# tusen-ai/SST

Measured on AMD Instinct MI355X. Metric: LiDAR frames/sec (SST backbone fwd+bwd) at Waymo 0.32m voxels, higher is better.
Workload: dtype f32 (storage, accumulation, attention, LayerNorm, reductions: fp32; the dense products of the encoder layers from the EXACT three-way bf16 split of both fp32 operands, six bf16 MFMA products with fp32 accumulation - error vs float64 <= 2 x the fp32 matrix pipe's: tests/test_gpu_dense_f32x6.py)

## Files before the change

include/sst_amd.h:

```cpp
#ifndef SST_AMD_H
#define SST_AMD_H

#include <stdint.h>

#ifdef __cplusplus
extern "C" {
#endif

#define SST_OK 0
#define SST_ERR_ARG (-1)
#define SST_ERR_UNSUPPORTED (-2)
#define SST_ERR_KEYSPACE (-3)

typedef enum { SST_REDUCE_SUM = 0, SST_REDUCE_MEAN = 1, SST_REDUCE_MAX = 2 } sst_reduce_t;

const char* sst_version(void);

int sst_dynamic_voxelize_f32(const float* d_points, int64_t n, int64_t row_stride,
                             const float voxel_size[3], const float coors_range[6],
                             int32_t* d_coors, int64_t coors_stride, int coors_col0, int batch_idx,
                             void* stream);
void sst_dynamic_voxelize_grid(const float voxel_size[3], const float coors_range[6], int32_t grid_xyz[3]);

int64_t sst_scan_workspace_bytes(int64_t n);
// ... 162 lines not shown
  float* out_b;
  int32_t p, bias_side, transpose_out, reserved;
} sst_wgrad_problem_bf16;
int64_t sst_wgrad_group_workspace_bytes(const sst_wgrad_problem_bf16* problems, int n);
int sst_wgrad_group_bf16(const sst_wgrad_problem_bf16* problems, int n, void* d_workspace, void* stream);
typedef struct sst_cast_problem_bf16 {
  const float* src;
  void* dst;
  int64_t ld_src;
  int32_t rows, cols, transpose, reserved;
} sst_cast_problem_bf16;
int sst_cast_group_bf16(const sst_cast_problem_bf16* problems, int n, void* stream);

int sst_gather_rows_f32(const float* d_src, int64_t ld_src, const int32_t* d_idx, int64_t n_out, int c,
                        float fill, float* d_out, int64_t ld_out, void* stream);
int sst_add_table_rows_f32(const float* d_x, int64_t ldx, const float* d_table, int64_t ld_table, const int32_t* d_idx, int64_t m,
                           int c, float* d_out, int64_t ld_out, void* stream);
int sst_scatter_rows_f32(const float* d_src, int64_t ld_src, const int32_t* d_idx, int64_t n_src, int c,
                         float* d_out, int64_t ld_out, void* stream);

int sst_add_layernorm_act_fwd_f32(const float* d_x, const float* d_res, const float* d_weight, const float* d_bias,
                                  int64_t m, int c, float eps, int act, float* d_y, float* d_sum, float* d_stats,
                                  void* stream);
int sst_add_layernorm_act_bwd_f32(const float* d_dy, const float* d_sum, const float* d_stats, const float* d_weight,
                                  const float* d_bias, int act, int64_t m, int c, float* d_dx, float* d_dweight,
                                  float* d_dbias, void* d_workspace, void* stream);
int sst_add_layernorm_fwd_f32(const float* d_x, const float* d_res, const float* d_weight, const float* d_bias,
                              int64_t m, int c, float eps, float* d_y, float* d_sum, float* d_stats,
                              void* stream);
int sst_add_layernorm_pos_fwd_f32(const float* d_x, const float* d_res, const float* d_weight, const float* d_bias, int64_t m,
                                  int c, float eps, float* d_y, float* d_sum, float* d_stats, const float* d_pos_table,
                                  const int32_t* d_pos_idx, float* d_y_plus_pos, void* stream);
int64_t sst_add_layernorm_bwd_workspace_bytes(int64_t m, int c);
int sst_add_layernorm_bwd_f32(const float* d_dy, const float* d_sum, const float* d_stats,
                              const float* d_weight, int64_t m, int c, float* d_dx, float* d_dweight,
                              float* d_dbias, void* d_workspace, void* stream);
int64_t sst_colsum_workspace_bytes(int64_t m, int c);
int sst_colsum_f32(const float* d_x, int64_t m, int c, int64_t ld, float* d_out, void* d_workspace, void* stream);

int64_t sst_weight_grad_workspace_bytes(int64_t m, int out, int in);
int sst_weight_grad_f32(const float* d_dy, const float* d_x, int64_t m, int out, int in, int64_t ld_dy,
                        int64_t ld_x, float* d_dw, float* d_db, void* d_workspace, void* stream);
typedef struct sst_wgrad_problem_f32 {
  const float* dy;
  const float* x;
  int64_t m, ld_dy, ld_x;
  float* dw;
  float* db;
  int32_t out, in;
  const float* x_add_rows;
  const int32_t* x_add_index;
} sst_wgrad_problem_f32;
int64_t sst_weight_grad_group_workspace_bytes(const sst_wgrad_problem_f32* problems, int n);
int sst_weight_grad_group_f32(const sst_wgrad_problem_f32* problems, int n, void* d_workspace, void* stream);
int64_t sst_weight_grad_group_f32x6_workspace_bytes(const sst_wgrad_problem_f32* problems, int n);
int sst_weight_grad_group_f32x6(const sst_wgrad_problem_f32* problems, int n, void* d_workspace, void* stream);
int sst_weight_grad_group_f32x6_plan(const sst_wgrad_problem_f32* problems, int n, int* tiles, int* slices,
                                     int64_t* tokens_per_slice, int* lean_slices);

int64_t sst_bn_workspace_bytes(int64_t n, int c);
int sst_bn_stats_f32(const float* d_x, int64_t n, int c, int64_t ld, float* d_mean, float* d_var,
                     void* d_workspace, void* stream);
int sst_bn_act_fwd_f32(const float* d_x, int64_t n, int c, int64_t ldx, const float* d_scale,
                       const float* d_shift, int act, float* d_y, int64_t ldy, void* stream);
int sst_bn_act_bwd_reduce_f32(const float* d_dy, const float* d_x, int64_t n, int c, int64_t lddy, int64_t ldx,
                              const float* d_mean, const float* d_invstd, const float* d_scale,
                              const float* d_shift, int act, float* d_sum_g, float* d_sum_gxhat,
                              void* d_workspace, void* stream);
int sst_bn_act_bwd_apply_f32(const float* d_dy, const float* d_x, int64_t n, int c, int64_t lddy, int64_t ldx,
                             const float* d_mean, const float* d_invstd, const float* d_scale,
                             const float* d_shift, const float* d_coef_a, const float* d_coef_b, float coef_scale,
                             int act, float* d_dx, int64_t lddx, void* stream);
int sst_bn_prepare_f32(const float* d_x, int64_t n, int c, int64_t ld, const float* d_weight, const float* d_bias,
                       float eps, float* d_running_mean, float* d_running_var, float factor, float* d_out4,
                       void* d_workspace, void* stream);
int sst_bn_prepare_tracked_f32(const float* d_x, int64_t n, int c, int64_t ld, const float* d_weight,
                               const float* d_bias, float eps, float* d_running_mean, float* d_running_var,
                               float factor, int64_t* d_num_batches_tracked, float* d_out4, void* d_workspace,
                               void* stream);
int sst_vfe_linear_moments_f32(const float* d_x, int64_t ldx, int64_t n, int k, const float* d_w, int64_t ldw, int c,
                               float* d_y, int64_t ldy, void* d_workspace, void* stream);
int sst_bn_prepare_from_partials_f32(int64_t n, int c, const float* d_weight, const float* d_bias, float eps,
                                     float* d_running_mean, float* d_running_var, float factor,
                                     int64_t* d_num_batches_tracked, float* d_out4, void* d_workspace, void* stream);
int sst_bn_stats_from_partials_f32(int64_t n, int c, float* d_mean, float* d_var, void* d_workspace, void* stream);
int sst_bn_act_pool_bwd_reduce_f32(const float* d_dy, const float* d_x, int64_t n, int c, int64_t lddy, int64_t ldx,
                                   const float* d_mean, const float* d_invstd, const float* d_scale, const float* d_shift,
                                   int act, const int32_t* d_group, const int32_t* d_arg, const float* d_dpool, int64_t ldp,
                                   float* d_sum_g, float* d_sum_gxhat, void* d_workspace, void* stream);
int sst_bn_act_pool_bwd_apply_f32(const float* d_dy, const float* d_x, int64_t n, int c, int64_t lddy, int64_t ldx,
                                  const float* d_mean, const float* d_invstd, const float* d_scale, const float* d_shift,
                                  const float* d_coef_a, const float* d_coef_b, float coef_scale, int act,
                                  const int32_t* d_group, const int32_t* d_arg, const float* d_dpool, int64_t ldp, float* d_dx,
                                  int64_t lddx, void* stream);
int sst_bn_act_res_fwd_f32(const float* d_x, int64_t n, int c, int64_t ldx, const float* d_res, int64_t ldr,
                           const float* d_scale, const float* d_shift, int act, float* d_y, int64_t ldy, void* stream);
int sst_bn_act_res_bwd_reduce_f32(const float* d_dy, const float* d_x, const float* d_res, int64_t n, int c,
                                  int64_t lddy, int64_t ldx, int64_t ldr, const float* d_mean, const float* d_invstd,
                                  const float* d_scale, const float* d_shift, int act, float* d_sum_g,
                                  float* d_sum_gxhat, void* d_workspace, void* stream);
int sst_bn_act_res_bwd_apply_f32(const float* d_dy, const float* d_x, const float* d_res, int64_t n, int c,
                                 int64_t lddy, int64_t ldx, int64_t ldr, const float* d_mean, const float* d_invstd,
                                 const float* d_scale, const float* d_shift, const float* d_coef_a,
                                 const float* d_coef_b, float coef_scale, int act, float* d_dres, int64_t lddres,
                                 float* d_dx, int64_t lddx, void* stream);

int sst_tall_linear_f32(const float* d_x, int64_t ldx, const float* d_w, int64_t ldw, const float* d_bias,
                        int64_t m, int n, int k, int trans_w, int accumulate, float* d_y, int64_t ldy,
                        void* stream);
int sst_tall_linear_ln_f32(const float* d_x, int64_t ldx, const float* d_w, int64_t ldw, const float* d_bias, int64_t m, int k,
                           const float* d_res, int64_t ldres, const float* d_ln_weight, const float* d_ln_bias, float eps,
                           float* d_y, float* d_sum, float* d_stats, const float* d_pos_table, const int32_t* d_pos_idx,
                           float* d_y_plus_pos, void* stream);
int sst_tall_linear_epi_f32x3(const float* d_x, int64_t ldx, const float* d_w, int64_t ldw, int trans_w, const float* d_bias,
                              int64_t m, int k, int n, int epilogue, const float* d_aux_in, float* d_aux_out, int64_t ldaux,
                              float* d_y, int64_t ldy, void* stream);
int sst_tall_linear_ln_f32x3(const float* d_x, int64_t ldx, const float* d_w, int64_t ldw, const float* d_bias, int64_t m, int k,
                             const float* d_res, int64_t ldres, const float* d_ln_weight, const float* d_ln_bias, float eps,
                             float* d_y, float* d_sum, float* d_stats, const float* d_pos_table, const int32_t* d_pos_idx,
                             float* d_y_plus_pos, void* stream);
int sst_tall_linear_epi_f32x6(const float* d_x, int64_t ldx, const float* d_w, int64_t ldw, int trans_w, const float* d_bias,
                              int64_t m, int k, int n, int epilogue, const float* d_aux_in, float* d_aux_out, int64_t ldaux,
                              float* d_y, int64_t ldy, void* stream);
int sst_tall_linear_epi2_f32x6(const float* d_x, const float* d_x2, int x2_from_col, int64_t ldx, const float* d_w, int64_t ldw,
                               int trans_w, const float* d_bias, int64_t m, int k, int n, int epilogue, const float* d_aux_in,
                               float* d_aux_out, int64_t ldaux, float* d_y, int64_t ldy, void* stream);
int sst_tall_linear_add_rows_f32x6(const float* d_x, int64_t ldx, const float* d_w, int64_t ldw, int64_t m, int k, int n,
                                   const float* d_rows, int64_t ldrows, const int32_t* d_row_index, float* d_y, int64_t ldy,
                                   void* stream);
int sst_inproj_pos_f32x6(const float* d_x, int64_t ldx, const float* d_rows, const int32_t* d_index, const float* d_w, int64_t ldw,
                         const float* d_bias, int64_t m, float* d_y, int64_t ldy, void* stream);
int sst_tall_linear_f32x6_partition(int64_t m, int groups, int64_t* row_blocks, int64_t* rows_per_wave);
int sst_tall_linear_ln_f32x6(const float* d_x, int64_t ldx, const float* d_w, int64_t ldw, const float* d_bias, int64_t m, int k,
                             const float* d_res, int64_t ldres, const float* d_ln_weight, const float* d_ln_bias, float eps,
                             float* d_y, float* d_sum, float* d_stats, const float* d_pos_table, const int32_t* d_pos_idx,
                             float* d_y_plus_pos, void* stream);
int sst_add_layernorm_bwd2_f32(const float* d_dy, const float* d_dy2, const float* d_sum, const float* d_stats,
                               const float* d_weight, int64_t m, int c, float* d_dx, float* d_dweight, float* d_dbias,
                               void* d_workspace, void* stream);
typedef struct sst_encoder_layer_fwd_args {
  int64_t m, n_windows;
  int32_t n_heads, act, max_tokens, impl;
  float eps, scale;
  const float *x, *xp;
  const float *w_in, *b_in, *w_out, *b_out, *w1, *b1, *w2, *b2, *n1w, *n1b, *n2w, *n2b;
  const int32_t *tok, *winoff, *order;
  const float* pos_table;
  const int32_t* pos_idx;
  float *qkv, *o, *lse, *y1, *s1, *st1, *pre, *h, *s2, *y2, *st2, *y2p;
  const float* head_scale;
  void* wpack;
  const float* xpos_table;
  const int32_t* xpos_idx;
} sst_encoder_layer_fwd_args;
typedef struct sst_encoder_layer_bwd_args {
  int64_t m, n_windows;
  int32_t n_heads, act, max_tokens, impl;
  float eps, scale;
  const float *dy2, *dy2p;
  const float *x, *xp, *qkv, *o, *lse, *s1, *st1, *y1, *pre, *h, *s2, *st2;
  const float *w_in, *w_out, *w1, *w2, *n1w, *n2w;
  const int32_t *tok, *winoff, *order;
  float *ds2, *dpre, *ds1, *d_o, *dqkv;
  float *dw_in, *db_in, *dwo, *dbo, *dw1, *db1, *dw2, *db2, *dn1w, *dn1b, *dn2w, *dn2b;
  void* workspace;
  const float* head_scale;
  float* cos_r;
  float* dy1;
  const void* wpack;
  const float* xpos_table;
  const int32_t* xpos_idx;
} sst_encoder_layer_bwd_args;
int64_t sst_encoder_layer_bwd_workspace_bytes(int64_t m, int n_heads);
int64_t sst_encoder_layer_wpack_bytes(void);
int sst_encoder_layer_fwd_f32x6(const sst_encoder_layer_fwd_args* args, void* stream);
int sst_encoder_layer_bwd_f32x6(const sst_encoder_layer_bwd_args* args, void* stream);

typedef struct sst_encoder_tail_fwd_args {
  int64_t m;
  int32_t act, reserved;
  float eps, reserved_f;
  const float *o, *x;
  const void* packed;
  const float *b_out, *b1, *b2, *n1w, *n1b, *n2w, *n2b;
  const float* pos_table;
  const int32_t* pos_idx;
  float *s1, *st1, *y1, *pre, *h, *s2, *st2, *y2, *y2p;
} sst_encoder_tail_fwd_args;
typedef struct sst_encoder_tail_bwd_args {
  int64_t m;
  int32_t act, reserved;
  const float *dy2, *dy2p, *s2, *st2, *pre, *s1, *st1;
  const void* packed;
  const float *n1w, *n2w;
  float *ds2, *dpre, *ds1, *d_o;
  float *dn2w, *dn2b, *dn1w, *dn1b;
  void* workspace;
} sst_encoder_tail_bwd_args;
int64_t sst_encoder_tail_pack_bytes(void);
int sst_encoder_tail_pack_f32x6(const float* d_w_out, const float* d_w1, const float* d_w2, void* d_packed, void* stream);
int sst_encoder_tail_pack_f32x6_many(const float* const* d_w_out, const float* const* d_w1, const float* const* d_w2,
                                     void* const* d_packed, int n, void* stream);
int64_t sst_encoder_tail_bwd_workspace_bytes(int64_t m);
int sst_encoder_tail_fwd_f32x6(const sst_encoder_tail_fwd_args* args, void* stream);
int sst_encoder_tail_bwd_f32x6(const sst_encoder_tail_bwd_args* args, void* stream);

typedef struct sst_encoder_tail_fwd_bf16_args {
  int64_t m;
  int32_t act, reserved;
  float eps, reserved_f;
  const void *o, *x;
  const void* packed;
  const float *b_out, *b1, *b2, *n1w, *n1b, *n2w, *n2b;
  const float* pos_table;
  const int32_t* pos_idx;
  void* s1;
  float* st1;
  void *y1, *pre, *h, *s2;
  float* st2;
  void *y2, *y2p;
} sst_encoder_tail_fwd_bf16_args;
typedef struct sst_encoder_tail_bwd_bf16_args {
  int64_t m;
  int32_t act, reserved;
  const void *dy2, *dy2p, *s2;
  const float* st2;
  const void *pre, *s1;
  const float* st1;
  const void* packed;
  const float *n1w, *n2w;
  void *ds2, *dpre, *ds1, *d_o;
  float *dn2w, *dn2b, *dn1w, *dn1b;
  void* workspace;
} sst_encoder_tail_bwd_bf16_args;
int64_t sst_encoder_tail_pack_bf16_bytes(void);
int sst_encoder_tail_pack_bf16(const float* d_w_out, const float* d_w1, const float* d_w2, void* d_packed, void* stream);
int sst_encoder_tail_pack_bf16_many(const float* const* d_w_out, const float* const* d_w1, const float* const* d_w2,
                                    void* const* d_packed, int n, void* stream);
int64_t sst_encoder_tail_bwd_bf16_workspace_bytes(int64_t m);
int sst_encoder_tail_fwd_bf16(const sst_encoder_tail_fwd_bf16_args* args, void* stream);
int sst_encoder_tail_bwd_bf16(const sst_encoder_tail_bwd_bf16_args* args, void* stream);

typedef struct sst_encoder_layer_fwd_bf16_args {
  int64_t m, n_windows;
  int32_t n_heads, act, max_tokens, reserved;
  float eps, scale;
  const void *x, *xp;
  const void *wqk, *wv, *wout, *w1, *w2;
  const float *b_in, *b_out, *b1, *b2, *n1w, *n1b, *n2w, *n2b;
  const int32_t *tok, *winoff, *order;
  const float* pos_table;
  const int32_t* pos_idx;
  void *qk, *v, *o;
  float* lse;
  void *y1, *s1;
  float* st1;
  void *pre, *h, *s2;
  float* st2;
  void *y2, *y2p;
  const float* head_scale;
  const void* wpack;
} sst_encoder_layer_fwd_bf16_args;
typedef struct sst_encoder_layer_bwd_bf16_args {
  int64_t m, n_windows;
  int32_t n_heads, act, max_tokens, reserved;
  float eps, scale;
  const void *dy2, *dy2p;
  const void *x, *xp, *qk, *v, *o;
  const float* lse;
  const void* s1;
  const float* st1;
  const void *y1, *pre, *h, *s2;
  const float* st2;
  const void *wqk_t, *wv_t, *wout_t, *w1_t, *w2_t;
  const float *n1w, *n2w;
  const int32_t *tok, *winoff, *order;
  void *ds2, *dpre, *dy1, *ds1, *d_o, *dqkv, *dxp, *dx;
  float *dw_in, *db_in, *dwo, *dbo, *dw1, *db1, *dw2, *db2, *dn1w, *dn1b, *dn2w, *dn2b;
  void* workspace;
  const float* head_scale;
  float* cos_r;
  const void* wpack;
} sst_encoder_layer_bwd_bf16_args;
int64_t sst_encoder_layer_bwd_bf16_workspace_bytes(int64_t m);
int sst_encoder_layer_fwd_bf16(const sst_encoder_layer_fwd_bf16_args* args, void* stream);
int sst_encoder_layer_bwd_bf16(const sst_encoder_layer_bwd_bf16_args* args, void* stream);

int sst_tall_linear_epi_f32(const float* d_x, int64_t ldx, const float* d_w, int64_t ldw, int trans_w, const float* d_bias,
                            int64_t m, int k, int n, int epilogue, const float* d_aux_in, float* d_aux_out, int64_t ldaux,
                            float* d_y, int64_t ldy, void* stream);
int sst_tall_linear_gelu_f32(const float* d_x, int64_t ldx, const float* d_w, int64_t ldw, const float* d_bias,
                             int64_t m, int n, int k, int trans_w, int mode, float* d_aux, float* d_y, int64_t ldy,
                             void* stream);

void* sst_event_create(void);
void sst_event_destroy(void* ev);
float sst_event_elapsed_ms(void* start, void* stop);
int sst_sra_attn_profile_next_fwd(void* start, void* stop);
int sst_sra_attn_profile_next_bwd(void* start, void* stop);

int64_t sst_connected_components_workspace_bytes(int64_t n);
int sst_connected_components_xy_f32(const float* d_points, int64_t ld, const int32_t* d_batch, int64_t n, float dist,
                                    int32_t* d_labels, int32_t* d_num_components, void* d_workspace, void* stream);

int64_t sst_dynamic_point_pool_workspace_bytes(int64_t n_rois, int64_t n_pts);
int sst_dynamic_point_pool_f32(const float* d_rois, const int32_t* d_rois_batch, int64_t n_rois, const float* d_pts,
                               int64_t ld_pts, const int32_t* d_pts_batch, int64_t n_pts, const float* extra_wlh,
                               int max_inbox_point, int64_t max_all_pts, int64_t* d_out_pts_idx,
                               int64_t* d_out_roi_idx, float* d_out_feats, int64_t* d_num_out, void* d_workspace,
                               void* stream);

int sst_spconv_candidates_i32(const int32_t* d_coors, int64_t n, const int32_t* in_shape, const int32_t* out_shape,
                              const int32_t* ksize, const int32_t* stride, const int32_t* padding,
                              const int32_t* dilation, int transpose, int32_t* d_rows, void* stream);
int sst_spconv_inverse_to_map_i32(const int32_t* d_inverse, int64_t total, int32_t* d_in2out, void* stream);
int sst_spconv_grid_subm_i32(const int32_t* d_coors, int64_t n, int batch, const int32_t* shape, const int32_t* ksize,
                             const int32_t* dilation, int32_t* d_grid, int32_t* d_in2out, int32_t* d_out2in,
                             void* stream);
int64_t sst_spconv_grid_conv_workspace_bytes(int64_t cells);
int sst_spconv_grid_conv_count_i32(const int32_t* d_coors, int64_t n, int batch, const int32_t* in_shape,
                                   const int32_t* out_shape, const int32_t* ksize, const int32_t* stride,
                                   const int32_t* padding, const int32_t* dilation, int transpose, void* d_workspace,
                                   int32_t* d_num_out, void* stream);
int sst_spconv_grid_conv_maps_i32(const int32_t* d_coors, int64_t n, int batch, const int32_t* in_shape,
                                  const int32_t* out_shape, const int32_t* ksize, const int32_t* stride,
                                  const int32_t* padding, const int32_t* dilation, int transpose, void* d_workspace,
                                  int64_t m, int32_t* d_outids, int32_t* d_in2out, int32_t* d_out2in, void* stream);
int sst_spconv_subm_map_i32(const int32_t* d_coors, int64_t n, const int32_t* shape, const int32_t* ksize,
                            const int32_t* dilation, const uint64_t* d_sorted_keys, const uint32_t* d_perm,
                            int32_t* d_in2out, void* stream);
int sst_spconv_invert_map_i32(const int32_t* d_in2out, int kvol, int64_t n, int64_t m, int32_t* d_out2in,
                              void* stream);
int64_t sst_spconv_pair_lists_workspace_bytes(int kvol, int64_t n);
int sst_spconv_pair_lists_i32(const int32_t* d_in2out, int kvol, int64_t n, int32_t* d_pairs, int32_t* d_num,
                              void* d_workspace, void* stream);
int sst_spconv_gather_gemm_f32(const float* d_x, int64_t ldx, const int32_t* d_map, int64_t m, int kvol,
                               const float* d_w, int cin, int cout, int trans_w, const float* d_bias, float* d_y,
                               int64_t ldy, int form, void* stream);
int sst_spconv_maxpool_fwd_f32(const float* d_x, int64_t ldx, const int32_t* d_out2in, int64_t m, int kvol, int c,
                               float* d_y, int64_t ldy, void* stream);
int sst_spconv_maxpool_bwd_f32(const float* d_x, int64_t ldx, const float* d_y, int64_t ldy, const float* d_dy,
                               int64_t lddy, const int32_t* d_in2out, int64_t n, int kvol, int c, float* d_dx,
                               int64_t lddx, void* stream);
int64_t sst_spconv_conv_os_workspace_bytes(int kvol, int cin, int cout);
int sst_spconv_conv_os_tile_rows(int64_t m, int cout, int tile_cfg);
int sst_spconv_os_tile_work_i32(const int32_t* d_map, int64_t m, int kvol, int tile_rows, int32_t* d_work, void* stream);
int sst_spconv_conv_os_f32(const float* d_x, int64_t ldx, const int32_t* d_map, int64_t m, int kvol, const float* d_w,
                           int cin, int cout, int trans_w, const float* d_bias, float* d_y, int64_t ldy,
                           int tile_cfg, const int32_t* d_tile_order, void* d_workspace, void* stream);
int sst_spconv_conv_os_f32x3(const float* d_x, int64_t ldx, const int32_t* d_map, int64_t m, int kvol, const float* d_w,
                             int cin, int cout, int trans_w, const float* d_bias, float* d_y, int64_t ldy, int tile_cfg,
// ... 701 lines not shown
```

sst_amd/_lib.py:

```python
import ctypes
import os
import subprocess

import torch

_HERE = os.path.dirname(os.path.abspath(__file__))
_CSRC = os.path.join(_HERE, 'csrc')
LIB_PATH = os.path.join(_CSRC, 'libsst_amd.so')

_lib = None

c_i64 = ctypes.c_int64
c_i32 = ctypes.c_int
c_f32 = ctypes.c_float
c_ptr = ctypes.c_void_p



class WgradProblemBF16(ctypes.Structure):
    _fields_ = [('a', c_ptr), ('b', c_ptr), ('lda', c_i64), ('ldb', c_i64), ('m', c_i64), ('out_w', c_ptr),
                ('out_b', c_ptr), ('p', ctypes.c_int32), ('bias_side', ctypes.c_int32),
                ('transpose_out', ctypes.c_int32), ('reserved', ctypes.c_int32)]


# ... 18 lines not shown
                ('out', ctypes.c_int32), ('inn', ctypes.c_int32), ('x_add_rows', c_ptr), ('x_add_index', c_ptr)]


def _struct(name, doc, fields):
    return type(name, (ctypes.Structure,), {'__doc__': doc, '_fields_': fields})


_I32 = ctypes.c_int32
RoiAssignArgs = _struct('RoiAssignArgs', 'sst_roi_assign_args of include/sst_amd.h', (
    [(k, ctypes.c_void_p) for k in ('props', 'prop_labels', 'prop_offsets', 'gts', 'gt_labels', 'gt_offsets', 'iou', 'max_iou',
                                    'argmax')]
    + [(k, c_i64) for k in ('n_props', 'n_gts', 'ld')]
    + [(k, _I32) for k in ('prop_cols', 'gt_cols', 'batch', 'num_classes', 'class_mask', 'reserved')]))
RoiSampleArgs = _struct('RoiSampleArgs', 'sst_roi_sample_args of include/sst_amd.h', (
    [(k, ctypes.c_void_p) for k in ('props', 'prop_labels', 'prop_offsets', 'gts', 'gt_labels', 'gt_offsets', 'iou', 'max_iou',
                                    'argmax', 'keys', 'assigned', 'rois', 'src', 'gt_index', 'labels', 'iou_out', 'soft_label',
                                    'reg_mask', 'targets', 'counts')]
    + [(k, c_i64) for k in ('n_props', 'n_gts', 'ld', 'max_props_per_sample')]
    + [(k, _I32) for k in ('prop_cols', 'gt_cols', 'batch', 'num_classes', 'class_mask', 'num', 'num_expected_pos', 'n_pieces')]
    + [(k, ctypes.c_float * 16) for k in ('pos_iou_thr', 'neg_iou_thr', 'min_pos_iou')]
    + [('piece_thr', ctypes.c_float * 8)]
    + [(k, ctypes.c_double * 16) for k in ('cls_pos_thr', 'cls_neg_thr')]
    + [('piece_frac', ctypes.c_double * 8)]))
RoiLossArgs = _struct('RoiLossArgs', 'sst_roi_loss_args of include/sst_amd.h', (
    [(k, ctypes.c_void_p) for k in ('cls_score', 'bbox_pred', 'nonempty', 'rois', 'soft_label', 'reg_mask', 'targets',
                                    'gt_index', 'labels', 'gts')]
    + [(k, c_i64) for k in ('n', 'n_gts')]
    + [(k, _I32) for k in ('roi_cols', 'gt_cols', 'with_corner', 'car_index')]
    + [(k, ctypes.c_float) for k in ('beta', 'w_cls', 'w_reg', 'w_corner')]
    + [('code_weight', ctypes.c_float * 7), ('reserved', ctypes.c_float)]))

AnchorGrid = _struct('AnchorGrid', 'sst_anchor_grid of include/sst_amd.h', (
    [('centers', ctypes.c_void_p)] + [(k, _I32) for k in ('H', 'W', 'n_sizes', 'n_rots')]
    + [('sizes', ctypes.c_float * 3 * 8), ('rots', ctypes.c_float * 4)]))
AnchorLossArgs = _struct('AnchorLossArgs', 'sst_anchor_loss_args of include/sst_amd.h', (
    [(k, ctypes.c_void_p) for k in ('cls_score', 'bbox_pred', 'dir_pred', 'assigned', 'gts', 'gt_labels', 'gt_offsets',
                                    'pos_counts')]
    + [('n_gts', c_i64)]
    + [(k, _I32) for k in ('gt_cols', 'batch', 'num_classes', 'smooth_l1', 'sin_diff', 'reserved')]
    + [(k, ctypes.c_float) for k in ('gamma', 'alpha', 'w_cls', 'w_bbox', 'w_dir', 'beta', 'pos_weight', 'dir_offset')]
    + [('code_weight', ctypes.c_float * 7), ('reserved_f', ctypes.c_float)]))

FgSampleArgs = _struct('FgSampleArgs', 'sst_fg_sample_args of include/sst_amd.h', (
    [(k, ctypes.c_void_p) for k in ('logits', 'votes', 'points', 'batch_idx', 'extra_mask', 'slot', 'mask', 'src', 'centers',
                                    'batch_out', 'points_out', 'info', 'aux', 'aux_out', 'aux_inv')]
    + [(k, c_i64) for k in ('n', 'ld_logits', 'ld_votes', 'ld_points', 'max_rows', 'aux_rows')]
    + [(k, _I32) for k in ('num_classes', 'point_cols', 'batch', 'batch_is_i64', 'apply_rule', 'sample_major')]
    + [('thresholds', ctypes.c_float * 32)]))
FgGatherArgs = _struct('FgGatherArgs', 'sst_fg_gather_args of include/sst_amd.h', (
    [(k, ctypes.c_void_p) for k in ('idx', 'logits', 'votes', 'feats', 'points', 'out', 'points_out')]
    + [(k, c_i64) for k in ('m', 'n', 'ld_logits', 'ld_votes', 'ld_feats', 'ld_points')]
    + [(k, _I32) for k in ('c_logits', 'c_votes', 'c_feats', 'c_points')]))
FgGroupSampleArgs = _struct('FgGroupSampleArgs', 'sst_fg_group_sample_args of include/sst_amd.h', (
    [(k, ctypes.c_void_p) for k in ('logits', 'votes', 'points', 'batch_idx', 'extra_mask', 'slot', 'mask', 'src', 'centers',
                                    'batch_out', 'points_out', 'info')]
    + [(k, c_i64) for k in ('n', 'ld_logits', 'ld_votes', 'ld_points', 'max_rows')]
    + [(k, _I32) for k in ('num_groups', 'num_logits', 'point_cols', 'batch', 'batch_is_i64', 'apply_rule')]
    + [('offset_scale', ctypes.c_float), ('thresholds', ctypes.c_float * 32), ('group_begin', ctypes.c_uint8 * 33),
       ('group_class', ctypes.c_uint8 * 64)]))
FgVirtualRowsArgs = _struct('FgVirtualRowsArgs', 'sst_fg_virtual_rows_args of include/sst_amd.h', (
    [(k, ctypes.c_void_p) for k in ('src', 'centers', 'feats', 'logits', 'points', 'out', 'clipped')]
    + [(k, c_i64) for k in ('m', 'n', 'ld_feats', 'ld_logits', 'ld_points')]
    + [(k, _I32) for k in ('c_feats', 'c_logits', 'c_points', 'reserved')]
    + [('lo', ctypes.c_float * 3), ('hi', ctypes.c_float * 3)]))
DeformConvShape = _struct('DeformConvShape', 'sst_deform_conv_shape of include/sst_amd.h', [
    (k, _I32) for k in ('batch', 'in_channels', 'height', 'width', 'out_channels', 'kernel_h', 'kernel_w', 'stride_h', 'stride_w',
                        'pad_h', 'pad_w', 'dil_h', 'dil_w', 'groups', 'deform_groups', 'reserved')])
OptimHyper = _struct('OptimHyper', 'sst_optim_hyper of include/sst_amd.h', (
    [(k, ctypes.c_double * 8) for k in ('lr', 'wd', 'b1', 'b2', 'eps')]
    + [(k, ctypes.c_double) for k in ('max_norm', 'growth_factor', 'backoff_factor')]
    + [(k, _I32) for k in ('growth_interval', 'scale_mode', 'skip_nonfinite', 'n_groups')]))
TrackletTargetsArgs = _struct('TrackletTargetsArgs', 'sst_tracklet_targets_args of include/sst_amd.h', (
    [(k, ctypes.c_void_p) for k in ('boxes', 'ts', 'scores', 'trk_offsets', 'cand_boxes', 'cand_ts', 'cand_offsets',
                                    'trk_cand_offsets', 'trk_class', 'chosen', 'counts', 'matched', 'overlaps',
                                    'assigned_gt_inds', 'rois', 'src', 'frame_inds', 'gt_index', 'labels', 'iou_out',
                                    'scores_out', 'soft_label', 'reg_mask', 'targets', 'pos_gt_bboxes')]
    + [(k, c_i64) for k in ('n_rows', 'n_cand_rows', 'n_cands', 'n_tracklets')]
    + [(k, _I32) for k in ('num_classes', 'object_centric')]
    + [(k, ctypes.c_float) for k in ('candidate_thresh', 'iou_thr')]
    + [(k, ctypes.c_double * 16) for k in ('cls_pos_thr', 'cls_neg_thr')]))
TrackletRowsArgs = _struct('TrackletRowsArgs', 'sst_tracklet_rows_args of include/sst_amd.h', (
    [(k, ctypes.c_void_p) for k in ('feats', 'xyz', 'pts_frame_inds', 'pts_inds', 'roi_inds', 'roi_frame_inds', 'roi_scores',
                                    'out', 'xyz_out')]
    + [(k, c_i64) for k in ('m', 'n_points', 'n_rois', 'ld_feats', 'ld_xyz')]
    + [(k, _I32) for k in ('feat_cols', 'xyz_cols', 'combined', 'with_roi_scores')]))
IncrArgs = _struct('IncrArgs', 'sst_incr_args of include/sst_amd.h', (
    [('points', ctypes.c_void_p * 16), ('frame_inds', ctypes.c_void_p * 16), ('n_points', c_i64 * 16)]
    + [(k, ctypes.c_void_p) for k in ('boxes', 'box_offsets', 'keys', 'counts', 'out', 'workspace')]
    + [('workspace_bytes', c_i64), ('seg_base', c_i64 * (16 * 20))]
    + [(k, _I32) for k in ('n_samples', 'cols', 'n_frames', 'n_queries', 'n_boxes', 'max_crop_points', 'lower_bound')]
    + [(k, _I32 * 4) for k in ('q_inc', 'q_lo', 'q_hi')]
    + [('q_tag', ctypes.c_float * 4), ('lo', ctypes.c_float * 3), ('vs', ctypes.c_float * 3), ('grid', _I32 * 3)]))
IncrDeltaArgs = _struct('IncrDeltaArgs', 'sst_incr_delta_args of include/sst_amd.h', (
    [('base', ctypes.c_void_p * 8), ('n_base', c_i64 * 8), ('ld_base', c_i64 * 8), ('query', ctypes.c_void_p),
     ('n_query', c_i64), ('ld_query', c_i64), ('mask', ctypes.c_void_p), ('workspace', ctypes.c_void_p),
     ('workspace_bytes', c_i64), ('n_clouds', _I32), ('lower_bound', _I32), ('lo', ctypes.c_float * 3),
     ('vs', ctypes.c_float * 3), ('grid', _I32 * 3)]))
FrameTransformArgs = _struct('FrameTransformArgs', 'sst_frame_transform_args of include/sst_amd.h', (
    [('src', ctypes.c_void_p * 8), ('dst', ctypes.c_void_p * 8), ('n', c_i64 * 8), ('mat', (ctypes.c_float * 12) * 8),
     ('n_clouds', _I32), ('cols', _I32)]))
AugmentParams = _struct('AugmentParams', 'sst_augment_params of include/sst_amd.h', (
    [(k, _I32) for k in ('flip_h', 'flip_v', 'rotate', 'shuffle')]
    + [(k, ctypes.c_float) for k in ('cos', 'sin', 'scale', 'angle')]
    + [('trans', ctypes.c_float * 3), ('reserved', ctypes.c_float), ('range', ctypes.c_float * 6), ('seed', ctypes.c_uint64)]))
AugmentArgs = _struct('AugmentArgs', 'sst_augment_args of include/sst_amd.h', (
    [(k, ctypes.c_void_p) for k in ('points', 'row_offsets', 'n_pasted', 'block_offsets', 'params', 'planes', 'plane_offsets',
                                    'out', 'counts', 'workspace')]
    + [(k, c_i64) for k in ('workspace_bytes', 'n_total')]
    + [(k, _I32) for k in ('batch', 'cols', 'n_blocks', 'n_planes', 'norm_mask', 'reserved')]
    + [('norm_mean', ctypes.c_float * 8), ('norm_std', ctypes.c_float * 8)]))
AugmentBoxArgs = _struct('AugmentBoxArgs', 'sst_augment_box_args of include/sst_amd.h', (
    [(k, ctypes.c_void_p) for k in ('boxes', 'labels', 'box_offsets', 'params', 'boxes_out', 'labels_out', 'counts')]
    + [(k, _I32) for k in ('batch', 'cols', 'n_boxes', 'filter', 'always_rotate', 'reserved')]))
TrackletAugmentArgs = _struct('TrackletAugmentArgs', 'sst_tracklet_augment_args of include/sst_amd.h', (
    [(k, ctypes.c_void_p) for k in ('points', 'frame_rows', 'sample_frames', 'block_offsets', 'frames', 'frame_values', 'params',
                                    'out', 'out_frame_inds', 'counts', 'workspace')]
    + [(k, c_i64) for k in ('workspace_bytes', 'n_total')]
    + [(k, _I32) for k in ('batch', 'cols', 'deco', 'n_blocks', 'n_frames', 'max_frames')]))
TrackletTTAViewsArgs = _struct('TrackletTTAViewsArgs', 'sst_tracklet_tta_views_args of include/sst_amd.h', (
    [(k, ctypes.c_void_p) for k in ('points', 'frame_rows', 'sample_frames', 'block_offsets', 'frames', 'frame_values', 'params',
                                    'out', 'out_frame_inds', 'counts', 'workspace')]
    + [(k, c_i64) for k in ('workspace_bytes', 'n_total')]
    + [(k, _I32) for k in ('batch', 'cols', 'deco', 'n_blocks', 'n_frames', 'max_frames', 'n_views', 'reserved')]))
TrackletTTABoxArgs = _struct('TrackletTTABoxArgs', 'sst_tracklet_tta_box_args of include/sst_amd.h', (
    [(k, ctypes.c_void_p) for k in ('boxes', 'box_offsets', 'params', 'boxes_out')]
    + [(k, _I32) for k in ('batch', 'cols', 'n_boxes', 'n_views')]))
TrackletTTAView = _struct('TrackletTTAView', 'sst_tracklet_tta_view of include/sst_amd.h', (
    [(k, _I32) for k in ('flip_h', 'flip_v', 'rotate')] + [(k, ctypes.c_float) for k in ('angle', 'cos', 'sin')]
    + [('reserved', ctypes.c_float * 2)]))
TrackletTTAFinishArgs = _struct('TrackletTTAFinishArgs', 'sst_tracklet_tta_finish_args of include/sst_amd.h', (
    [(k, ctypes.c_void_p) for k in ('boxes', 'scores', 'valid', 'old_boxes', 'old_scores', 'mats', 'merged_boxes', 'merged_scores',
                                    'view_boxes', 'view_scores', 'workspace')]
    + [(k, c_i64) for k in ('workspace_bytes', 'n_rows')]
    + [(k, _I32) for k in ('n_views', 'mode')] + [('iou_merge_thresh', ctypes.c_float), ('reserved', _I32)]
    + [('views', TrackletTTAView * 32)]))
TrackletAffinityArgs = _struct('TrackletAffinityArgs', 'sst_tracklet_affinity_args of include/sst_amd.h', (
    [(k, ctypes.c_void_p) for k in ('pd_boxes', 'pd_ts', 'pd_offsets', 'gt_boxes', 'gt_ts', 'gt_offsets', 'pd_gt_begin', 'pd_gt_end',
                                    'out_offsets', 'block_offsets', 'affinity')]
    + [(k, c_i64) for k in ('n_pd_rows', 'n_gt_rows', 'n_pd', 'n_gt', 'n_out', 'n_blocks')]))
BoxCropsArgs = _struct('BoxCropsArgs', 'sst_box_crops_args of include/sst_amd.h', (
    [(k, ctypes.c_void_p) for k in ('points', 'boxes', 'pt_offsets', 'box_offsets', 'tile_offsets', 'cell_offsets', 'counts',
                                    'tile_counts', 'tile_starts', 'total', 'rows', 'src', 'workspace')]
    + [(k, c_i64) for k in ('workspace_bytes', 'n_points', 'n_boxes', 'n_tiles', 'n_cells', 'n_rows')]
    + [(k, _I32) for k in ('n_frames', 'cols')]))
FgGroupOffsets = _struct('FgGroupOffsets', 'sst_fg_group_offsets of include/sst_amd.h', [('off', c_i64 * 33)])

_P = ctypes.c_void_p
EncoderLayerFwdArgs = _struct('EncoderLayerFwdArgs', 'sst_encoder_layer_fwd_args of include/sst_amd.h', (
    [('m', c_i64), ('n_windows', c_i64)] + [(k, ctypes.c_int32) for k in ('n_heads', 'act', 'max_tokens', 'impl')]
    + [('eps', ctypes.c_float), ('scale', ctypes.c_float)]
    + [(k, _P) for k in ('x', 'xp', 'w_in', 'b_in', 'w_out', 'b_out', 'w1', 'b1', 'w2', 'b2', 'n1w', 'n1b', 'n2w', 'n2b',
                         'tok', 'winoff', 'order', 'pos_table', 'pos_idx',
                         'qkv', 'o', 'lse', 'y1', 's1', 'st1', 'pre', 'h', 's2', 'y2', 'st2', 'y2p', 'head_scale', 'wpack',
                         'xpos_table', 'xpos_idx')]))
EncoderLayerBwdArgs = _struct('EncoderLayerBwdArgs', 'sst_encoder_layer_bwd_args of include/sst_amd.h', (
    [('m', c_i64), ('n_windows', c_i64)] + [(k, ctypes.c_int32) for k in ('n_heads', 'act', 'max_tokens', 'impl')]
    + [('eps', ctypes.c_float), ('scale', ctypes.c_float)]
    + [(k, _P) for k in ('dy2', 'dy2p', 'x', 'xp', 'qkv', 'o', 'lse', 's1', 'st1', 'y1', 'pre', 'h', 's2', 'st2',
                         'w_in', 'w_out', 'w1', 'w2', 'n1w', 'n2w', 'tok', 'winoff', 'order',
                         'ds2', 'dpre', 'ds1', 'd_o', 'dqkv',
                         'dw_in', 'db_in', 'dwo', 'dbo', 'dw1', 'db1', 'dw2', 'db2', 'dn1w', 'dn1b', 'dn2w', 'dn2b',
                         'workspace', 'head_scale', 'cos_r', 'dy1', 'wpack', 'xpos_table', 'xpos_idx')]))


EncoderTailFwdArgs = _struct('EncoderTailFwdArgs', 'sst_encoder_tail_fwd_args of include/sst_amd.h', (
    [('m', c_i64), ('act', ctypes.c_int32), ('reserved', ctypes.c_int32), ('eps', ctypes.c_float), ('reserved_f', ctypes.c_float)]
    + [(k, _P) for k in ('o', 'x', 'packed', 'b_out', 'b1', 'b2', 'n1w', 'n1b', 'n2w', 'n2b', 'pos_table', 'pos_idx',
                         's1', 'st1', 'y1', 'pre', 'h', 's2', 'st2', 'y2', 'y2p')]))
EncoderTailBwdArgs = _struct('EncoderTailBwdArgs', 'sst_encoder_tail_bwd_args of include/sst_amd.h', (
    [('m', c_i64), ('act', ctypes.c_int32), ('reserved', ctypes.c_int32)]
    + [(k, _P) for k in ('dy2', 'dy2p', 's2', 'st2', 'pre', 's1', 'st1', 'packed', 'n1w', 'n2w',
                         'ds2', 'dpre', 'ds1', 'd_o', 'dn2w', 'dn2b', 'dn1w', 'dn1b', 'workspace')]))

EncoderTailFwdBF16Args = _struct('EncoderTailFwdBF16Args', 'sst_encoder_tail_fwd_bf16_args of include/sst_amd.h', (
    [('m', c_i64), ('act', ctypes.c_int32), ('reserved', ctypes.c_int32), ('eps', ctypes.c_float), ('reserved_f', ctypes.c_float)]
    + [(k, _P) for k in ('o', 'x', 'packed', 'b_out', 'b1', 'b2', 'n1w', 'n1b', 'n2w', 'n2b', 'pos_table', 'pos_idx',
                         's1', 'st1', 'y1', 'pre', 'h', 's2', 'st2', 'y2', 'y2p')]))
EncoderTailBwdBF16Args = _struct('EncoderTailBwdBF16Args', 'sst_encoder_tail_bwd_bf16_args of include/sst_amd.h', (
    [('m', c_i64), ('act', ctypes.c_int32), ('reserved', ctypes.c_int32)]
    + [(k, _P) for k in ('dy2', 'dy2p', 's2', 'st2', 'pre', 's1', 'st1', 'packed', 'n1w', 'n2w',
                         'ds2', 'dpre', 'ds1', 'd_o', 'dn2w', 'dn2b', 'dn1w', 'dn1b', 'workspace')]))


EncoderLayerFwdBF16Args = _struct('EncoderLayerFwdBF16Args', 'sst_encoder_layer_fwd_bf16_args of include/sst_amd.h', (
    [('m', c_i64), ('n_windows', c_i64)] + [(k, ctypes.c_int32) for k in ('n_heads', 'act', 'max_tokens', 'reserved')]
    + [('eps', ctypes.c_float), ('scale', ctypes.c_float)]
    + [(k, _P) for k in ('x', 'xp', 'wqk', 'wv', 'wout', 'w1', 'w2', 'b_in', 'b_out', 'b1', 'b2', 'n1w', 'n1b', 'n2w', 'n2b',
                         'tok', 'winoff', 'order', 'pos_table', 'pos_idx',
                         'qk', 'v', 'o', 'lse', 'y1', 's1', 'st1', 'pre', 'h', 's2', 'st2', 'y2', 'y2p', 'head_scale', 'wpack')]))
EncoderLayerBwdBF16Args = _struct('EncoderLayerBwdBF16Args', 'sst_encoder_layer_bwd_bf16_args of include/sst_amd.h', (
    [('m', c_i64), ('n_windows', c_i64)] + [(k, ctypes.c_int32) for k in ('n_heads', 'act', 'max_tokens', 'reserved')]
    + [('eps', ctypes.c_float), ('scale', ctypes.c_float)]
    + [(k, _P) for k in ('dy2', 'dy2p', 'x', 'xp', 'qk', 'v', 'o', 'lse', 's1', 'st1', 'y1', 'pre', 'h', 's2', 'st2',
                         'wqk_t', 'wv_t', 'wout_t', 'w1_t', 'w2_t', 'n1w', 'n2w', 'tok', 'winoff', 'order',
                         'ds2', 'dpre', 'dy1', 'ds1', 'd_o', 'dqkv', 'dxp', 'dx',
                         'dw_in', 'db_in', 'dwo', 'dbo', 'dw1', 'db1', 'dw2', 'db2', 'dn1w', 'dn1b', 'dn2w', 'dn2b',
                         'workspace', 'head_scale', 'cos_r', 'wpack')]))


_SIGNATURES = {
    'sst_version': (ctypes.c_char_p, []),
    'sst_dynamic_voxelize_f32': (c_i32, [c_ptr, c_i64, c_i64, c_ptr, c_ptr, c_ptr, c_i64, c_i32, c_i32, c_ptr]),
    'sst_dynamic_voxelize_grid': (None, [c_ptr, c_ptr, c_ptr]),
    'sst_scan_workspace_bytes': (c_i64, [c_i64]),
    'sst_exclusive_scan_i32': (c_i32, [c_ptr, c_ptr, c_i64, c_ptr, c_ptr, c_ptr]),
    'sst_sort_workspace_bytes': (c_i64, [c_i64]),
    'sst_sort_pairs_u64': (c_i32, [c_ptr, c_ptr, c_ptr, c_i64, c_i32, c_ptr, c_ptr]),
    'sst_unique_workspace_bytes': (c_i64, [c_i64]),
    'sst_unique_rows': (c_i32, [c_ptr, c_i32, c_i64, c_i32, c_i64, c_ptr, c_ptr, c_i32,
                                c_ptr, c_ptr, c_ptr, c_ptr, c_ptr, c_ptr, c_ptr]),
    'sst_unpack_keys': (c_i32, [c_ptr, c_i64, c_i32, c_ptr, c_ptr, c_ptr, c_i32, c_i64, c_i32, c_ptr]),
    'sst_segment_reduce_fwd_f32': (c_i32, [c_ptr, c_i64, c_i32, c_ptr, c_ptr, c_ptr, c_i64, c_i32, c_ptr, c_ptr,
                                           c_ptr, c_ptr]),
    'sst_encoder_layer_bwd_workspace_bytes': (c_i64, [c_i64, c_i32]),
    'sst_tall_linear_f32x6_partition': (c_i32, [c_i64, c_i32, c_ptr, c_ptr]),
    'sst_inproj_pos_f32x6': (c_i32, [c_ptr, c_i64, c_ptr, c_ptr, c_ptr, c_i64, c_ptr, c_i64, c_ptr, c_i64, c_ptr]),
    'sst_encoder_layer_wpack_bytes': (c_i64, []),
    'sst_encoder_layer_fwd_f32x6': (c_i32, [c_ptr, c_ptr]),
    'sst_encoder_layer_bwd_f32x6': (c_i32, [c_ptr, c_ptr]),
    'sst_encoder_tail_pack_bytes': (c_i64, []),
    'sst_encoder_tail_pack_f32x6': (c_i32, [c_ptr, c_ptr, c_ptr, c_ptr, c_ptr]),
    'sst_encoder_tail_pack_f32x6_many': (c_i32, [c_ptr, c_ptr, c_ptr, c_ptr, c_i32, c_ptr]),
    'sst_encoder_tail_bwd_workspace_bytes': (c_i64, [c_i64]),
    'sst_encoder_tail_fwd_f32x6': (c_i32, [c_ptr, c_ptr]),
    'sst_encoder_tail_bwd_f32x6': (c_i32, [c_ptr, c_ptr]),
    'sst_encoder_tail_pack_bf16_bytes': (c_i64, []),
    'sst_encoder_tail_pack_bf16': (c_i32, [c_ptr, c_ptr, c_ptr, c_ptr, c_ptr]),
    'sst_encoder_tail_pack_bf16_many': (c_i32, [c_ptr, c_ptr, c_ptr, c_ptr, c_i32, c_ptr]),
    'sst_encoder_tail_bwd_bf16_workspace_bytes': (c_i64, [c_i64]),
    'sst_encoder_tail_fwd_bf16': (c_i32, [c_ptr, c_ptr]),
    'sst_encoder_tail_bwd_bf16': (c_i32, [c_ptr, c_ptr]),
    'sst_encoder_layer_bwd_bf16_workspace_bytes': (c_i64, [c_i64]),
    'sst_encoder_layer_fwd_bf16': (c_i32, [c_ptr, c_ptr]),
    'sst_encoder_layer_bwd_bf16': (c_i32, [c_ptr, c_ptr]),
    'sst_segment_reduce_work_words': (c_i64, [c_i64, c_i64, c_i32]),
    'sst_segment_reduce_fwd_work_f32': (c_i32, [c_ptr, c_i64, c_i32, c_ptr, c_ptr, c_ptr, c_i64, c_i32, c_ptr, c_ptr,
                                                c_ptr, c_ptr, c_i64, c_ptr, c_ptr, c_ptr]),
    'sst_vfe_linear_moments_f32': (c_i32, [c_ptr, c_i64, c_i64, c_i32, c_ptr, c_i64, c_i32, c_ptr, c_i64, c_ptr, c_ptr]),
    'sst_bn_prepare_from_partials_f32': (c_i32, [c_i64, c_i32, c_ptr, c_ptr, c_f32, c_ptr, c_ptr, c_f32, c_ptr, c_ptr, c_ptr,
                                                 c_ptr]),
    'sst_bn_stats_from_partials_f32': (c_i32, [c_i64, c_i32, c_ptr, c_ptr, c_ptr, c_ptr]),
    'sst_bn_act_pool_bwd_reduce_f32': (c_i32, [c_ptr, c_ptr, c_i64, c_i32, c_i64, c_i64, c_ptr, c_ptr, c_ptr, c_ptr, c_i32,
                                               c_ptr, c_ptr, c_ptr, c_i64, c_ptr, c_ptr, c_ptr, c_ptr]),
    'sst_bn_act_pool_bwd_apply_f32': (c_i32, [c_ptr, c_ptr, c_i64, c_i32, c_i64, c_i64, c_ptr, c_ptr, c_ptr, c_ptr, c_ptr,
                                              c_ptr, c_f32, c_i32, c_ptr, c_ptr, c_ptr, c_i64, c_ptr, c_i64, c_ptr]),
    'sst_tall_linear_add_rows_f32x6': (c_i32, [c_ptr, c_i64, c_ptr, c_i64, c_i64, c_i32, c_i32, c_ptr, c_i64, c_ptr, c_ptr,
                                               c_i64, c_ptr]),
    'sst_segment_long_scratch_bytes': (c_i64, [c_i64, c_i64, c_i32]),
    'sst_segment_reduce_long_f32': (c_i32, [c_ptr, c_i64, c_i32, c_ptr, c_ptr, c_i32, c_ptr, c_i64, c_i32, c_ptr, c_ptr, c_ptr,
                                            c_ptr]),
    'sst_segment_reduce_profile_next': (c_i32, [c_ptr, c_ptr]),
    'sst_segment_reduce_bwd_f32': (c_i32, [c_ptr, c_i64, c_i32, c_ptr, c_i32, c_ptr, c_ptr, c_ptr, c_i64, c_i32,
                                           c_ptr, c_ptr, c_ptr]),
    'sst_ingroup_rank_workspace_bytes': (c_i64, [c_i64]),
    'sst_ingroup_rank_i64': (c_i32, [c_ptr, c_i64, c_i32, c_ptr, c_ptr, c_ptr]),
    'sst_window_coors': (c_i32, [c_ptr, c_i32, c_i64, c_ptr, c_ptr, c_ptr, c_ptr, c_ptr, c_ptr, c_ptr]),
    'sst_window_order_i32': (c_i32, [c_ptr, c_i32, c_i32, c_ptr, c_ptr]),
    'sst_region_batching_workspace_bytes': (c_i64, [c_i64]),
    'sst_region_batching': (c_i32, [c_ptr, c_ptr, c_i64, c_i32, c_ptr, c_i32] + [c_ptr] * 15 + [c_ptr, c_ptr]),
    'sst_frame_windows_per_sample': (c_i64, [c_ptr, c_ptr]),
    'sst_frame_voxels_i32': (c_i32, [c_ptr, c_ptr, c_ptr, c_i64, c_i32, c_ptr, c_i32, c_ptr, c_ptr, c_ptr, c_ptr,
                                     c_ptr, c_ptr, c_ptr]),
    'sst_window_plan_workspace_bytes': (c_i64, [c_i64, c_i64]),
    'sst_window_plan_i32': (c_i32, [c_ptr, c_ptr, c_i64, c_i32, c_ptr, c_ptr, c_ptr, c_i32, ctypes.c_uint32] + [c_ptr] * 11),
    'sst_sra_attn_fwd_f32': (c_i32, [c_ptr, c_ptr, c_ptr, c_i64, c_i64, c_i64, c_ptr, c_ptr, c_i64, c_i32,
                                     c_f32, c_i32, c_i32, c_ptr, c_i64, c_ptr, c_ptr]),
    'sst_sra_attn_bwd_f32': (c_i32, [c_ptr] * 6 + [c_i64] * 5 + [c_ptr, c_ptr, c_i64, c_i64, c_i32, c_f32,
                                                                 c_i32, c_i32, c_ptr, c_ptr, c_ptr,
                                                                 c_i64, c_i64, c_i64, c_ptr, c_ptr]),
    'sst_sra_attn_fwd_ord_f32': (c_i32, [c_ptr, c_ptr, c_ptr, c_i64, c_i64, c_i64, c_ptr, c_ptr, c_ptr, c_i64, c_i32,
                                         c_f32, c_i32, c_i32, c_ptr, c_i64, c_ptr, c_ptr]),
    'sst_sra_attn_bwd_ord_f32': (c_i32, [c_ptr] * 6 + [c_i64] * 5 + [c_ptr, c_ptr, c_ptr, c_i64, c_i64, c_i32, c_f32,
                                                                     c_i32, c_i32, c_ptr, c_ptr, c_ptr,
                                                                     c_i64, c_i64, c_i64, c_ptr, c_ptr]),
    'sst_sra_attn_bwd_workspace_bytes': (c_i64, [c_i64, c_i32]),
    'sst_sra_attn_cos_fwd_f32': (c_i32, [c_ptr, c_ptr, c_ptr, c_i64, c_i64, c_i64, c_ptr, c_ptr, c_ptr, c_i64, c_i32,
                                         c_ptr, c_i32, c_ptr, c_i64, c_ptr, c_ptr]),
    'sst_sra_attn_cos_bwd_f32': (c_i32, [c_ptr] * 6 + [c_i64] * 5 + [c_ptr, c_ptr, c_ptr, c_i64, c_i64, c_i32, c_ptr,
                                                                     c_i32, c_ptr, c_ptr, c_ptr,
                                                                     c_i64, c_i64, c_i64, c_ptr, c_ptr]),
    'sst_sra_attn_fwd_bf16': (c_i32, [c_ptr, c_ptr, c_ptr, c_i64, c_i64, c_i64, c_ptr, c_ptr, c_i64, c_i32, c_f32, c_i32,
                                      c_ptr, c_i64, c_ptr, c_ptr]),
    'sst_sra_attn_bwd_bf16': (c_i32, [c_ptr] * 6 + [c_i64] * 5 + [c_ptr, c_ptr, c_i64, c_i32, c_f32, c_i32, c_ptr, c_ptr,
                                                                  c_ptr, c_i64, c_i64, c_i64, c_ptr]),
    'sst_sra_attn_bf16_profile_next': (c_i32, [c_i32, c_ptr, c_ptr]),
    'sst_sra_attn_fwd_ord_bf16': (c_i32, [c_ptr, c_ptr, c_ptr, c_i64, c_i64, c_i64, c_ptr, c_ptr, c_ptr, c_i64, c_i32, c_f32,
                                          c_i32, c_ptr, c_i64, c_ptr, c_ptr]),
    'sst_sra_attn_bwd_ord_bf16': (c_i32, [c_ptr] * 6 + [c_i64] * 5 + [c_ptr, c_ptr, c_ptr, c_i64, c_i32, c_f32, c_i32, c_ptr,
                                                                      c_ptr, c_ptr, c_i64, c_i64, c_i64, c_ptr]),
    'sst_sra_attn_cos_fwd_bf16': (c_i32, [c_ptr, c_ptr, c_ptr, c_i64, c_i64, c_i64, c_ptr, c_ptr, c_ptr, c_i64, c_i32, c_ptr,
                                          c_i32, c_ptr, c_i64, c_ptr, c_ptr]),
    'sst_sra_attn_cos_bwd_bf16': (c_i32, [c_ptr] * 6 + [c_i64] * 5 + [c_ptr, c_ptr, c_ptr, c_i64, c_i32, c_ptr, c_i32, c_ptr,
                                                                      c_ptr, c_ptr, c_i64, c_i64, c_i64, c_ptr, c_ptr]),
    'sst_add_layernorm_fwd_bf16': (c_i32, [c_ptr, c_ptr, c_ptr, c_ptr, c_i64, c_i32, c_f32, c_ptr, c_ptr, c_ptr, c_ptr,
                                           c_ptr, c_ptr, c_ptr]),
    'sst_add_layernorm_bwd_bf16': (c_i32, [c_ptr, c_ptr, c_ptr, c_ptr, c_ptr, c_i64, c_i32, c_ptr, c_ptr, c_ptr, c_ptr,
                                           c_ptr]),
    'sst_cast_add_pos_bf16': (c_i32, [c_ptr, c_i32, c_i64, c_i32, c_ptr, c_ptr, c_ptr, c_ptr]),
    'sst_weight_grad_group_workspace_bytes': (c_i64, [c_ptr, c_i32]),
    'sst_weight_grad_group_f32': (c_i32, [c_ptr, c_i32, c_ptr, c_ptr]),
    'sst_weight_grad_group_f32x6_workspace_bytes': (c_i64, [c_ptr, c_i32]),
    'sst_weight_grad_group_f32x6': (c_i32, [c_ptr, c_i32, c_ptr, c_ptr]),
    'sst_weight_grad_group_f32x6_plan': (c_i32, [c_ptr, c_i32, c_ptr, c_ptr, c_ptr, c_ptr]),
    'sst_tall_linear_ln_f32': (c_i32, [c_ptr, c_i64, c_ptr, c_i64, c_ptr, c_i64, c_i32, c_ptr, c_i64, c_ptr, c_ptr, c_f32, c_ptr,
                                       c_ptr, c_ptr, c_ptr, c_ptr, c_ptr, c_ptr]),
    'sst_tall_linear_ln_f32x3': (c_i32, [c_ptr, c_i64, c_ptr, c_i64, c_ptr, c_i64, c_i32, c_ptr, c_i64, c_ptr, c_ptr, c_f32, c_ptr,
                                         c_ptr, c_ptr, c_ptr, c_ptr, c_ptr, c_ptr]),
    'sst_tall_linear_epi_f32x3': (c_i32, [c_ptr, c_i64, c_ptr, c_i64, c_i32, c_ptr, c_i64, c_i32, c_i32, c_i32, c_ptr, c_ptr,
                                          c_i64, c_ptr, c_i64, c_ptr]),
    'sst_tall_linear_ln_f32x6': (c_i32, [c_ptr, c_i64, c_ptr, c_i64, c_ptr, c_i64, c_i32, c_ptr, c_i64, c_ptr, c_ptr, c_f32, c_ptr,
                                         c_ptr, c_ptr, c_ptr, c_ptr, c_ptr, c_ptr]),
    'sst_tall_linear_epi_f32x6': (c_i32, [c_ptr, c_i64, c_ptr, c_i64, c_i32, c_ptr, c_i64, c_i32, c_i32, c_i32, c_ptr, c_ptr,
                                          c_i64, c_ptr, c_i64, c_ptr]),
    'sst_tall_linear_epi2_f32x6': (c_i32, [c_ptr, c_ptr, c_i32, c_i64, c_ptr, c_i64, c_i32, c_ptr, c_i64, c_i32, c_i32, c_i32,
                                           c_ptr, c_ptr, c_i64, c_ptr, c_i64, c_ptr]),
    'sst_add_layernorm_bwd2_f32': (c_i32, [c_ptr, c_ptr, c_ptr, c_ptr, c_ptr, c_i64, c_i32, c_ptr, c_ptr, c_ptr, c_ptr, c_ptr]),
    'sst_tall_linear_epi_f32': (c_i32, [c_ptr, c_i64, c_ptr, c_i64, c_i32, c_ptr, c_i64, c_i32, c_i32, c_i32, c_ptr, c_ptr,
                                        c_i64, c_ptr, c_i64, c_ptr]),
    'sst_tall_linear_bf16': (c_i32, [c_ptr, c_i64, c_ptr, c_ptr, c_i64, c_i32, c_i32, c_i32, c_ptr, c_ptr, c_i64, c_ptr,
                                     c_i64, c_ptr]),
    'sst_tall_linear_bf16_partition': (c_i32, [c_i64, c_i32, c_i32, c_i32, c_ptr, c_ptr]),
    'sst_tall_linear_ln_bf16': (c_i32, [c_ptr, c_i64, c_ptr, c_ptr, c_i64, c_i32, c_ptr, c_i64, c_ptr, c_ptr, c_f32, c_ptr, c_ptr,
                                        c_ptr, c_ptr, c_ptr, c_ptr, c_ptr]),
    'sst_wgrad_group_workspace_bytes': (c_i64, [c_ptr, c_i32]),
    'sst_wgrad_group_bf16': (c_i32, [c_ptr, c_i32, c_ptr, c_ptr]),
    'sst_cast_group_bf16': (c_i32, [c_ptr, c_i32, c_ptr]),
    'sst_gather_rows_f32': (c_i32, [c_ptr, c_i64, c_ptr, c_i64, c_i32, c_f32, c_ptr, c_i64, c_ptr]),
    'sst_add_table_rows_f32': (c_i32, [c_ptr, c_i64, c_ptr, c_i64, c_ptr, c_i64, c_i32, c_ptr, c_i64, c_ptr]),
    'sst_scatter_rows_f32': (c_i32, [c_ptr, c_i64, c_ptr, c_i64, c_i32, c_ptr, c_i64, c_ptr]),
    'sst_add_layernorm_fwd_f32': (c_i32, [c_ptr, c_ptr, c_ptr, c_ptr, c_i64, c_i32, c_f32, c_ptr, c_ptr, c_ptr,
                                          c_ptr]),
    'sst_add_layernorm_bwd_workspace_bytes': (c_i64, [c_i64, c_i32]),
    'sst_add_layernorm_pos_fwd_f32': (c_i32, [c_ptr, c_ptr, c_ptr, c_ptr, c_i64, c_i32, c_f32, c_ptr, c_ptr, c_ptr, c_ptr, c_ptr,
                                              c_ptr, c_ptr]),
    'sst_add_layernorm_act_fwd_f32': (c_i32, [c_ptr, c_ptr, c_ptr, c_ptr, c_i64, c_i32, c_f32, c_i32, c_ptr, c_ptr, c_ptr,
                                              c_ptr]),
    'sst_add_layernorm_act_bwd_f32': (c_i32, [c_ptr, c_ptr, c_ptr, c_ptr, c_ptr, c_i32, c_i64, c_i32, c_ptr, c_ptr, c_ptr,
                                              c_ptr, c_ptr]),
    'sst_add_layernorm_bwd_f32': (c_i32, [c_ptr, c_ptr, c_ptr, c_ptr, c_i64, c_i32, c_ptr, c_ptr, c_ptr, c_ptr,
                                          c_ptr]),
    'sst_weight_grad_workspace_bytes': (c_i64, [c_i64, c_i32, c_i32]),
    'sst_weight_grad_f32': (c_i32, [c_ptr, c_ptr, c_i64, c_i32, c_i32, c_i64, c_i64, c_ptr, c_ptr, c_ptr, c_ptr]),
    'sst_colsum_workspace_bytes': (c_i64, [c_i64, c_i32]),
    'sst_colsum_f32': (c_i32, [c_ptr, c_i64, c_i32, c_i64, c_ptr, c_ptr, c_ptr]),
    'sst_tall_linear_f32': (c_i32, [c_ptr, c_i64, c_ptr, c_i64, c_ptr, c_i64, c_i32, c_i32, c_i32, c_i32, c_ptr, c_i64,
                                    c_ptr]),
    'sst_tall_linear_gelu_f32': (c_i32, [c_ptr, c_i64, c_ptr, c_i64, c_ptr, c_i64, c_i32, c_i32, c_i32, c_i32, c_ptr, c_ptr,
                                         c_i64, c_ptr]),
    'sst_connected_components_workspace_bytes': (c_i64, [c_i64]),
    'sst_connected_components_xy_f32': (c_i32, [c_ptr, c_i64, c_ptr, c_i64, ctypes.c_float, c_ptr, c_ptr, c_ptr, c_ptr]),
    'sst_dynamic_point_pool_workspace_bytes': (c_i64, [c_i64, c_i64]),
    'sst_dynamic_point_pool_f32': (c_i32, [c_ptr, c_ptr, c_i64, c_ptr, c_i64, c_ptr, c_i64, c_ptr, c_i32, c_i64, c_ptr,
                                           c_ptr, c_ptr, c_ptr, c_ptr, c_ptr]),
    'sst_spconv_candidates_i32': (c_i32, [c_ptr, c_i64, c_ptr, c_ptr, c_ptr, c_ptr, c_ptr, c_ptr, c_i32, c_ptr, c_ptr]),
    'sst_spconv_inverse_to_map_i32': (c_i32, [c_ptr, c_i64, c_ptr, c_ptr]),
    'sst_spconv_grid_subm_i32': (c_i32, [c_ptr, c_i64, c_i32, c_ptr, c_ptr, c_ptr, c_ptr, c_ptr, c_ptr, c_ptr]),
    'sst_spconv_grid_conv_workspace_bytes': (c_i64, [c_i64]),
    'sst_spconv_grid_conv_count_i32': (c_i32, [c_ptr, c_i64, c_i32, c_ptr, c_ptr, c_ptr, c_ptr, c_ptr, c_ptr, c_i32, c_ptr,
                                               c_ptr, c_ptr]),
    'sst_spconv_grid_conv_maps_i32': (c_i32, [c_ptr, c_i64, c_i32, c_ptr, c_ptr, c_ptr, c_ptr, c_ptr, c_ptr, c_i32, c_ptr,
                                              c_i64, c_ptr, c_ptr, c_ptr, c_ptr]),
    'sst_spconv_subm_map_i32': (c_i32, [c_ptr, c_i64, c_ptr, c_ptr, c_ptr, c_ptr, c_ptr, c_ptr, c_ptr]),
    'sst_spconv_invert_map_i32': (c_i32, [c_ptr, c_i32, c_i64, c_i64, c_ptr, c_ptr]),
    'sst_spconv_pair_lists_workspace_bytes': (c_i64, [c_i32, c_i64]),
    'sst_spconv_pair_lists_i32': (c_i32, [c_ptr, c_i32, c_i64, c_ptr, c_ptr, c_ptr, c_ptr]),
    'sst_spconv_gather_gemm_f32': (c_i32, [c_ptr, c_i64, c_ptr, c_i64, c_i32, c_ptr, c_i32, c_i32, c_i32, c_ptr, c_ptr,
                                           c_i64, c_i32, c_ptr]),
    'sst_spconv_conv_os_workspace_bytes': (c_i64, [c_i32, c_i32, c_i32]),
    'sst_spconv_conv_os_f32': (c_i32, [c_ptr, c_i64, c_ptr, c_i64, c_i32, c_ptr, c_i32, c_i32, c_i32, c_ptr, c_ptr, c_i64,
                                       c_i32, c_ptr, c_ptr, c_ptr]),
    'sst_spconv_conv_os_tile_rows': (c_i32, [c_i64, c_i32, c_i32]),
    'sst_spconv_conv_os_f32x3': (c_i32, [c_ptr, c_i64, c_ptr, c_i64, c_i32, c_ptr, c_i32, c_i32, c_i32, c_ptr, c_ptr, c_i64,
# ... 314 lines not shown
```

sst_amd/csrc/gelu.h:

```cpp
#pragma once
#include <math.h>
#include "common.h"

namespace {

enum { kEpiBias = 0, kEpiGelu = 1, kEpiRelu = 2, kEpiMulGeluGrad = 3, kEpiMulReluGrad = 4, kEpiAdd = 5, kEpiAddLN = 6,
       kEpiAddRows = 7 };

__device__ __forceinline__ float erf_as(float z, float& e) {
  const float az = fabsf(z);
  const float t = __builtin_amdgcn_rcpf(fmaf(0.3275911f, az, 1.f));
  e = __expf(-az * az);
  const float poly = t * fmaf(t, fmaf(t, fmaf(t, fmaf(t, 1.061405429f, -1.453152027f), 1.421413741f), -0.284496736f), 0.254829592f);
  return copysignf(fmaf(-poly, e, 1.f), z);
}
__device__ __forceinline__ float gelu_f(float x) {
  float e;
  return 0.5f * x * (1.f + erf_as(x * 0.70710678118654752f, e));
}
__device__ __forceinline__ float gelu_grad_f(float x) {
  float e;
  const float phi = 0.5f * (1.f + erf_as(x * 0.70710678118654752f, e));
  return fmaf(x * 0.3989422804014327f, e, phi);
}

}
```

sst_amd/csrc/layer_exec.hip:

```cpp
#include <stdint.h>
#include "common.h"

namespace {

enum { kEpiBias = 0, kEpiGelu = 1, kEpiRelu = 2, kEpiMulGeluGrad = 3, kEpiMulReluGrad = 4, kEpiAdd = 5 };
constexpr int kC = 128, kFF = 256;

int64_t wg_ws(int64_t m, int which) {
  sst_wgrad_problem_f32 p[5];
  float* const any = (float*)(uintptr_t)256;
  for (auto& q : p) {
    q.dy = q.x = any;
    q.dw = q.db = any;
    q.m = m;
    q.x_add_rows = nullptr, q.x_add_index = nullptr;
  }
  if (which == 0 || which == 2) {
    p[0].ld_dy = kC, p[0].ld_x = kFF, p[0].out = kC, p[0].in = kFF;
    p[1].ld_dy = kFF, p[1].ld_x = kC, p[1].out = kFF, p[1].in = kC;
    if (which == 0) return sst_weight_grad_group_f32x6_workspace_bytes(p, 2);
    p[2].ld_dy = kC, p[2].ld_x = kC, p[2].out = kC, p[2].in = kC;
    p[3].ld_dy = 3 * kC, p[3].ld_x = kC, p[3].out = 2 * kC, p[3].in = kC;
    p[4].ld_dy = 3 * kC, p[4].ld_x = kC, p[4].out = kC, p[4].in = kC;
    return sst_weight_grad_group_f32x6_workspace_bytes(p, 5);
  }
  p[0].ld_dy = kC, p[0].ld_x = kC, p[0].out = kC, p[0].in = kC;
  p[1].ld_dy = 3 * kC, p[1].ld_x = kC, p[1].out = 2 * kC, p[1].in = kC;
  p[2].ld_dy = 3 * kC, p[2].ld_x = kC, p[2].out = kC, p[2].in = kC;
  return sst_weight_grad_group_f32x6_workspace_bytes(p, 3);
}

int64_t wg_ws_bf16(int64_t m) {
  sst_wgrad_problem_bf16 p[5];
  for (auto& q : p) q.m = m;
  p[0].p = 2 * kC, p[1].p = kC, p[2].p = kC, p[3].p = kFF, p[4].p = kFF;
  return sst_wgrad_group_workspace_bytes(p, 5);
}

}

extern "C" {

int64_t sst_encoder_layer_bwd_workspace_bytes(int64_t m, int n_heads) {
  if (m < 0 || n_heads < 1) return SST_ERR_ARG;
  const int64_t a = sst_encoder_tail_bwd_workspace_bytes(m), d = sst_sra_attn_bwd_workspace_bytes(m, n_heads), e = wg_ws(m, 2);
  if (a < 0 || d < 0 || e < 0) return SST_ERR_UNSUPPORTED;
  return sst_align_up(a, 256) + sst_align_up(e, 256) + sst_align_up(d, 256) + 256;
}

int64_t sst_encoder_layer_wpack_bytes(void) { return sst_encoder_tail_pack_bytes(); }

int sst_encoder_layer_fwd_f32x6(const sst_encoder_layer_fwd_args* a, void* stream) {
  if (!a || a->m < 0 || a->n_heads * 16 != kC || (a->act != 1 && a->act != 2)) return SST_ERR_ARG;
  if (a->m == 0) return SST_OK;
  if (!a->x || !a->qkv || !a->o || !a->lse || !a->y1 || !a->st1 || !a->pre || !a->h || !a->s2 || !a->y2 || !a->st2)
    return SST_ERR_ARG;
  if (!a->xp && (!a->xpos_table || !a->xpos_idx)) return SST_ERR_ARG;
  const int64_t m = a->m;
  int rc;
  if (a->xp == nullptr)
    rc = sst_inproj_pos_f32x6(a->x, kC, a->xpos_table, a->xpos_idx, a->w_in, kC, a->b_in, m, a->qkv, 3 * kC, stream);
  else
    rc = sst_tall_linear_epi2_f32x6(a->xp, a->x, 2 * kC, kC, a->w_in, kC, 0, a->b_in, m, kC, 3 * kC, kEpiBias, nullptr, nullptr, 0,
                                    a->qkv, 3 * kC, stream);
  if (rc) return rc;
  if (a->head_scale != nullptr)
    rc = sst_sra_attn_cos_fwd_f32(a->qkv, a->qkv + kC, a->qkv + 2 * kC, 3 * kC, 3 * kC, 3 * kC, a->tok, a->winoff, a->order,
                                  a->n_windows, a->n_heads, a->head_scale, a->max_tokens, a->o, kC, a->lse, stream);
  else
    rc = sst_sra_attn_fwd_ord_f32(a->qkv, a->qkv + kC, a->qkv + 2 * kC, 3 * kC, 3 * kC, 3 * kC, a->tok, a->winoff, a->order,
                                  a->n_windows, a->n_heads, a->scale, a->max_tokens, a->impl, a->o, kC, a->lse, stream);
  if (rc) return rc;
  if (!a->wpack) return SST_ERR_ARG;
  if (a->w_out || a->w1 || a->w2) {
    rc = sst_encoder_tail_pack_f32x6(a->w_out, a->w1, a->w2, a->wpack, stream);
    if (rc) return rc;
  }
  sst_encoder_tail_fwd_args t;
  t.m = m, t.act = a->act, t.reserved = 0, t.eps = a->eps, t.reserved_f = 0.f;
  t.o = a->o, t.x = a->x, t.packed = a->wpack;
  t.b_out = a->b_out, t.b1 = a->b1, t.b2 = a->b2, t.n1w = a->n1w, t.n1b = a->n1b, t.n2w = a->n2w, t.n2b = a->n2b;
  t.pos_table = a->pos_table, t.pos_idx = a->pos_idx;
  t.s1 = a->s1, t.st1 = a->st1, t.y1 = a->y1, t.pre = a->pre, t.h = a->h, t.s2 = a->s2, t.st2 = a->st2, t.y2 = a->y2;
  t.y2p = a->pos_table != nullptr ? a->y2p : nullptr;
  return sst_encoder_tail_fwd_f32x6(&t, stream);
}

int sst_encoder_layer_bwd_f32x6(const sst_encoder_layer_bwd_args* a, void* stream) {
  if (!a || a->m < 0 || a->n_heads * 16 != kC || (a->act != 1 && a->act != 2)) return SST_ERR_ARG;
  if (a->m == 0) return SST_OK;
  if (!a->dy2 || !a->workspace || !a->ds2 || !a->dpre || !a->ds1 || !a->d_o || !a->dqkv || !a->wpack) return SST_ERR_ARG;
  if (!a->dn2w || !a->dn2b || !a->dn1w || !a->dn1b) return SST_ERR_ARG;
  if (!a->xp && (!a->xpos_table || !a->xpos_idx)) return SST_ERR_ARG;
  const int64_t m = a->m;
  char* ws = (char*)a->workspace;
  void* ws_tail = ws;
  ws += sst_align_up(sst_encoder_tail_bwd_workspace_bytes(m), 256);
  void* ws_wg = ws;
  ws += sst_align_up(wg_ws(m, 2), 256);
  void* ws_sra = ws;
  int rc;
  sst_encoder_tail_bwd_args t;
  t.m = m, t.act = a->act, t.reserved = 0;
  t.dy2 = a->dy2, t.dy2p = a->dy2p, t.s2 = a->s2, t.st2 = a->st2, t.pre = a->pre, t.s1 = a->s1, t.st1 = a->st1;
  t.packed = a->wpack, t.n1w = a->n1w, t.n2w = a->n2w;
  t.ds2 = a->ds2, t.dpre = a->dpre, t.ds1 = a->ds1, t.d_o = a->d_o;
  t.dn2w = a->dn2w, t.dn2b = a->dn2b, t.dn1w = a->dn1w, t.dn1b = a->dn1b;
  t.workspace = ws_tail;
  float *part2 = nullptr, *part1 = nullptr;
  int rows = 0;
  rc = sst_internal_encoder_tail_bwd_f32x6(&t, &part2, &part1, &rows, stream);
  if (rc) return rc;
  sst_colsum_rider riders[2];
  riders[0].partials = part2, riders[0].nb = rows, riders[0].width = 2 * kC, riders[0].split = kC;
  riders[0].out0 = a->dn2w, riders[0].out1 = a->dn2b;
  riders[1].partials = part1, riders[1].nb = rows, riders[1].width = 2 * kC, riders[1].split = kC;
  riders[1].out0 = a->dn1w, riders[1].out1 = a->dn1b;
  if (a->head_scale != nullptr)
    rc = sst_sra_attn_cos_bwd_f32(a->qkv, a->qkv + kC, a->qkv + 2 * kC, a->o, a->d_o, a->lse, 3 * kC, 3 * kC, 3 * kC, kC, kC, a->tok,
                                  a->winoff, a->order, a->n_windows, m, a->n_heads, a->head_scale, a->max_tokens, a->dqkv,
                                  a->dqkv + kC, a->dqkv + 2 * kC, 3 * kC, 3 * kC, 3 * kC, a->cos_r, stream);
  else
    rc = sst_sra_attn_bwd_ord_f32(a->qkv, a->qkv + kC, a->qkv + 2 * kC, a->o, a->d_o, a->lse, 3 * kC, 3 * kC, 3 * kC, kC, kC, a->tok,
                                  a->winoff, a->order, a->n_windows, m, a->n_heads, a->scale, a->max_tokens, a->impl, a->dqkv,
                                  a->dqkv + kC, a->dqkv + 2 * kC, 3 * kC, 3 * kC, 3 * kC, ws_sra, stream);
  if (rc) return rc;
  sst_wgrad_problem_f32 g[5];
  for (auto& q : g) q.x_add_rows = nullptr, q.x_add_index = nullptr;
  g[0].dy = a->ds2, g[0].x = a->h, g[0].m = m, g[0].ld_dy = kC, g[0].ld_x = kFF, g[0].dw = a->dw2, g[0].db = a->db2;
  g[0].out = kC, g[0].in = kFF;
  g[1].dy = a->dpre, g[1].x = a->y1, g[1].m = m, g[1].ld_dy = kFF, g[1].ld_x = kC, g[1].dw = a->dw1, g[1].db = a->db1;
  g[1].out = kFF, g[1].in = kC;
  g[2].dy = a->ds1, g[2].x = a->o, g[2].m = m, g[2].ld_dy = kC, g[2].ld_x = kC, g[2].dw = a->dwo, g[2].db = a->dbo;
  g[2].out = kC, g[2].in = kC;
  g[3].dy = a->dqkv, g[3].x = a->xp ? a->xp : a->x, g[3].m = m, g[3].ld_dy = 3 * kC, g[3].ld_x = kC, g[3].dw = a->dw_in;
  g[3].db = a->db_in, g[3].out = 2 * kC, g[3].in = kC;
  if (!a->xp) g[3].x_add_rows = a->xpos_table, g[3].x_add_index = a->xpos_idx;
  g[4].dy = a->dqkv + 2 * kC, g[4].x = a->x, g[4].m = m, g[4].ld_dy = 3 * kC, g[4].ld_x = kC;
  g[4].dw = a->dw_in + 2 * kC * kC, g[4].db = a->db_in + 2 * kC, g[4].out = kC, g[4].in = kC;
  rc = sst_internal_weight_grad_group_f32x6(g, 5, ws_wg, riders, 2, stream);
  if (rc) return rc;
  return sst_tall_linear_epi_f32x6(a->dqkv, 3 * kC, a->w_in, kC, 1, nullptr, m, 3 * kC, kC, kEpiAdd, a->ds1, nullptr, kC, a->ds1, kC,
                                   stream);
}

int64_t sst_encoder_layer_bwd_bf16_workspace_bytes(int64_t m) {
  if (m < 0) return SST_ERR_ARG;
  const int64_t a = sst_encoder_tail_bwd_bf16_workspace_bytes(m), b = wg_ws_bf16(m);
  if (a < 0 || b < 0) return SST_ERR_UNSUPPORTED;
  return sst_align_up(a, 256) + sst_align_up(b, 256) + 256;
}

int sst_encoder_layer_fwd_bf16(const sst_encoder_layer_fwd_bf16_args* a, void* stream) {
  if (!a || a->m < 0 || a->n_heads * 16 != kC || (a->act != 1 && a->act != 2)) return SST_ERR_ARG;
  if (a->m == 0) return SST_OK;
  if (!a->x || !a->xp || !a->wqk || !a->wv || !a->wout || !a->w1 || !a->w2 || !a->qk || !a->v || !a->o || !a->lse || !a->y1 ||
      !a->st1 || !a->pre || !a->h || !a->y2 || !a->st2)
    return SST_ERR_ARG;
  const int64_t m = a->m;
  const unsigned short* qk = (const unsigned short*)a->qk;
  int rc;
  rc = sst_tall_linear_bf16(a->xp, kC, a->wqk, a->b_in, m, kC, 2 * kC, kEpiBias, nullptr, nullptr, 0, a->qk, 2 * kC, stream);
  if (rc) return rc;
  rc = sst_tall_linear_bf16(a->x, kC, a->wv, a->b_in ? a->b_in + 2 * kC : nullptr, m, kC, kC, kEpiBias, nullptr, nullptr, 0, a->v,
                            kC, stream);
  if (rc) return rc;
  if (a->head_scale != nullptr)
    rc = sst_sra_attn_cos_fwd_bf16(qk, qk + kC, a->v, 2 * kC, 2 * kC, kC, a->tok, a->winoff, a->order, a->n_windows, a->n_heads,
                                   a->head_scale, a->max_tokens, a->o, kC, a->lse, stream);
  else
    rc = sst_sra_attn_fwd_ord_bf16(qk, qk + kC, a->v, 2 * kC, 2 * kC, kC, a->tok, a->winoff, a->order, a->n_windows, a->n_heads,
                                   a->scale, a->max_tokens, a->o, kC, a->lse, stream);
  if (rc) return rc;
  if (!a->wpack) return SST_ERR_ARG;
  sst_encoder_tail_fwd_bf16_args t;
  t.m = m, t.act = a->act, t.reserved = 0, t.eps = a->eps, t.reserved_f = 0.f;
  t.o = a->o, t.x = a->x, t.packed = a->wpack;
  t.b_out = a->b_out, t.b1 = a->b1, t.b2 = a->b2, t.n1w = a->n1w, t.n1b = a->n1b, t.n2w = a->n2w, t.n2b = a->n2b;
  t.pos_table = a->pos_table, t.pos_idx = a->pos_idx;
  t.s1 = a->s1, t.st1 = a->st1, t.y1 = a->y1, t.pre = a->pre, t.h = a->h, t.s2 = a->s2, t.st2 = a->st2, t.y2 = a->y2;
  t.y2p = a->pos_table ? a->y2p : nullptr;
  return sst_encoder_tail_fwd_bf16(&t, stream);
}

int sst_encoder_layer_bwd_bf16(const sst_encoder_layer_bwd_bf16_args* a, void* stream) {
  if (!a || a->m < 0 || a->n_heads * 16 != kC || (a->act != 1 && a->act != 2)) return SST_ERR_ARG;
  if (a->m == 0) return SST_OK;
  if (!a->dy2 || !a->workspace || !a->ds2 || !a->dpre || !a->ds1 || !a->d_o || !a->dqkv || !a->dxp || !a->dx ||
      !a->s1 || !a->s2 || !a->wpack)
    return SST_ERR_ARG;
  if (!a->dn2w || !a->dn2b || !a->dn1w || !a->dn1b) return SST_ERR_ARG;
  const int64_t m = a->m;
  char* ws = (char*)a->workspace;
  void* ws_tail = ws;
  ws += sst_align_up(sst_encoder_tail_bwd_bf16_workspace_bytes(m), 256);
  void* ws_wg = ws;
  const unsigned short* qk = (const unsigned short*)a->qk;
  unsigned short* dqkv = (unsigned short*)a->dqkv;
  int rc;
  sst_encoder_tail_bwd_bf16_args t;
  t.m = m, t.act = a->act, t.reserved = 0;
  t.dy2 = a->dy2, t.dy2p = a->dy2p, t.s2 = a->s2, t.st2 = a->st2, t.pre = a->pre, t.s1 = a->s1, t.st1 = a->st1;
  t.packed = a->wpack, t.n1w = a->n1w, t.n2w = a->n2w;
  t.ds2 = a->ds2, t.dpre = a->dpre, t.ds1 = a->ds1, t.d_o = a->d_o;
  t.dn2w = a->dn2w, t.dn2b = a->dn2b, t.dn1w = a->dn1w, t.dn1b = a->dn1b;
  t.workspace = ws_tail;
  float *part2 = nullptr, *part1 = nullptr;
  int rows = 0;
  rc = sst_internal_encoder_tail_bwd_bf16(&t, &part2, &part1, &rows, stream);
  if (rc) return rc;
  sst_colsum_rider riders[2];
  riders[0].partials = part2, riders[0].nb = rows, riders[0].width = 2 * kC, riders[0].split = kC;
  riders[0].out0 = a->dn2w, riders[0].out1 = a->dn2b;
  riders[1].partials = part1, riders[1].nb = rows, riders[1].width = 2 * kC, riders[1].split = kC;
  riders[1].out0 = a->dn1w, riders[1].out1 = a->dn1b;
  if (a->head_scale != nullptr)
    rc = sst_sra_attn_cos_bwd_bf16(qk, qk + kC, a->v, a->o, a->d_o, a->lse, 2 * kC, 2 * kC, kC, kC, kC, a->tok, a->winoff,
                                   a->order, a->n_windows, a->n_heads, a->head_scale, a->max_tokens, dqkv, dqkv + kC,
                                   dqkv + 2 * kC, 3 * kC, 3 * kC, 3 * kC, a->cos_r, stream);
  else
    rc = sst_sra_attn_bwd_ord_bf16(qk, qk + kC, a->v, a->o, a->d_o, a->lse, 2 * kC, 2 * kC, kC, kC, kC, a->tok, a->winoff,
                                   a->order, a->n_windows, a->n_heads, a->scale, a->max_tokens, dqkv, dqkv + kC, dqkv + 2 * kC,
                                   3 * kC, 3 * kC, 3 * kC, stream);
  if (rc) return rc;
  rc = sst_tall_linear_bf16(dqkv, 3 * kC, a->wqk_t, nullptr, m, 2 * kC, kC, kEpiBias, nullptr, nullptr, 0, a->dxp, kC, stream);
  if (rc) return rc;
  rc = sst_tall_linear_bf16(dqkv + 2 * kC, 3 * kC, a->wv_t, nullptr, m, kC, kC, kEpiAdd, a->ds1, nullptr, kC, a->dx, kC, stream);
  if (rc) return rc;
  sst_wgrad_problem_bf16 g[5];
  for (auto& q : g) {
    q.m = m;
    q.ldb = kC;
    q.bias_side = 1;
    q.transpose_out = 0;
    q.reserved = 0;
  }
  g[0].a = dqkv, g[0].lda = 3 * kC, g[0].b = a->xp, g[0].out_w = a->dw_in, g[0].out_b = a->db_in, g[0].p = 2 * kC;
  g[1].a = dqkv + 2 * kC, g[1].lda = 3 * kC, g[1].b = a->x, g[1].out_w = a->dw_in + 2 * kC * kC, g[1].out_b = a->db_in + 2 * kC;
  g[1].p = kC;
  g[2].a = a->ds1, g[2].lda = kC, g[2].b = a->o, g[2].out_w = a->dwo, g[2].out_b = a->dbo, g[2].p = kC;
  g[3].a = a->dpre, g[3].lda = kFF, g[3].b = a->y1, g[3].out_w = a->dw1, g[3].out_b = a->db1, g[3].p = kFF;
  g[4].a = a->h, g[4].lda = kFF, g[4].b = a->ds2, g[4].out_w = a->dw2, g[4].out_b = a->db2, g[4].p = kFF;
  g[4].bias_side = 2, g[4].transpose_out = 1;
  return sst_internal_wgrad_group_bf16(g, 5, ws_wg, riders, 2, stream);
}

}
```

sst_amd/csrc/layer_tail_x6.hip:

```cpp
#include <math.h>
#include <stdlib.h>
#include "common.h"
#include "gelu.h"
#include "mfma_tile.h"

#ifndef SST_NT_OUT
#define SST_NT_OUT false
#endif
#ifndef SST_NT_BWD
#define SST_NT_BWD true
#endif

namespace {

struct img3 {
  u32x4 p0, p1, p2;
};
__device__ __forceinline__ img3 split8(const f32x4& a, const f32x4& b) {
  img3 r;
  split8(a, b, r.p0, r.p1, r.p2);
  return r;
}
__device__ __forceinline__ void join8(const img3& v, f32x4& a, f32x4& b) {
#pragma unroll
// ... 35 lines not shown
__device__ __forceinline__ void stage_load(const tail_weights W, int chunk, int t, float (&r)[16]) {
  if (!BWD) {
    if (chunk < 2) {
#pragma unroll
      for (int u = 0; u < 2; ++u) {
        const int idx = t + 512 * u, n = idx >> 3, k8 = (idx & 7) * 8;
        const float* p = W.wo + n * kC + 64 * chunk + k8;
        const f32x4 a = *(const f32x4*)p, b = *(const f32x4*)(p + 4);
#pragma unroll
        for (int e = 0; e < 4; ++e) r[8 * u + e] = a[e], r[8 * u + 4 + e] = b[e];
      }
    } else {
      const int j = chunk - 2;
      {
        const float* p = W.w1 + (size_t)(kHC * j + (t >> 4)) * kC + (t & 15) * 8;
        const f32x4 a = *(const f32x4*)p, b = *(const f32x4*)(p + 4);
#pragma unroll
        for (int e = 0; e < 4; ++e) r[e] = a[e], r[4 + e] = b[e];
      }
      {
        const float* p = W.w2 + (size_t)(t >> 2) * kFF + kHC * j + (t & 3) * 8;
        const f32x4 a = *(const f32x4*)p, b = *(const f32x4*)(p + 4);
#pragma unroll
        for (int e = 0; e < 4; ++e) r[8 + e] = a[e], r[12 + e] = b[e];
      }
    }
  } else {
    if (chunk >= kNF) {
      const int q = chunk - kNF;
#pragma unroll
      for (int u = 0; u < 2; ++u) {
        const int idx = t + 512 * u, jn = idx & 127, k8 = (idx >> 7) * 8;
        const float* p = W.wo + (size_t)(64 * q + k8) * kC + jn;
#pragma unroll
        for (int e = 0; e < 8; ++e) r[8 * u + e] = p[e * kC];
      }
    } else {
      const int j = chunk;
      {
        const float* p = W.w2 + (size_t)((t >> 5) * 8) * kFF + kHC * j + (t & 31);
#pragma unroll
        for (int e = 0; e < 8; ++e) r[e] = p[e * kFF];
      }
      {
        const float* p = W.w1 + (size_t)(kHC * j + (t >> 7) * 8) * kC + (t & 127);
#pragma unroll
        for (int e = 0; e < 8; ++e) r[8 + e] = p[e * kC];
      }
    }
  }
}

__device__ __forceinline__ void store_images(unsigned char* base, int image_bytes, int off, const float* v) {
  const f32x4 a = {v[0], v[1], v[2], v[3]}, b = {v[4], v[5], v[6], v[7]};
  const img3 s = split8(a, b);
  *(u32x4*)(base + off) = s.p0;
  *(u32x4*)(base + image_bytes + off) = s.p1;
  *(u32x4*)(base + 2 * image_bytes + off) = s.p2;
}

template <bool BWD>
__device__ __forceinline__ void stage_store(unsigned char* slot, int chunk, int t, const float (&r)[16]) {
  const bool outproj = BWD ? chunk >= kNF : chunk < 2;
  if (outproj) {
#pragma unroll
    for (int u = 0; u < 2; ++u) {
      const int idx = t + 512 * u;
      const int n = BWD ? (idx & 127) : (idx >> 3), k8 = BWD ? (idx >> 7) * 8 : (idx & 7) * 8;
      store_images(slot, kIA, frag_off(w_lds_row(n), k8, 2), r + 8 * u);
    }
  } else {
    const int n1 = BWD ? (t & 31) : (t >> 4), k1 = BWD ? (t >> 5) * 8 : (t & 15) * 8;
    store_images(slot, kI1, frag_off(w_lds_row(n1), k1, 4), r);
    const int n2 = BWD ? (t & 127) : (t >> 2), k2 = BWD ? (t >> 7) * 8 : (t & 3) * 8;
    store_images(slot + kPart1, kI2, frag_off(w_lds_row(n2), k2, 1), r + 8);
  }
}

constexpr int kPackMany = 16;
struct pack_batch {
  tail_weights w[kPackMany];
  unsigned char* dst[kPackMany];
};
__global__ __launch_bounds__(512) void encoder_tail_pack_k(const pack_batch B) {
  extern __shared__ __attribute__((aligned(16))) unsigned char lds[];
  const int layer = blockIdx.x / (2 * kNChunks), blk = blockIdx.x % (2 * kNChunks);
  const tail_weights W = B.w[layer];
  const int chunk = blk % kNChunks, dir = blk / kNChunks;
  float r[16];
  if (dir == 0) {
    stage_load<false>(W, chunk, threadIdx.x, r);
    stage_store<false>(lds, chunk, threadIdx.x, r);
  } else {
    stage_load<true>(W, chunk, threadIdx.x, r);
    stage_store<true>(lds, chunk, threadIdx.x, r);
  }
  __syncthreads();
  unsigned char* dst = B.dst[layer] + (size_t)blk * kSlot;
  for (int i = threadIdx.x; i < kSlot / 16; i += 512) *(u32x4*)(dst + 16 * i) = *(const u32x4*)(lds + 16 * i);
}

__device__ __forceinline__ void barrier_lds_only() { asm volatile("s_waitcnt lgkmcnt(0)\n\ts_barrier" ::: "memory"); }

struct tile_io {
  unsigned char* scr;
  int frag_off0;
  int row_off[2];
  int64_t rrow[2];
  bool rvalid[2];
  int rcol;
};
__device__ __forceinline__ tile_io make_tile_io(unsigned char* scr, int lane, int64_t r0, int64_t m) {
  tile_io t;
  const int c = lane & 15, g = lane >> 4;
  t.scr = scr;
  t.frag_off0 = c * 128 + (((2 * g) ^ (c & 7)) << 4);
#pragma unroll
  for (int i = 0; i < 2; ++i) {
    const int r = 8 * i + (lane >> 3), p = lane & 7;
    t.row_off[i] = r * 128 + ((p ^ (r & 7)) << 4);
    t.rvalid[i] = r0 + r < m;
    t.rrow[i] = t.rvalid[i] ? r0 + r : m - 1;
  }
  t.rcol = (lane & 7) * 4;
  return t;
}
template <bool STREAM>
__device__ __forceinline__ void store32(const tile_io& t, float* __restrict__ base, int64_t ld, int col0, const f32x4& v0,
                                        const f32x4& v1) {
  *(f32x4*)(t.scr + t.frag_off0) = v0;
  *(f32x4*)(t.scr + (t.frag_off0 ^ 16)) = v1;
#pragma unroll
  for (int i = 0; i < 2; ++i) {
    const f32x4 w = *(const f32x4*)(t.scr + t.row_off[i]);
    if (t.rvalid[i]) {
      if (STREAM)
        __builtin_nontemporal_store(w, (f32x4*)(base + t.rrow[i] * ld + col0 + t.rcol));
      else
        *(f32x4*)(base + t.rrow[i] * ld + col0 + t.rcol) = w;
    }
  }
}
__device__ __forceinline__ void load32_issue(const tile_io& t, const float* __restrict__ base, int64_t ld, int col0, f32x4 (&w)[2]) {
#pragma unroll
  for (int i = 0; i < 2; ++i) w[i] = *(const f32x4*)(base + t.rrow[i] * ld + col0 + t.rcol);
}
__device__ __forceinline__ void load32_finish(const tile_io& t, const f32x4 (&w)[2], f32x4& v0, f32x4& v1) {
#pragma unroll
  for (int i = 0; i < 2; ++i) *(f32x4*)(t.scr + t.row_off[i]) = w[i];
  v0 = *(const f32x4*)(t.scr + t.frag_off0);
  v1 = *(const f32x4*)(t.scr + (t.frag_off0 ^ 16));
}

template <int HALF>
__device__ __forceinline__ void mma_half(const unsigned char* slot, int lane_off, const f32x4 (&x)[4][2], f32x4 (&acc)[8]) {
#pragma unroll
  for (int s2 = 0; s2 < 2; ++s2) {
    const img3 xs = split8(x[2 * HALF + s2][0], x[2 * HALF + s2][1]);
#pragma unroll
    for (int t0 = 0; t0 < 8; t0 += 4) {
      u32x4 a0[4], a1[4], a2[4];
#pragma unroll
      for (int u = 0; u < 4; ++u) {
        const int off = lane_off + ((t0 + u) * 2 + s2) * kFrag;
        a0[u] = *(const u32x4*)(slot + off);
        a1[u] = *(const u32x4*)(slot + kIA + off);
        a2[u] = *(const u32x4*)(slot + 2 * kIA + off);
      }
#pragma unroll
      for (int u = 0; u < 4; ++u) acc[t0 + u] = mma32(a0[u], xs.p2, acc[t0 + u]);
#pragma unroll
      for (int u = 0; u < 4; ++u) acc[t0 + u] = mma32(a2[u], xs.p0, acc[t0 + u]);
#pragma unroll
      for (int u = 0; u < 4; ++u) acc[t0 + u] = mma32(a1[u], xs.p1, acc[t0 + u]);
#pragma unroll
      for (int u = 0; u < 4; ++u) acc[t0 + u] = mma32(a0[u], xs.p1, acc[t0 + u]);
#pragma unroll
      for (int u = 0; u < 4; ++u) acc[t0 + u] = mma32(a1[u], xs.p0, acc[t0 + u]);
#pragma unroll
      for (int u = 0; u < 4; ++u) acc[t0 + u] = mma32(a0[u], xs.p0, acc[t0 + u]);
    }
  }
}

__device__ __forceinline__ f32x4 add4(const f32x4& a, const f32x4& b) {
  return (f32x4){a[0] + b[0], a[1] + b[1], a[2] + b[2], a[3] + b[3]};
}

__device__ __forceinline__ void mma_first(const unsigned char* slot, int lane_off1, const img3 (&y)[4], f32x4& out0, f32x4& out1) {
  const f32x4 z = {0.f, 0.f, 0.f, 0.f};
  f32x4 am[2] = {z, z}, ca[2] = {z, z}, cb[2] = {z, z};
#pragma unroll
  for (int s = 0; s < 4; ++s) {
    u32x4 a0[2], a1[2], a2[2];
#pragma unroll
    for (int T = 0; T < 2; ++T) {
      const int off = lane_off1 + (T * 4 + s) * kFrag;
      a0[T] = *(const u32x4*)(slot + off);
      a1[T] = *(const u32x4*)(slot + kI1 + off);
      a2[T] = *(const u32x4*)(slot + 2 * kI1 + off);
    }
#pragma unroll
    for (int T = 0; T < 2; ++T) ca[T] = mma32(a0[T], y[s].p2, ca[T]);
#pragma unroll
    for (int T = 0; T < 2; ++T) cb[T] = mma32(a0[T], y[s].p1, cb[T]);
#pragma unroll
    for (int T = 0; T < 2; ++T) ca[T] = mma32(a2[T], y[s].p0, ca[T]);
#pragma unroll
    for (int T = 0; T < 2; ++T) am[T] = mma32(a0[T], y[s].p0, am[T]);
#pragma unroll
    for (int T = 0; T < 2; ++T) ca[T] = mma32(a1[T], y[s].p1, ca[T]);
#pragma unroll
    for (int T = 0; T < 2; ++T) cb[T] = mma32(a1[T], y[s].p0, cb[T]);
  }
  out0 = add4(am[0], add4(cb[0], ca[0]));
  out1 = add4(am[1], add4(cb[1], ca[1]));
}

__device__ __forceinline__ void mma_second(const unsigned char* slot2, int lane_off2, const img3& h, f32x4 (&acc)[8]) {
#pragma unroll
  for (int t0 = 0; t0 < 8; t0 += 4) {
    u32x4 a0[4], a1[4], a2[4];
#pragma unroll
    for (int u = 0; u < 4; ++u) {
      const int off = lane_off2 + (t0 + u) * kFrag;
      a0[u] = *(const u32x4*)(slot2 + off);
      a1[u] = *(const u32x4*)(slot2 + kI2 + off);
      a2[u] = *(const u32x4*)(slot2 + 2 * kI2 + off);
    }
#pragma unroll
    for (int u = 0; u < 4; ++u) acc[t0 + u] = mma32(a0[u], h.p2, acc[t0 + u]);
#pragma unroll
    for (int u = 0; u < 4; ++u) acc[t0 + u] = mma32(a2[u], h.p0, acc[t0 + u]);
#pragma unroll
    for (int u = 0; u < 4; ++u) acc[t0 + u] = mma32(a1[u], h.p1, acc[t0 + u]);
#pragma unroll
    for (int u = 0; u < 4; ++u) acc[t0 + u] = mma32(a0[u], h.p1, acc[t0 + u]);
#pragma unroll
    for (int u = 0; u < 4; ++u) acc[t0 + u] = mma32(a1[u], h.p0, acc[t0 + u]);
#pragma unroll
    for (int u = 0; u < 4; ++u) acc[t0 + u] = mma32(a0[u], h.p0, acc[t0 + u]);
  }
}

__device__ __forceinline__ void ln_stats(f32x4 (&v)[4][2], float eps, float& mean, float& rstd) {
  float sum = 0.f;
#pragma unroll
  for (int s = 0; s < 4; ++s)
#pragma unroll
    for (int r = 0; r < 4; ++r) sum += v[s][0][r] + v[s][1][r];
  sum += __shfl_xor(sum, 16, 64);
  sum += __shfl_xor(sum, 32, 64);
  mean = sum * (1.f / 128.f);
  float sq = 0.f;
#pragma unroll
  for (int s = 0; s < 4; ++s)
#pragma unroll
    for (int h = 0; h < 2; ++h)
#pragma unroll
      for (int r = 0; r < 4; ++r) {
        v[s][h][r] -= mean;
        sq = fmaf(v[s][h][r], v[s][h][r], sq);
      }
  sq += __shfl_xor(sq, 16, 64);
  sq += __shfl_xor(sq, 32, 64);
  rstd = rsqrtf(sq * (1.f / 128.f) + eps);
}

struct tail_fwd_params {
  const float *o, *x;
  const unsigned char* packed;
  const float *b_out, *b1, *b2, *n1w, *n1b, *n2w, *n2b;
  float eps;
  int64_t m;
  float *s1, *st1, *y1, *pre, *h, *s2, *st2, *y2;
  const float* pos_table;
  const int32_t* pos_idx;
  float* y2p;
};

template <int ACT>
__global__ __launch_bounds__(kNTH, 2) void encoder_tail_fwd_x6_k(const tail_fwd_params P) {
  extern __shared__ __attribute__((aligned(16))) unsigned char lds[];
  float* par = (float*)(lds + kArea);
  const int lane = threadIdx.x & 63, g = lane >> 4, c = lane & 15, wave = threadIdx.x >> 6;
  const int64_t r0 = (int64_t)blockIdx.x * kRowsPerWg + wave * 16;
  const bool valid = r0 + c < P.m;
  const int64_t row = valid ? r0 + c : P.m - 1;
  const tile_io io = make_tile_io(lds + kArea + kParF * 4 + wave * kScr, lane, r0, P.m);
  const unsigned char* packed = P.packed;
  unsigned char* const part2 = lds + kPart1;
  dma_pieces<kWaves>(packed, lds, 3 * kIA / 1024, wave, lane);
  f32x4 ob[4][2], xr[4][2];
  {
    f32x4 wo[4][2], wx[4][2];
#pragma unroll
    for (int s = 0; s < 4; ++s) load32_issue(io, P.o, kC, 32 * s, wo[s]);
#pragma unroll
    for (int s = 0; s < 4; ++s) load32_issue(io, P.x, kC, 32 * s, wx[s]);
#pragma unroll
    for (int s = 0; s < 4; ++s) load32_finish(io, wo[s], ob[s][0], ob[s][1]);
#pragma unroll
    for (int s = 0; s < 4; ++s) load32_finish(io, wx[s], xr[s][0], xr[s][1]);
  }
  for (int i = threadIdx.x; i < kC; i += kNTH) {
    par[i] = P.b_out ? P.b_out[i] : 0.f;
    par[kC + i] = P.n1w[i];
    par[2 * kC + i] = P.n1b[i];
    par[3 * kC + i] = P.b2 ? P.b2[i] : 0.f;
    par[4 * kC + i] = P.n2w[i];
    par[5 * kC + i] = P.n2b[i];
  }
  for (int i = threadIdx.x; i < kFF; i += kNTH) par[6 * kC + i] = P.b1 ? P.b1[i] : 0.f;

  const int lane_offA = lane * 16, lane_off1 = lane * 16, lane_off2 = lane * 16;
  const f32x4 z4 = {0.f, 0.f, 0.f, 0.f};
  f32x4 acc[8];
#pragma unroll
  for (int T = 0; T < 8; ++T) acc[T] = z4;
  img3 yi[4];

  barrier_drain();
  mma_half<0>(lds, lane_offA, ob, acc);
  barrier_drain();
  dma_pieces<kWaves>(packed + kSlot, lds, 3 * kIA / 1024, wave, lane);
  barrier_drain();
  mma_half<1>(lds, lane_offA, ob, acc);
  barrier_drain();
  dma_pieces<kWaves>(packed + 2 * kSlot, lds, kSlot / 1024, wave, lane);
  {
    f32x4 v[4][2];
#pragma unroll
    for (int s = 0; s < 4; ++s) {
      const int n0 = 32 * s + 8 * g;
      v[s][0] = acc[2 * s] + *(const f32x4*)(par + n0) + xr[s][0];
      v[s][1] = acc[2 * s + 1] + *(const f32x4*)(par + n0 + 4) + xr[s][1];
      if (P.s1 != nullptr) store32<true>(io, P.s1, kC, 32 * s, v[s][0], v[s][1]);
    }
    float mean, rstd;
    ln_stats(v, P.eps, mean, rstd);
    if (valid && g == 0) ((float2*)P.st1)[row] = make_float2(mean, rstd);
#pragma unroll
    for (int s = 0; s < 4; ++s) {
      const int n0 = 32 * s + 8 * g;
      const f32x4 y0 = v[s][0] * rstd * *(const f32x4*)(par + kC + n0) + *(const f32x4*)(par + 2 * kC + n0);
      const f32x4 y1 = v[s][1] * rstd * *(const f32x4*)(par + kC + n0 + 4) + *(const f32x4*)(par + 2 * kC + n0 + 4);
      store32<true>(io, P.y1, kC, 32 * s, y0, y1);
      yi[s] = split8(y0, y1);
    }
#pragma unroll
    for (int T = 0; T < 8; ++T) acc[T] = z4;
  }
  barrier_drain();
  f32x4 sp0 = z4, sp1 = z4, sh0 = z4, sh1 = z4;
#pragma unroll 1
  for (int j = 0; j < kNF; ++j) {
    if (j > 0) {
      store32<true>(io, P.pre, kFF, kHC * (j - 1), sp0, sp1);
      store32<true>(io, P.h, kFF, kHC * (j - 1), sh0, sh1);
    }
    f32x4 p0, p1;
    mma_first(lds, lane_off1, yi, p0, p1);
    const int nl = kHC * j + 8 * g;
    p0 = add4(p0, *(const f32x4*)(par + 6 * kC + nl));
    p1 = add4(p1, *(const f32x4*)(par + 6 * kC + nl + 4));
    f32x4 h0, h1;
#pragma unroll
    for (int r = 0; r < 4; ++r) {
      h0[r] = ACT == 1 ? gelu_f(p0[r]) : fmaxf(p0[r], 0.f);
      h1[r] = ACT == 1 ? gelu_f(p1[r]) : fmaxf(p1[r], 0.f);
    }
    const img3 hs = split8(h0, h1);
    barrier_drain();
    if (j + 1 < kNF) dma_pieces<kWaves>(packed + (size_t)(j + 3) * kSlot, lds, kPart1 / 1024, wave, lane);
    mma_second(part2, lane_off2, hs, acc);
    sp0 = p0, sp1 = p1, sh0 = h0, sh1 = h1;
    barrier_drain();
    if (j + 1 < kNF) dma_pieces<kWaves>(packed + (size_t)(j + 3) * kSlot + kPart1, part2, kPart2 / 1024, wave, lane);
  }
  store32<true>(io, P.pre, kFF, kHC * (kNF - 1), sp0, sp1);
  store32<true>(io, P.h, kFF, kHC * (kNF - 1), sh0, sh1);
  f32x4 v[4][2];
#pragma unroll
  for (int s = 0; s < 4; ++s) {
    const int n0 = 32 * s + 8 * g;
    f32x4 ya, yb;
    join8(yi[s], ya, yb);
    v[s][0] = acc[2 * s] + *(const f32x4*)(par + 3 * kC + n0) + ya;
    v[s][1] = acc[2 * s + 1] + *(const f32x4*)(par + 3 * kC + n0 + 4) + yb;
    if (P.s2 != nullptr) store32<true>(io, P.s2, kC, 32 * s, v[s][0], v[s][1]);
  }
  float mean, rstd;
  ln_stats(v, P.eps, mean, rstd);
  if (valid && g == 0) ((float2*)P.st2)[row] = make_float2(mean, rstd);
  const float* prow = P.pos_table != nullptr ? P.pos_table + (size_t)P.pos_idx[row] * kC : nullptr;
#pragma unroll
  for (int s = 0; s < 4; ++s) {
    const int n0 = 32 * s + 8 * g;
    const f32x4 y0 = v[s][0] * rstd * *(const f32x4*)(par + 4 * kC + n0) + *(const f32x4*)(par + 5 * kC + n0);
    const f32x4 y1 = v[s][1] * rstd * *(const f32x4*)(par + 4 * kC + n0 + 4) + *(const f32x4*)(par + 5 * kC + n0 + 4);
    store32<SST_NT_OUT>(io, P.y2, kC, 32 * s, y0, y1);
    if (prow != nullptr) store32<SST_NT_OUT>(io, P.y2p, kC, 32 * s, y0 + *(const f32x4*)(prow + n0), y1 + *(const f32x4*)(prow + n0 + 4));
  }
}

struct tail_bwd_params {
  const float *dy2, *dy2p, *s2, *st2, *n2w, *pre, *s1, *st1, *n1w;
  const unsigned char* packed;
  int64_t m;
  float *ds2, *dpre, *ds1, *d_o;
  float *part2, *part1;
};

__device__ __forceinline__ void ln_bwd(f32x4 (&d)[4][2], f32x4 (&sv)[4][2], const float2 st, const float* gamma, int g, int c,
                                       bool valid, float* red) {
  float sg = 0.f, sgx = 0.f;
#pragma unroll
  for (int s = 0; s < 4; ++s)
#pragma unroll
    for (int h = 0; h < 2; ++h) {
      const f32x4 w = *(const f32x4*)(gamma + 32 * s + 8 * g + 4 * h);
      sv[s][h] = (sv[s][h] - st.x) * st.y;
      f32x4 a, b;
#pragma unroll
      for (int r = 0; r < 4; ++r) {
        a[r] = row_sum16(valid ? d[s][h][r] * sv[s][h][r] : 0.f);
        b[r] = row_sum16(valid ? d[s][h][r] : 0.f);
      }
      if (c == 0) {
        *(f32x4*)(red + 32 * s + 8 * g + 4 * h) = a;
        *(f32x4*)(red + kC + 32 * s + 8 * g + 4 * h) = b;
      }
      d[s][h] *= w;
#pragma unroll
      for (int r = 0; r < 4; ++r) {
        sg += d[s][h][r];
        sgx = fmaf(d[s][h][r], sv[s][h][r], sgx);
      }
    }
  sg += __shfl_xor(sg, 16, 64);
  sg += __shfl_xor(sg, 32, 64);
  sgx += __shfl_xor(sgx, 16, 64);
  sgx += __shfl_xor(sgx, 32, 64);
  const float mg = sg * (1.f / 128.f), mgx = sgx * (1.f / 128.f);
#pragma unroll
  for (int s = 0; s < 4; ++s)
#pragma unroll
    for (int h = 0; h < 2; ++h)
#pragma unroll
      for (int r = 0; r < 4; ++r) d[s][h][r] = st.y * (d[s][h][r] - mg - sv[s][h][r] * mgx);
}

template <int ACT>
__global__ __launch_bounds__(kNTH, 2) void encoder_tail_bwd_x6_k(const tail_bwd_params P) {
  extern __shared__ __attribute__((aligned(16))) unsigned char lds[];
  float* par = (float*)(lds + kArea);
  float* red = par + 2 * kC;
  const int lane = threadIdx.x & 63, g = lane >> 4, c = lane & 15, wave = threadIdx.x >> 6;
  const int64_t r0 = (int64_t)blockIdx.x * kRowsPerWg + wave * 16;
  const bool valid = r0 + c < P.m;
  const int64_t row = valid ? r0 + c : P.m - 1;
  const tile_io io = make_tile_io(lds + kArea + 2 * kC * 4 + kWaves * 2 * kC * 4 + wave * kScr, lane, r0, P.m);
  const unsigned char* packed = P.packed;
  unsigned char* const part2 = lds + kPart1;
  dma_pieces<kWaves>(packed, lds, kSlot / 1024, wave, lane);
  f32x4 d[4][2], sv[4][2];
  {
    f32x4 wd[4][2], we[4][2];
#pragma unroll
    for (int s = 0; s < 4; ++s) load32_issue(io, P.dy2, kC, 32 * s, wd[s]);
    if (P.dy2p != nullptr) {
#pragma unroll
      for (int s = 0; s < 4; ++s) load32_issue(io, P.dy2p, kC, 32 * s, we[s]);
#pragma unroll
      for (int s = 0; s < 4; ++s) {
        wd[s][0] += we[s][0];
        wd[s][1] += we[s][1];
      }
    }
#pragma unroll
    for (int s = 0; s < 4; ++s) load32_issue(io, P.s2, kC, 32 * s, we[s]);
#pragma unroll
    for (int s = 0; s < 4; ++s) load32_finish(io, wd[s], d[s][0], d[s][1]);
#pragma unroll
    for (int s = 0; s < 4; ++s) load32_finish(io, we[s], sv[s][0], sv[s][1]);
  }
  const float2 st2 = ((const float2*)P.st2)[row];
  for (int i = threadIdx.x; i < kC; i += kNTH) {
    par[i] = P.n2w[i];
    par[kC + i] = P.n1w[i];
  }
  barrier_drain();

  img3 di[4];
  {
    ln_bwd(d, sv, st2, par, g, c, valid, red + wave * 2 * kC);
#pragma unroll
    for (int s = 0; s < 4; ++s) {
      store32<SST_NT_BWD>(io, P.ds2, kC, 32 * s, d[s][0], d[s][1]);
      di[s] = split8(d[s][0], d[s][1]);
    }
  }
  const int lane_offA = lane * 16, lane_off1 = lane * 16, lane_off2 = lane * 16;
  const f32x4 z4 = {0.f, 0.f, 0.f, 0.f};
  f32x4 acc[8];
#pragma unroll
  for (int T = 0; T < 8; ++T) acc[T] = z4;
  f32x4 xs1[4][2];
  f32x4 pq[2];
  load32_issue(io, P.pre, kFF, 0, pq);

  f32x4 sd0 = z4, sd1 = z4;
  auto ffn_chunk = [&](int j, const f32x4 q0, const f32x4 q1) __attribute__((always_inline)) {
    if (j > 0) store32<SST_NT_BWD>(io, P.dpre, kFF, kHC * (j - 1), sd0, sd1);
    f32x4 p0, p1;
    mma_first(lds, lane_off1, di, p0, p1);
#pragma unroll
    for (int r = 0; r < 4; ++r) {
      p0[r] *= ACT == 1 ? gelu_grad_f(q0[r]) : (q0[r] > 0.f ? 1.f : 0.f);
      p1[r] *= ACT == 1 ? gelu_grad_f(q1[r]) : (q1[r] > 0.f ? 1.f : 0.f);
    }
    const img3 hs = split8(p0, p1);
    barrier_drain();
    if (j + 1 < kNF) dma_pieces<kWaves>(packed + (size_t)(j + 1) * kSlot, lds, kPart1 / 1024, wave, lane);
    mma_second(part2, lane_off2, hs, acc);
    sd0 = p0, sd1 = p1;
    barrier_drain();
    if (j + 1 < kNF)
      dma_pieces<kWaves>(packed + (size_t)(j + 1) * kSlot + kPart1, part2, kPart2 / 1024, wave, lane);
    else
      dma_pieces<kWaves>(packed + (size_t)kNF * kSlot, lds, 3 * kIA / 1024, wave, lane);
  };
  barrier_drain();
  if (threadIdx.x < 2 * kC) {
    float a = 0.f;
#pragma unroll
    for (int w = 0; w < kWaves; ++w) a += red[w * 2 * kC + threadIdx.x];
    P.part2[(int64_t)blockIdx.x * 2 * kC + threadIdx.x] = a;
  }
#pragma unroll 1
  for (int j = 0; j < kNF - 1; ++j) {
    f32x4 q0, q1;
    load32_finish(io, pq, q0, q1);
    load32_issue(io, P.pre, kFF, kHC * (j + 1), pq);
    ffn_chunk(j, q0, q1);
  }
  {
    f32x4 q0, q1;
    load32_finish(io, pq, q0, q1);
    ffn_chunk(kNF - 1, q0, q1);
    store32<SST_NT_BWD>(io, P.dpre, kFF, kHC * (kNF - 1), sd0, sd1);
    {
      f32x4 ws[4][2];
#pragma unroll
      for (int s = 0; s < 4; ++s) load32_issue(io, P.s1, kC, 32 * s, ws[s]);
#pragma unroll
      for (int s = 0; s < 4; ++s) load32_finish(io, ws[s], xs1[s][0], xs1[s][1]);
    }
    f32x4 dd[4][2];
#pragma unroll
    for (int s = 0; s < 4; ++s) {
      f32x4 ya, yb;
      join8(di[s], ya, yb);
      dd[s][0] = acc[2 * s] + ya;
      dd[s][1] = acc[2 * s + 1] + yb;
    }
    const float2 st1 = ((const float2*)P.st1)[row];
    barrier_drain();
    ln_bwd(dd, xs1, st1, par + kC, g, c, valid, red + wave * 2 * kC);
#pragma unroll
    for (int s = 0; s < 4; ++s) {
      store32<SST_NT_BWD>(io, P.ds1, kC, 32 * s, dd[s][0], dd[s][1]);
      xs1[s][0] = dd[s][0];
      xs1[s][1] = dd[s][1];
    }
#pragma unroll
    for (int T = 0; T < 8; ++T) acc[T] = z4;
    barrier_drain();
    mma_half<0>(lds, lane_offA, xs1, acc);
    barrier_drain();
    dma_pieces<kWaves>(packed + (size_t)(kNF + 1) * kSlot, lds, 3 * kIA / 1024, wave, lane);
    barrier_drain();
    mma_half<1>(lds, lane_offA, xs1, acc);
  }
#pragma unroll
  for (int s = 0; s < 4; ++s) store32<SST_NT_OUT>(io, P.d_o, kC, 32 * s, acc[2 * s], acc[2 * s + 1]);
  barrier_drain();
  if (threadIdx.x < 2 * kC) {
    float b = 0.f;
#pragma unroll
    for (int w = 0; w < kWaves; ++w) b += red[w * 2 * kC + threadIdx.x];
    P.part1[(int64_t)blockIdx.x * 2 * kC + threadIdx.x] = b;
  }
}

bool aligned16(const void* p) { return ((uintptr_t)p & 15) == 0; }

template <typename K>
int configure(K kernel, int lds_bytes, unsigned long long* mask) {
  if (sst_first_use_on_device(mask)) {
    SST_HIP(hipFuncSetAttribute((const void*)kernel, hipFuncAttributeMaxDynamicSharedMemorySize, lds_bytes));
    sst_mark_device(mask);
  }
  return SST_OK;
}

}

int sst_internal_encoder_tail_bwd_f32x6(const sst_encoder_tail_bwd_args* a, float** part2, float** part1, int* partial_rows,
                                        void* stream) {
  if (!a || a->m <= 0 || (a->act != 1 && a->act != 2)) return SST_ERR_ARG;
  const void* need[] = {a->dy2, a->s2, a->st2, a->n2w, a->pre, a->s1, a->st1, a->n1w, a->packed,
                        a->ds2, a->dpre, a->ds1, a->d_o, a->workspace};
  for (const void* p : need)
    if (!p || !aligned16(p)) return SST_ERR_ARG;
  if (a->dy2p && !aligned16(a->dy2p)) return SST_ERR_ARG;
  const int64_t rows = sst_div_up(a->m, (int64_t)kRowsPerWg);
  if (rows > 0x7fffffff / 2) return SST_ERR_UNSUPPORTED;
  tail_bwd_params P;
  P.dy2 = a->dy2, P.dy2p = a->dy2p, P.s2 = a->s2, P.st2 = a->st2, P.n2w = a->n2w, P.pre = a->pre, P.s1 = a->s1, P.st1 = a->st1;
  P.n1w = a->n1w, P.packed = (const unsigned char*)a->packed + kPackDir, P.m = a->m;
  P.ds2 = a->ds2, P.dpre = a->dpre, P.ds1 = a->ds1, P.d_o = a->d_o;
  P.part2 = (float*)a->workspace;
  P.part1 = P.part2 + rows * 2 * kC;
  hipStream_t st = (hipStream_t)stream;
  static unsigned long long cfg1 = 0, cfg2 = 0;
  if (a->act == 1) {
    const int rc = configure(encoder_tail_bwd_x6_k<1>, kLdsBwd, &cfg1);
    if (rc) return rc;
    hipLaunchKernelGGL(encoder_tail_bwd_x6_k<1>, dim3((unsigned)rows), dim3(kNTH), kLdsBwd, st, P);
  } else {
    const int rc = configure(encoder_tail_bwd_x6_k<2>, kLdsBwd, &cfg2);
    if (rc) return rc;
    hipLaunchKernelGGL(encoder_tail_bwd_x6_k<2>, dim3((unsigned)rows), dim3(kNTH), kLdsBwd, st, P);
  }
  SST_LAUNCH_CHECK();
  *part2 = P.part2, *part1 = P.part1, *partial_rows = (int)rows;
  return SST_OK;
}

namespace {
__global__ __launch_bounds__(1024) void tail_colsum_k(const float* __restrict__ partials, int nb, int width, float* __restrict__ out0,
                                                      float* __restrict__ out1, int split) {
  __shared__ float red[32][33];
  const int cx = threadIdx.x & 31, gy = threadIdx.x >> 5;
  const int i = blockIdx.x * 32 + cx;
  float acc = 0.f;
  if (i < width)
    for (int b = gy; b < nb; b += 32) acc += partials[(int64_t)b * width + i];
  red[gy][cx] = acc;
  __syncthreads();
  if (gy == 0 && i < width) {
    float t = 0.f;
#pragma unroll
    for (int k = 0; k < 32; ++k) t += red[k][cx];
    if (i < split)
      out0[i] = t;
    else
      out1[i - split] = t;
  }
}
}

extern "C" {

int64_t sst_encoder_tail_pack_bytes(void) { return 2 * (int64_t)kPackDir; }

int sst_encoder_tail_pack_f32x6_many(const float* const* d_w_out, const float* const* d_w1, const float* const* d_w2,
                                     void* const* d_packed, int n, void* stream) {
  if (n < 0 || (n > 0 && (!d_w_out || !d_w1 || !d_w2 || !d_packed))) return SST_ERR_ARG;
  static unsigned long long cfg = 0;
  const int rc = configure(encoder_tail_pack_k, kSlot, &cfg);
  if (rc) return rc;
  for (int base = 0; base < n; base += kPackMany) {
    pack_batch B;
    const int cnt = n - base < kPackMany ? n - base : kPackMany;
    for (int i = 0; i < cnt; ++i) {
      const float *wo = d_w_out[base + i], *w1 = d_w1[base + i], *w2 = d_w2[base + i];
      void* dst = d_packed[base + i];
      if (!wo || !w1 || !w2 || !dst || !aligned16(wo) || !aligned16(w1) || !aligned16(w2) || !aligned16(dst)) return SST_ERR_ARG;
      B.w[i].wo = wo, B.w[i].w1 = w1, B.w[i].w2 = w2;
      B.dst[i] = (unsigned char*)dst;
    }
    hipLaunchKernelGGL(encoder_tail_pack_k, dim3(cnt * 2 * kNChunks), dim3(512), kSlot, (hipStream_t)stream, B);
  }
  SST_LAUNCH_CHECK();
  return SST_OK;
}

int sst_encoder_tail_pack_f32x6(const float* d_w_out, const float* d_w1, const float* d_w2, void* d_packed, void* stream) {
  return sst_encoder_tail_pack_f32x6_many(&d_w_out, &d_w1, &d_w2, &d_packed, 1, stream);
}

int64_t sst_encoder_tail_bwd_workspace_bytes(int64_t m) {
  if (m < 0) return SST_ERR_ARG;
  return sst_align_up(2 * sst_div_up(m > 0 ? m : 1, (int64_t)kRowsPerWg) * 2 * kC * (int64_t)sizeof(float), 256);
}

int sst_encoder_tail_fwd_f32x6(const sst_encoder_tail_fwd_args* a, void* stream) {
  if (!a || a->m < 0 || (a->act != 1 && a->act != 2)) return SST_ERR_ARG;
  if (a->m == 0) return SST_OK;
  const void* need[] = {a->o, a->x, a->packed, a->n1w, a->n1b, a->n2w, a->n2b, a->st1, a->y1, a->pre, a->h, a->st2, a->y2};
  for (const void* p : need)
    if (!p || !aligned16(p)) return SST_ERR_ARG;
  if ((a->s1 && !aligned16(a->s1)) || (a->s2 && !aligned16(a->s2))) return SST_ERR_ARG;
  if ((a->pos_table != nullptr) != (a->pos_idx != nullptr) || (a->pos_table != nullptr) != (a->y2p != nullptr)) return SST_ERR_ARG;
  if (a->pos_table && (!aligned16(a->pos_table) || !aligned16(a->y2p))) return SST_ERR_ARG;
  tail_fwd_params P;
  P.o = a->o, P.x = a->x, P.packed = (const unsigned char*)a->packed;
  P.b_out = a->b_out, P.b1 = a->b1, P.b2 = a->b2, P.n1w = a->n1w, P.n1b = a->n1b, P.n2w = a->n2w, P.n2b = a->n2b;
  P.eps = a->eps, P.m = a->m;
  P.s1 = a->s1, P.st1 = a->st1, P.y1 = a->y1, P.pre = a->pre, P.h = a->h, P.s2 = a->s2, P.st2 = a->st2, P.y2 = a->y2;
  P.pos_table = a->pos_table, P.pos_idx = a->pos_idx, P.y2p = a->y2p;
  const int64_t rows = sst_div_up(a->m, (int64_t)kRowsPerWg);
  if (rows > 0x7fffffff) return SST_ERR_UNSUPPORTED;
  hipStream_t st = (hipStream_t)stream;
  static unsigned long long cfg1 = 0, cfg2 = 0;
  if (a->act == 1) {
    const int rc = configure(encoder_tail_fwd_x6_k<1>, kLdsFwd, &cfg1);
    if (rc) return rc;
    hipLaunchKernelGGL(encoder_tail_fwd_x6_k<1>, dim3((unsigned)rows), dim3(kNTH), kLdsFwd, st, P);
  } else {
    const int rc = configure(encoder_tail_fwd_x6_k<2>, kLdsFwd, &cfg2);
    if (rc) return rc;
    hipLaunchKernelGGL(encoder_tail_fwd_x6_k<2>, dim3((unsigned)rows), dim3(kNTH), kLdsFwd, st, P);
  }
  SST_LAUNCH_CHECK();
  return SST_OK;
}

int sst_encoder_tail_bwd_f32x6(const sst_encoder_tail_bwd_args* a, void* stream) {
  if (!a || a->m < 0) return SST_ERR_ARG;
  if (!a->dn2w || !a->dn2b || !a->dn1w || !a->dn1b) return SST_ERR_ARG;
  hipStream_t st = (hipStream_t)stream;
  if (a->m == 0) {
    for (float* p : {a->dn2w, a->dn2b, a->dn1w, a->dn1b}) SST_HIP(hipMemsetAsync(p, 0, sizeof(float) * kC, st));
    return SST_OK;
  }
  float *part2 = nullptr, *part1 = nullptr;
  int rows = 0;
  const int rc = sst_internal_encoder_tail_bwd_f32x6(a, &part2, &part1, &rows, stream);
  if (rc) return rc;
  hipLaunchKernelGGL(tail_colsum_k, dim3(2 * kC / 32), dim3(1024), 0, st, part2, rows, 2 * kC, a->dn2w, a->dn2b, kC);
  hipLaunchKernelGGL(tail_colsum_k, dim3(2 * kC / 32), dim3(1024), 0, st, part1, rows, 2 * kC, a->dn1w, a->dn1b, kC);
  SST_LAUNCH_CHECK();
  return SST_OK;
}

}
```

sst_amd/dense.py:

```python
import torch
from torch.autograd import Function

from . import _lib


def colsum(x):
    m, c = x.shape
    if x.dtype != torch.float32 or (c % 4) != 0 or c > 1024 or x.stride(1) != 1 or not x.is_cuda:
        return x.sum(0)
    out = torch.empty(c, dtype=torch.float32, device=x.device)
    lib = _lib.load()
    ws = _lib.workspace(lib.sst_colsum_workspace_bytes(m, c), x.device)
    rc = lib.sst_colsum_f32(_lib.ptr(x), m, c, x.stride(0), _lib.ptr(out), _lib.ptr(ws), _lib.stream_ptr())
    _lib.check(rc, 'sst_colsum_f32')
    return out


def weight_grad_splitk(dy, x, chunk=1024):
    m = dy.size(0)
    s = m // chunk
    if s < 4:
        return dy.t() @ x
    body = s * chunk
    dw = torch.bmm(dy[:body].view(s, chunk, -1).transpose(1, 2), x[:body].view(s, chunk, -1)).sum(0)
# ... 219 lines not shown
    return pre, h


def dgrad_gelu(dy, w2, pre):
    m, k = dy.shape
    n = w2.size(1)
    if w2.size(0) != k or not _gelu_gemm_ok(dy, w2, n, k) or pre.shape != (m, n) or not pre.is_contiguous():
        return None
    out = torch.empty((m, n), dtype=torch.float32, device=dy.device)
    lib = _lib.load()
    for j in range(0, n, 128):
        rc = lib.sst_tall_linear_gelu_f32(_lib.ptr(dy), dy.stride(0), _lib.ptr(w2[:, j:]), w2.stride(0), None, m, 128,
                                          k, 1, 1, _lib.ptr(pre[:, j:]), _lib.ptr(out[:, j:]), n, _lib.stream_ptr())
        _lib.check(rc, 'sst_tall_linear_gelu_f32')
    return out


class TallLinear(Function):

    @staticmethod
    def forward(ctx, x, weight, bias):
        ctx.save_for_backward(x, weight)
        ctx.has_bias = bias is not None
        if bias is not None:
            return torch.addmm(bias, x, weight.t())
        return x @ weight.t()

    @staticmethod
    def backward(ctx, dy):
        x, weight = ctx.saved_tensors
        dy = dy.contiguous()
        dx = dw = db = None
        if ctx.needs_input_grad[0]:
            dx = dy @ weight
        want_b = ctx.has_bias and ctx.needs_input_grad[2]
        if ctx.needs_input_grad[1]:
            dw, db = weight_bias_grad(dy, x, want_b)
        elif want_b:
            db = colsum(dy)
        return dx, dw, db


def tall_linear(x, weight, bias=None):
    if x.dim() != 2 or x.dtype != torch.float32 or not x.is_cuda:
        return torch.nn.functional.linear(x, weight, bias)
    return TallLinear.apply(x, weight, bias)


_LN_ACTS = {None: 0, 'gelu': 1, 'relu': 2}


def add_ln_fwd(x, res, weight, bias, eps, save_sum=True, act=None, pos=None):
    x = x.contiguous()
    m, c = x.shape
    if res is not None:
        res = res.contiguous()
    y = torch.empty_like(x)
    s = (torch.empty_like(x) if save_sum else None) if res is not None else x
    stats = torch.empty((m, 2), dtype=torch.float32, device=x.device)
    if pos is not None:
        assert act is None
        yp = torch.empty_like(x)
        rc = _lib.load().sst_add_layernorm_pos_fwd_f32(_lib.ptr(x), _lib.ptr(res), _lib.ptr(weight), _lib.ptr(bias), m, c, float(eps),
                                                       _lib.ptr(y), _lib.ptr(s) if (res is not None and save_sum) else None,
                                                       _lib.ptr(stats), _lib.ptr(pos[0]), _lib.ptr(pos[1]), _lib.ptr(yp),
                                                       _lib.stream_ptr())
        _lib.check(rc, 'sst_add_layernorm_pos_fwd_f32')
        return y, s, stats, yp
    rc = _lib.load().sst_add_layernorm_act_fwd_f32(_lib.ptr(x), _lib.ptr(res), _lib.ptr(weight), _lib.ptr(bias), m, c,
                                                   float(eps), _LN_ACTS[act], _lib.ptr(y),
                                                   _lib.ptr(s) if (res is not None and save_sum) else None,
                                                   _lib.ptr(stats), _lib.stream_ptr())
    _lib.check(rc, 'sst_add_layernorm_act_fwd_f32')
    return y, s, stats


def add_ln_act_bwd(dy, s, stats, weight, bias, act):
    dy = dy.contiguous()
    m, c = s.shape
    dx = torch.empty_like(s)
    dw = torch.empty(c, dtype=torch.float32, device=s.device)
    db = torch.empty(c, dtype=torch.float32, device=s.device)
    lib = _lib.load()
    ws = _lib.workspace(lib.sst_add_layernorm_bwd_workspace_bytes(m, c), s.device)
    rc = lib.sst_add_layernorm_act_bwd_f32(_lib.ptr(dy), _lib.ptr(s), _lib.ptr(stats), _lib.ptr(weight), _lib.ptr(bias),
                                           _LN_ACTS[act], m, c, _lib.ptr(dx), _lib.ptr(dw), _lib.ptr(db), _lib.ptr(ws),
                                           _lib.stream_ptr())
    _lib.check(rc, 'sst_add_layernorm_act_bwd_f32')
    return dx, dw, db


def add_ln_bwd(dy, s, stats, weight, dy2=None):
    dy = dy.contiguous()
    m, c = s.shape
    dx = torch.empty_like(s)
    dw = torch.empty(c, dtype=torch.float32, device=s.device)
    db = torch.empty(c, dtype=torch.float32, device=s.device)
    lib = _lib.load()
    ws = _lib.workspace(lib.sst_add_layernorm_bwd_workspace_bytes(m, c), s.device)
    if dy2 is not None and c != 128:
        dy, dy2 = dy + dy2, None
    rc = lib.sst_add_layernorm_bwd2_f32(_lib.ptr(dy), _lib.ptr(dy2.contiguous() if dy2 is not None else None), _lib.ptr(s),
                                        _lib.ptr(stats), _lib.ptr(weight), m, c, _lib.ptr(dx), _lib.ptr(dw), _lib.ptr(db),
                                        _lib.ptr(ws), _lib.stream_ptr())
    _lib.check(rc, 'sst_add_layernorm_bwd2_f32')
    return dx, dw, db


def lds_linear_add_ln_ok(x, w, res, c):
    return (c == 128 and lds_linear_ok(x, w) and w.size(0) == 128 and res.is_cuda and res.dtype == torch.float32
            and res.shape == (x.size(0), 128) and res.is_contiguous() and res.data_ptr() % 16 == 0)


def lds_linear_add_ln(x, w, bias, res, ln_weight, ln_bias, eps, save_sum=True, pos=None):
    m, k = x.shape
    y = torch.empty((m, 128), dtype=torch.float32, device=x.device)
    s = torch.empty((m, 128), dtype=torch.float32, device=x.device) if save_sum else None
    stats = torch.empty((m, 2), dtype=torch.float32, device=x.device)
    yp = torch.empty((m, 128), dtype=torch.float32, device=x.device) if pos is not None else None
    lib = _lib.load()
    if _MATMUL_MODE == 'f32x6' and k != 128:
        s = lds_linear(x, w, bias, EPI_ADD, aux_in=res)
        out = add_ln_fwd(s, None, ln_weight, ln_bias, eps, pos=pos)
        return out[0], s, out[2], (out[3] if pos is not None else None)
    entry = getattr(lib, 'sst_tall_linear_ln_' + _MATMUL_MODE)
    rc = entry(
        _lib.ptr(x), x.stride(0), _lib.ptr(w), w.stride(0), _lib.ptr(bias), m, k, _lib.ptr(res), 128, _lib.ptr(ln_weight),
        _lib.ptr(ln_bias), float(eps), _lib.ptr(y), _lib.ptr(s), _lib.ptr(stats),
        _lib.ptr(pos[0]) if pos is not None else None, _lib.ptr(pos[1]) if pos is not None else None, _lib.ptr(yp),
        _lib.stream_ptr())
    _lib.check(rc, 'sst_tall_linear_ln_' + _MATMUL_MODE)
    return y, s, stats, yp


def encoder_tail_ok(o, x, w_out, w1, w2):
    if _MATMUL_MODE != 'f32x6':
        return False
    if not (o.shape == x.shape and x.dim() == 2 and x.size(1) == 128 and w_out.shape == (128, 128) and w1.shape == (256, 128)
            and w2.shape == (128, 256)):
        return False
    return all(t.is_cuda and t.dtype == torch.float32 and t.is_contiguous() and t.data_ptr() % 16 == 0
               for t in (o, x, w_out, w1, w2))


def encoder_tail_pack(w_out, w1, w2, out=None):
    lib = _lib.load()
    if out is None:
        out = torch.empty(int(lib.sst_encoder_tail_pack_bytes()), dtype=torch.uint8, device=w_out.device)
    _lib.check(lib.sst_encoder_tail_pack_f32x6(_lib.ptr(w_out), _lib.ptr(w1), _lib.ptr(w2), _lib.ptr(out), _lib.stream_ptr()),
               'sst_encoder_tail_pack_f32x6')
    return out


def encoder_tail_fwd(o, x, packed, b_out, b1, b2, n1w, n1b, n2w, n2b, eps, act, save=True, pos=None, out=None):
    m = x.size(0)
    dev = x.device
    out = dict(out) if out else {}

    def e(name, cols):
        if name not in out or out[name] is None:
            out[name] = torch.empty((m, cols), dtype=torch.float32, device=dev)
        return out[name]
    s1 = e('s1', 128) if save else None
    out['s1'] = s1
    st1, y1, pre, h, s2, st2, y2 = e('st1', 2), e('y1', 128), e('pre', 256), e('h', 256), e('s2', 128), e('st2', 2), e('y2', 128)
    y2p = e('y2p', 128) if pos is not None else None
    out['y2p'] = y2p
    P = lambda t: None if t is None else t.data_ptr()
    args = _lib.EncoderTailFwdArgs(
        m, 1 if act == 'gelu' else 2, 0, float(eps), 0.0, P(o), P(x), P(packed), P(b_out), P(b1), P(b2), P(n1w), P(n1b),
        P(n2w), P(n2b), P(pos[0]) if pos is not None else None, P(pos[1]) if pos is not None else None,
        P(s1), P(st1), P(y1), P(pre), P(h), P(s2), P(st2), P(y2), P(y2p))
    import ctypes
    _lib.check(_lib.load().sst_encoder_tail_fwd_f32x6(ctypes.byref(args), _lib.stream_ptr()), 'sst_encoder_tail_fwd_f32x6')
    return out


def encoder_tail_bwd(dy2, dy2p, s2, st2, pre, s1, st1, packed, n1w, n2w, act, out=None):
    m = dy2.size(0)
    dev = dy2.device
    out = out or {}

    def e(name, cols):
        return out[name] if name in out else torch.empty((m, cols), dtype=torch.float32, device=dev)
    ds2, dpre, ds1, d_o = e('ds2', 128), e('dpre', 256), e('ds1', 128), e('d_o', 128)
    dn = out['dn'] if 'dn' in out else torch.empty((4, 128), dtype=torch.float32, device=dev)
    lib = _lib.load()
    ws = out['ws'] if 'ws' in out else _lib.workspace(lib.sst_encoder_tail_bwd_workspace_bytes(m), dev)
    P = lambda t: None if t is None else t.data_ptr()
    d0 = dn.data_ptr()
    args = _lib.EncoderTailBwdArgs(m, 1 if act == 'gelu' else 2, 0, P(dy2), P(dy2p), P(s2), P(st2), P(pre), P(s1), P(st1), P(packed),
                                   P(n1w), P(n2w), P(ds2), P(dpre), P(ds1), P(d_o), d0, d0 + 512, d0 + 1024, d0 + 1536, P(ws))
    import ctypes
    _lib.check(lib.sst_encoder_tail_bwd_f32x6(ctypes.byref(args), _lib.stream_ptr()), 'sst_encoder_tail_bwd_f32x6')
    return ds2, dpre, ds1, d_o, dn


class AddLayerNorm(Function):

    @staticmethod
    def forward(ctx, x, res, weight, bias, eps, act=None):
        y, s, stats = add_ln_fwd(x, res, weight, bias, eps, act=act)
        ctx.save_for_backward(s, stats, weight, bias)
        ctx.has_res, ctx.act = res is not None, act
        return y

    @staticmethod
    def backward(ctx, dy):
        s, stats, weight, bias = ctx.saved_tensors
        if ctx.act is None:
            dx, dw, db = add_ln_bwd(dy, s, stats, weight)
        else:
            dx, dw, db = add_ln_act_bwd(dy, s, stats, weight, bias, ctx.act)
        return dx, (dx if ctx.has_res else None), dw, db, None, None


def _act_name(act):
    if act is None or isinstance(act, torch.nn.Identity):
        return None
    if isinstance(act, torch.nn.GELU) and getattr(act, 'approximate', 'none') == 'none':
        return 'gelu'
    if type(act) is torch.nn.ReLU:
        return 'relu'
    return False


def add_layer_norm(x, res, norm, act=None):
    c = x.size(-1)
    post = (lambda t: t) if act is None else act
    if not isinstance(norm, torch.nn.LayerNorm):
        return post(norm(x + res if res is not None else x))
    ok = (x.dim() == 2 and x.dtype == torch.float32 and x.is_cuda
          and norm.elementwise_affine and norm.bias is not None and 1 <= c <= 512 and len(norm.normalized_shape) == 1)
    if not ok:
        y = x + res if res is not None else x
        return post(torch.nn.functional.layer_norm(y, norm.normalized_shape, norm.weight, norm.bias, norm.eps))
    name = _act_name(act)
    if name is False:
        return act(AddLayerNorm.apply(x, res, norm.weight, norm.bias, norm.eps))
    return AddLayerNorm.apply(x, res, norm.weight, norm.bias, norm.eps, name)
```

sst_amd/sst_basic_block.py:

```python
import math

import torch
import torch.nn as nn
import torch.nn.functional as F
from torch.utils.checkpoint import checkpoint

from . import _lib
from . import kernels as K
from .sra_composed import sra_attention_composed
from .dense import (encoder_tail_ok, encoder_tail_pack, encoder_tail_fwd, encoder_tail_bwd, inproj_pos_ok, inproj_pos,
                    EPI_ADD, EPI_BIAS, EPI_GELU, EPI_MUL_GELU_GRAD, EPI_MUL_RELU_GRAD, EPI_RELU, lds_linear, lds_linear_ok,
                    lds_linear_add_ln, lds_linear_add_ln_ok, lds_linear_dqkv_ok, lds_linear_qkv, lds_linear_qkv_ok,
                    weight_bias_grad_group,
                    tall_gemm, add_layer_norm, add_ln_bwd, add_ln_fwd, dgrad_gelu, linear_gelu, tall_linear,
                    weight_bias_grad)
from .norm import build_norm_layer


class CosineMultiheadAttention(nn.MultiheadAttention):

    def __init__(self, embed_dim, num_heads, dropout=0.0, batch_first=False, tau_min=0.01, cosine=True,
                 non_shared_tau=False):
        super().__init__(embed_dim, num_heads, dropout=dropout)
        self.tau_min = tau_min
# ... 12 lines not shown
    for dl in info:
        if dl not in ind_dict:
            continue
        f2w, (flat_pos,) = ind_dict[dl][0].long(), ind_dict[dl][1]
        if f2w.numel() == 0:
            continue
        t = int(info[dl]['max_tokens'])
        tmax = max(tmax, t)
        w = torch.div(f2w, t, rounding_mode='floor')
        wkeys.append(w + wbase)
        inner.append(f2w - w * t)
        toks.append(flat_pos.long())
        wbase += int(w.max().item()) + 1
    wkeys, inner, toks = torch.cat(wkeys), torch.cat(inner), torch.cat(toks)
    order = torch.argsort(wkeys * tmax + inner)
    _, counts = torch.unique_consecutive(wkeys[order], return_counts=True)
    winoff = torch.zeros(counts.numel() + 1, dtype=torch.int32, device=device)
    winoff[1:] = torch.cumsum(counts, 0).to(torch.int32)
    return K.WindowPlan(toks[order].to(torch.int32).contiguous(), winoff, counts.numel(), num_voxels, tmax)


def flat_pos_from_reference_dict(pos_dict, ind_dict, num_voxels):
    from .sst_ops import window2flat_v2
    if pos_dict is None or any(v is None for v in pos_dict.values()):
        return None
    return window2flat_v2(pos_dict, ind_dict)


class WindowAttention(nn.Module):

    def __init__(self, d_model, nhead, dropout, batch_first=False, layer_id=None, layer_cfg=dict()):
        super().__init__()
        self.nhead = nhead
        self.d_model = d_model
        if d_model % nhead != 0:
            raise ValueError('embed_dim must be divisible by num_heads')
        self.head_dim = d_model // nhead
        self.cosine = layer_cfg.get('cosine', False)
        if self.cosine:
            tau_min = layer_cfg.get('tau_min', 0.01)
            self.self_attn = CosineMultiheadAttention(
                d_model, nhead, dropout=dropout, batch_first=False, tau_min=tau_min, cosine=True,
                non_shared_tau=layer_cfg.get('non_shared_tau', False))
        elif layer_cfg.get('linear', False):
            raise NotImplementedError
        else:
            self.self_attn = nn.MultiheadAttention(d_model, nhead, dropout=dropout)
        self.attn_dropout = dropout
        self.exe_counter = 0
        self.layer_id = layer_id
        self.impl = 0

    def head_scale(self):
        if not self.cosine:
            return None
        attn = self.self_attn
        return (1.0 / attn.tau.float().clamp(min=attn.tau_min)).reshape(-1).expand(self.nhead).contiguous()

    def forward(self, feat_2d, pos_dict, ind_dict, key_padding_dict=None):
        composed = self.head_dim != 16 or (self.attn_dropout > 0 and self.training)
        if isinstance(ind_dict, K.WindowPlan):
            plan, pos = ind_dict, pos_dict
        else:
            plan = plan_from_reference_dicts(ind_dict, feat_2d.size(0), feat_2d.device)
            pos = flat_pos_from_reference_dict(pos_dict, ind_dict, feat_2d.size(0)) if isinstance(pos_dict, dict) \
                else pos_dict
        attn = self.self_attn
        c = self.d_model
        x = feat_2d.float()
        w, b = attn.in_proj_weight, attn.in_proj_bias
        xp = x + pos if pos is not None else x
        qk = tall_linear(xp, w[:2 * c], b[:2 * c])
        v = tall_linear(x, w[2 * c:], b[2 * c:])
        if self.cosine and not composed and K.cosine_kernels_ok(plan, self.nhead, self.impl) and qk.is_cuda:
            o = K.sra_cosine_attention_qk_v(qk, v, self.head_scale(), plan, self.nhead)
        elif self.cosine:
            h = self.nhead
            q = F.normalize(qk[:, :c].reshape(-1, h, self.head_dim), dim=2)
            k = F.normalize(qk[:, c:].reshape(-1, h, self.head_dim), dim=2)
            tau = attn.tau.clamp(min=attn.tau_min).reshape(1, -1, 1)
            q = (q / tau).reshape(-1, c)
            if composed:
                o = sra_attention_composed(q, k.reshape(-1, c), v, plan, h, 1.0, self.attn_dropout, self.training)
            else:
                o = K.sra_attention(q, k.reshape(-1, c), v, plan, h, scale=1.0, impl=self.impl)
        elif composed:
            o = sra_attention_composed(qk[:, :c], qk[:, c:], v, plan, self.nhead, 1.0 / math.sqrt(self.head_dim),
                                       self.attn_dropout, self.training)
        else:
            o = K.sra_attention_qk_v(qk, v, plan, self.nhead, scale=1.0 / math.sqrt(16.0), impl=self.impl)
        return tall_linear(o, attn.out_proj.weight, attn.out_proj.bias)


import os as _os
_TALL_GEMM = int(_os.environ.get('SST_AMD_TALL_GEMM', '1'))
_FUSED_GELU = int(_os.environ.get('SST_AMD_FUSED_GELU', '0'))
_LDS_LINEAR = int(_os.environ.get('SST_AMD_LDS_LINEAR', '1'))


def _linear_fwd(x, w, b):
    if _LDS_LINEAR and lds_linear_ok(x, w):
        return lds_linear(x, w, b)
    if _TALL_GEMM and w.size(0) == 128 and (w.size(1) == 128 or _TALL_GEMM > 1):
        y = tall_gemm(x, w, b)
        if y is not None:
            return y
    return torch.addmm(b, x, w.t())


def _linear_dgrad(dy, w, out=None, add=None):
    if _LDS_LINEAR and lds_linear_ok(dy, w, trans_w=True):
        if out is not None:
            return lds_linear(dy, w, None, EPI_ADD, trans_w=True, aux_in=out if add is None else add, out=out)
        return lds_linear(dy, w, None, trans_w=True)
    if out is not None and add is not None:
        out.copy_(add)
    if _TALL_GEMM and w.size(1) == 128 and (w.size(0) == 128 or _TALL_GEMM > 1):
        y = tall_gemm(dy, w, None, trans_w=True, out=out, accumulate=out is not None)
        if y is not None:
            return y
    if out is not None:
        return out.addmm_(dy, w)
    return dy @ w


_LAYER_EXEC = int(_os.environ.get('SST_AMD_LAYER_EXEC', '1'))
_POS_FOLD = int(_os.environ.get('SST_AMD_POS_FOLD', '1'))


def _layer_exec_ok(x, xp, plan, nhead, act, params):
    from . import dense
    if not (_LAYER_EXEC and _LDS_LINEAR and dense.matmul_mode() == 'f32x6' and act in ('gelu', 'relu') and nhead == 8):
        return False
    w_in, b_in, w_out, b_out, w1, b1, w2, b2, n1w, n1b, n2w, n2b = params
    if any(p is None for p in params):
        return False
    m = x.size(0)
    shapes_ok = (x.shape == (m, 128) and (xp is None or xp.shape == (m, 128)) and w_in.shape == (384, 128) and w_out.shape == (128, 128)
                 and w1.shape == (256, 128) and w2.shape == (128, 256) and plan.n_tokens == m
                 and m >= 4096)
    if not shapes_ok:
        return False
    for t in (x,) + ((xp,) if xp is not None else ()) + tuple(params):
        if not (t.is_cuda and t.dtype == torch.float32 and t.is_contiguous() and t.data_ptr() % 16 == 0):
            return False
    from . import _lib
    return int(_lib.load().sst_encoder_layer_bwd_workspace_bytes(m, nhead)) >= 0


_SLAB = (('qkv', 384), ('o', 128), ('lse', 8), ('s1', 128), ('st1', 2), ('y1', 128), ('pre', 256), ('h', 256), ('s2', 128),
         ('st2', 2))


def _slab_offsets(m):
    off, out = 0, {}
    for name, cols in _SLAB:
        out[name] = off
        off += (m * cols * 4 + 255) // 256 * 256
    return out, off


def _layer_exec_fwd(x, xp, plan, nhead, impl, act, params, eps, scale, pos_next, need_bwd, head_scale=None, pos_spec=None,
                    wpack=None):
    from . import _lib
    import ctypes
    w_in, b_in, w_out, b_out, w1, b1, w2, b2, n1w, n1b, n2w, n2b = params
    m = x.size(0)
    dev = x.device
    offs, total = _slab_offsets(m)
    slab = torch.empty(total, dtype=torch.uint8, device=dev)
    base = slab.data_ptr()
    y2 = torch.empty((m, 128), dtype=torch.float32, device=dev)
    y2p = torch.empty((m, 128), dtype=torch.float32, device=dev) if pos_next is not None else None
    lib = _lib.load()
    packed = wpack is not None
    if not packed:
        wpack = torch.empty(int(lib.sst_encoder_layer_wpack_bytes()), dtype=torch.uint8, device=dev)
    order = plan.order
    P = lambda t: None if t is None else t.data_ptr()
    S = lambda name: base + offs[name]
    args = _lib.EncoderLayerFwdArgs(
        m, plan.n_windows, nhead, 1 if act == 'gelu' else 2, plan.max_tokens, impl, float(eps), float(scale),
        P(x), P(xp), P(w_in), P(b_in), None if packed else P(w_out), P(b_out), None if packed else P(w1), P(b1),
        None if packed else P(w2), P(b2), P(n1w), P(n1b), P(n2w), P(n2b),
        None if plan.tok_ptr(impl) is None else plan.tok.data_ptr(), P(plan.winoff), P(order),
        P(pos_next[0]) if pos_next is not None else None, P(pos_next[1]) if pos_next is not None else None,
        S('qkv'), S('o'), S('lse'), S('y1'), S('s1') if need_bwd else None, S('st1'), S('pre'), S('h'), S('s2'), P(y2), S('st2'),
        P(y2p), P(head_scale), P(wpack), P(pos_spec[0]) if pos_spec is not None else None,
        P(pos_spec[1]) if pos_spec is not None else None)
    rc = K._bracket('sra_fwd', plan.n_tokens, lambda: lib.sst_encoder_layer_fwd_f32x6(ctypes.byref(args), _lib.stream_ptr()))
    if rc == _lib.SST_ERR_UNSUPPORTED:
        return None
    _lib.check(rc, 'sst_encoder_layer_fwd_f32x6')
    return slab, y2, y2p, wpack


def _layer_exec_bwd(ctx, dy2, dy2p, saved):
    from . import _lib
    import ctypes
    x, xp, slab, w_in, w_out, w1, w2, n1w, n2w, wpack = saved[:10]
    rest = list(saved[10:])
    pos_spec = (rest.pop(0), rest.pop(0)) if ctx.pos_fold else None
    if ctx.pos_fold:
        xp = None
    head_scale = rest.pop(0) if rest else None
    m = x.size(0)
    dev = x.device
    plan, nhead, impl = ctx.plan, ctx.nhead, ctx.impl
    offs, _ = _slab_offsets(m)
    base = slab.data_ptr()

    def e(*shape):
        return torch.empty(shape, dtype=torch.float32, device=dev)
    dy2 = dy2.contiguous()
    dy2p = dy2p.contiguous() if dy2p is not None else None
    ds1 = e(m, 128)
    scratch = e(m, 128 + 256 + 128 + 384)
    sb = scratch.data_ptr()
    p_ds2, p_dpre, p_do, p_dqkv = sb, sb + 4 * m * 128, sb + 4 * m * 384, sb + 4 * m * 512
    dw_in, db_in, dwo, dbo = e(384, 128), e(384), e(128, 128), e(128)
    dw1, db1, dw2, db2 = e(256, 128), e(256), e(128, 256), e(128)
    dn = e(4, 128)
    cos_r = e(m, nhead) if head_scale is not None else None
    lib = _lib.load()
    nbytes = lib.sst_encoder_layer_bwd_workspace_bytes(m, nhead)
    if nbytes < 0:
        _lib.check(int(nbytes), 'sst_encoder_layer_bwd_workspace_bytes')
    ws = _lib.workspace(nbytes, dev)
    order = plan.order
    P = lambda t: None if t is None else t.data_ptr()
    S = lambda name: base + offs[name]
    dnp = dn.data_ptr()
    args = _lib.EncoderLayerBwdArgs(
        m, plan.n_windows, nhead, 1 if ctx.act == 'gelu' else 2, plan.max_tokens, impl, 0.0, float(ctx.scale),
        P(dy2), P(dy2p), P(x), P(xp), S('qkv'), S('o'), S('lse'), S('s1'), S('st1'), S('y1'), S('pre'), S('h'), S('s2'), S('st2'),
        P(w_in), P(w_out), P(w1), P(w2), P(n1w), P(n2w),
        None if plan.tok_ptr(impl) is None else plan.tok.data_ptr(), P(plan.winoff), P(order),
        p_ds2, p_dpre, P(ds1), p_do, p_dqkv,
        P(dw_in), P(db_in), P(dwo), P(dbo), P(dw1), P(db1), P(dw2), P(db2), dnp, dnp + 512, dnp + 1024, dnp + 1536, P(ws),
        P(head_scale), P(cos_r), None, P(wpack), P(pos_spec[0]) if pos_spec is not None else None,
        P(pos_spec[1]) if pos_spec is not None else None)
    rc = K._bracket('sra_bwd', plan.n_tokens, lambda: lib.sst_encoder_layer_bwd_f32x6(ctypes.byref(args), _lib.stream_ptr()))
    _lib.check(rc, 'sst_encoder_layer_bwd_f32x6')
    d_scale = K.head_scale_grad(cos_r, head_scale) if head_scale is not None else None
    return (ds1, None, None, None, None, None, dw_in, db_in, dwo, dbo, dw1, db1, dw2, db2, dn[0], dn[1], dn[2], dn[3], None, None,
            None, d_scale, None, None, None, None)


def _bn_rows_fwd(bn, s):
    from .norm import bn_prepare
    prep, batch_stats, count, sync = bn_prepare(bn, s)
    m, c = s.shape
    y = torch.empty((m, c), dtype=torch.float32, device=s.device)
    _lib.check(_lib.load().sst_bn_act_res_fwd_f32(_lib.ptr(s), m, c, s.stride(0), None, 0, _lib.ptr(prep[2]), _lib.ptr(prep[3]), 0,
                                                  _lib.ptr(y), y.stride(0), _lib.stream_ptr()), 'sst_bn_act_res_fwd_f32')
    return y, prep, (bool(batch_stats), float(count), bool(sync))


def _bn_rows_bwd(dy, s, prep, cfg):
    from torch import distributed as dist
    batch_stats, count, sync = cfg
    m, c = s.shape
    dy = dy.contiguous()
    lib = _lib.load()
    sums = torch.empty((2, c), dtype=torch.float32, device=s.device)
    ws = _lib.workspace(lib.sst_bn_workspace_bytes(m, c), s.device)
    _lib.check(lib.sst_bn_act_res_bwd_reduce_f32(_lib.ptr(dy), _lib.ptr(s), None, m, c, dy.stride(0), s.stride(0), 0, _lib.ptr(prep[0]),
                                                 _lib.ptr(prep[1]), _lib.ptr(prep[2]), _lib.ptr(prep[3]), 0, _lib.ptr(sums[0]),
                                                 _lib.ptr(sums[1]), _lib.ptr(ws), _lib.stream_ptr()), 'sst_bn_act_res_bwd_reduce_f32')
    total = sums
    if sync and batch_stats:
        total = sums.clone()
        dist.all_reduce(total, async_op=False)
    ds = torch.empty((m, c), dtype=torch.float32, device=s.device)
    _lib.check(lib.sst_bn_act_res_bwd_apply_f32(_lib.ptr(dy), _lib.ptr(s), None, m, c, dy.stride(0), s.stride(0), 0, _lib.ptr(prep[0]),
                                                _lib.ptr(prep[1]), _lib.ptr(prep[2]), _lib.ptr(prep[3]), _lib.ptr(total[0]),
                                                _lib.ptr(total[1]), (1.0 / count) if batch_stats else 0.0, 0, None, 0, _lib.ptr(ds),
                                                ds.stride(0), _lib.stream_ptr()), 'sst_bn_act_res_bwd_apply_f32')
    return ds, sums[1], sums[0]


def _bn_layer_ok(norm, c):
    return (isinstance(norm, nn.BatchNorm1d) and norm.weight is not None and norm.bias is not None and norm.num_features == c
            and c % 4 == 0 and c <= 1024)


class FusedEncoderLayerFn(torch.autograd.Function):

    @staticmethod
    def forward(ctx, x, pos, plan, nhead, impl, act, w_in, b_in, w_out, b_out, w1, b1, w2, b2, n1w, n1b, n2w, n2b, eps,
                xp=None, pos_next=None, head_scale=None, xp_shares_x=False, pos_spec=None, bn=None, wpack=None):
        c = x.size(1)
        x = x.contiguous()
        if head_scale is not None:
            head_scale = head_scale.contiguous()
        ctx.cosine = head_scale is not None
        from . import dense as _dense
        ctx.matmul = _dense.matmul_mode()
        ctx.set_materialize_grads(False)
        ctx.pos_fold = False
        if pos_spec is not None:
            assert xp is None and pos is None, 'pos_spec replaces pos / xp'
            if _LDS_LINEAR and inproj_pos_ok(x, pos_spec, w_in):
                ctx.pos_fold = True
            else:
                xp = K.add_table_rows(x, pos_spec[0], pos_spec[1])
                xp_shares_x = True
        ctx.split_input = xp is not None
        ctx.fold_xp = (xp is None) or bool(xp_shares_x)
        if xp is None and not ctx.pos_fold:
            xp = x + pos if pos is not None else x
        params = (w_in, b_in, w_out, b_out, w1, b1, w2, b2, n1w, n1b, n2w, n2b)
        ctx.exec = False
        ctx.bn = bn is not None
        if bn is None and c == 128 and ctx.fold_xp and _layer_exec_ok(x, xp, plan, nhead, act, params):
            need_bwd = any(ctx.needs_input_grad)
            scale = 1.0 / math.sqrt(16.0)
            done = _layer_exec_fwd(x, xp, plan, nhead, impl, act, params, eps, scale, pos_next, need_bwd, head_scale,
                                   pos_spec if ctx.pos_fold else None, wpack)
            if done is not None:
                slab, y2, y2p, wpack = done
                if need_bwd:
                    ctx.save_for_backward(x, xp if xp is not None else x, slab, w_in, w_out, w1, w2, n1w, n2w, wpack,
                                          *(pos_spec if ctx.pos_fold else ()), *((head_scale,) if ctx.cosine else ()))
                    ctx.plan, ctx.nhead, ctx.impl, ctx.act, ctx.scale = plan, nhead, impl, act, scale
                    ctx.exec = True
                ctx.two = pos_next is not None
                return (y2, y2p) if ctx.two else y2
        if ctx.pos_fold:
            qkv = inproj_pos(x, pos_spec, w_in, b_in)
            qk, v = qkv[:, :2 * c], qkv[:, 2 * c:]
            xp = x
        elif _LDS_LINEAR and c == 128 and lds_linear_qkv_ok(xp, x, w_in):
            qkv = lds_linear_qkv(xp, x, w_in, b_in)
            qk, v = qkv[:, :2 * c], qkv[:, 2 * c:]
        else:
            qk = _linear_fwd(xp, w_in[:2 * c], b_in[:2 * c])
            v = _linear_fwd(x, w_in[2 * c:], b_in[2 * c:])
        scale = 1.0 / math.sqrt(16.0)
        if ctx.cosine:
            res = K._sra_cos_fwd(qk[:, :c], qk[:, c:], v, plan, nhead, head_scale)
            if res is None:
                raise RuntimeError('sst_amd: cosine attention kernels refused a layout _can_fuse admitted')
            o, lse = res
        else:
            o, lse = K._sra_fwd(qk[:, :c], qk[:, c:], v, plan, nhead, scale, impl)
        need_bwd = any(ctx.needs_input_grad)
        ctx.tail = False
        if bn is not None:
            y1, s1, st1, pre, h, s2, st2, y2, y2p, ctx.bn_cfg = FusedEncoderLayerFn._tail_batch_norm(
                o, x, w_out, b_out, w1, b1, w2, b2, bn, act, pos_next)
        elif (_LDS_LINEAR and c == 128 and act in ('gelu', 'relu') and o.is_contiguous()
                and encoder_tail_ok(o, x, w_out, w1, w2) and all(t is not None for t in (b_out, b1, b2))):
            if wpack is None:
                wpack = encoder_tail_pack(w_out, w1, w2)
            t = encoder_tail_fwd(o, x, wpack, b_out, b1, b2, n1w, n1b, n2w, n2b, eps, act, save=need_bwd, pos=pos_next)
            s1, st1, y1, pre, h, s2, st2, y2, y2p = (t[k] for k in ('s1', 'st1', 'y1', 'pre', 'h', 's2', 'st2', 'y2', 'y2p'))
            ctx.tail = True
        else:
            y1, s1, st1, pre, h, s2, st2, y2, y2p = FusedEncoderLayerFn._tail_by_products(
                o, x, w_out, b_out, w1, b1, w2, b2, n1w, n1b, n2w, n2b, eps, act, need_bwd, pos_next, c)
        if need_bwd:
            ctx.save_for_backward(x, xp, qk, v, o, lse, s1, st1, y1, pre, h, s2, st2, w_in, w_out, w1, w2, n1w, n2w,
                                  *((wpack,) if ctx.tail else ()), *(pos_spec if ctx.pos_fold else ()),
                                  *((head_scale,) if ctx.cosine else ()))
            ctx.plan, ctx.nhead, ctx.impl, ctx.act, ctx.scale = plan, nhead, impl, act, scale
        ctx.two = pos_next is not None
        return (y2, y2p) if ctx.two else y2

    @staticmethod
    def _tail_batch_norm(o, x, w_out, b_out, w1, b1, w2, b2, bn, act, pos_next):
        if _LDS_LINEAR and lds_linear_ok(o, w_out) and x.is_contiguous():
            s1 = lds_linear(o, w_out, b_out, EPI_ADD, aux_in=x)
        else:
            s1 = torch.addmm(b_out, o, w_out.t()).add_(x)
        y1, prep1, cfg1 = _bn_rows_fwd(bn[0], s1)
        if _LDS_LINEAR and lds_linear_ok(y1, w1) and act in ('gelu', 'relu'):
            h, pre = lds_linear(y1, w1, b1, EPI_GELU if act == 'gelu' else EPI_RELU, want_pre=True)
        else:
            pre = torch.addmm(b1, y1, w1.t())
            h = F.gelu(pre) if act == 'gelu' else F.relu(pre)
        if _LDS_LINEAR and lds_linear_ok(h, w2):
            s2 = lds_linear(h, w2, b2, EPI_ADD, aux_in=y1)
        else:
            s2 = torch.addmm(b2, h, w2.t()).add_(y1)
        y2, prep2, cfg2 = _bn_rows_fwd(bn[1], s2)
        y2p = y2 + pos_next[0].index_select(0, pos_next[1].long()) if pos_next is not None else None
        return y1, s1, prep1, pre, h, s2, prep2, y2, y2p, (cfg1, cfg2)

    @staticmethod
    def _tail_by_products(o, x, w_out, b_out, w1, b1, w2, b2, n1w, n1b, n2w, n2b, eps, act, need_bwd, pos_next, c):
        fuse_ln = _LDS_LINEAR and lds_linear_add_ln_ok(o, w_out, x, c)
        if fuse_ln:
            y1, s1, st1, _ = lds_linear_add_ln(o, w_out, b_out, x, n1w, n1b, eps, save_sum=need_bwd)
        else:
            a = _linear_fwd(o, w_out, b_out)
            y1, s1, st1 = add_ln_fwd(x, a, n1w, n1b, eps, save_sum=need_bwd)
        fused_act = linear_gelu(y1, w1, b1) if (act == 'gelu' and _FUSED_GELU) else None
        if _LDS_LINEAR and lds_linear_ok(y1, w1):
            h, pre = lds_linear(y1, w1, b1, EPI_GELU if act == 'gelu' else EPI_RELU, want_pre=True)
        elif fused_act is not None:
            pre, h = fused_act
        else:
            pre = torch.addmm(b1, y1, w1.t())
            h = F.gelu(pre) if act == 'gelu' else F.relu(pre)
        y2p = None
        if fuse_ln and lds_linear_add_ln_ok(h, w2, y1, c):
            y2, s2, st2, y2p = lds_linear_add_ln(h, w2, b2, y1, n2w, n2b, eps, save_sum=need_bwd, pos=pos_next)
        elif _LDS_LINEAR and lds_linear_ok(h, w2):
            s2 = lds_linear(h, w2, b2, EPI_ADD, aux_in=y1)
            y2, _, st2 = add_ln_fwd(s2, None, n2w, n2b, eps)
        else:
            f = _linear_fwd(h, w2, b2)
            y2, s2, st2 = add_ln_fwd(y1, f, n2w, n2b, eps, save_sum=need_bwd)
        if pos_next is not None and y2p is None:
            y2p = y2 + pos_next[0].index_select(0, pos_next[1].long())
        return y1, s1, st1, pre, h, s2, st2, y2, y2p

    @staticmethod
    def backward(ctx, dy2, dy2p=None):
        from . import dense as _dense
        with _dense.matmul_mode_scope(ctx.matmul):
            return FusedEncoderLayerFn._backward(ctx, dy2, dy2p)

    @staticmethod
    def _backward(ctx, dy2, dy2p=None):
        if ctx.exec:
            if dy2 is None:
                dy2, dy2p = dy2p, None
            return _layer_exec_bwd(ctx, dy2, dy2p if ctx.two else None, ctx.saved_tensors)
        saved = ctx.saved_tensors
        x, xp, qk, v, o, lse, s1, st1, y1, pre, h, s2, st2, w_in, w_out, w1, w2, n1w, n2w = saved[:19]
        rest = list(saved[19:])
        wpack = rest.pop(0) if ctx.tail else None
        pos_spec = (rest.pop(0), rest.pop(0)) if ctx.pos_fold else None
        head_scale = rest.pop(0) if ctx.cosine else None
        c = x.size(1)
        if dy2 is None:
            dy2, dy2p = dy2p, None
        f32 = dict(dtype=torch.float32, device=x.device)
        dw2, db2 = torch.empty_like(w2), torch.empty(w2.size(0), **f32)
        dw1, db1 = torch.empty_like(w1), torch.empty(w1.size(0), **f32)
        if ctx.tail:
            ds2, dpre, ds1, do, dn = encoder_tail_bwd(dy2.contiguous(), dy2p.contiguous() if (ctx.two and dy2p is not None) else None,
                                                      s2, st2, pre, s1, st1, wpack, n1w, n2w, ctx.act)
            ds2_for_w2 = ds2
            dn2w, dn2b, dn1w, dn1b = dn[0], dn[1], dn[2], dn[3]
        else:
            if ctx.bn:
                if ctx.two and dy2p is not None:
                    dy2 = dy2 + dy2p
                ds2, dn2w, dn2b = _bn_rows_bwd(dy2, s2, st2, ctx.bn_cfg[1])
            else:
                ds2, dn2w, dn2b = add_ln_bwd(dy2, s2, st2, n2w, dy2=dy2p if ctx.two else None)
            ds2_for_w2 = ds2
            dpre = dgrad_gelu(ds2, w2, pre) if (ctx.act == 'gelu' and _FUSED_GELU) else None
            if _LDS_LINEAR and lds_linear_ok(ds2, w2, trans_w=True) and pre.is_contiguous():
                dpre = lds_linear(ds2, w2, None, EPI_MUL_GELU_GRAD if ctx.act == 'gelu' else EPI_MUL_RELU_GRAD, trans_w=True,
                                  aux_in=pre)
            if dpre is None:
                dh = ds2 @ w2
                if ctx.act == 'gelu':
                    dpre = torch.ops.aten.gelu_backward(dh, pre)
                else:
                    dpre = dh * (pre > 0).to(dh.dtype)
            dy1 = _linear_dgrad(dpre, w1, out=torch.empty_like(ds2), add=ds2)
            if ctx.bn:
                ds1, dn1w, dn1b = _bn_rows_bwd(dy1, s1, st1, ctx.bn_cfg[0])
            else:
                ds1, dn1w, dn1b = add_ln_bwd(dy1, s1, st1, n1w)
            do = _linear_dgrad(ds1, w_out)
        dqkv = torch.empty((x.size(0), 3 * c), dtype=torch.float32, device=x.device)
        dqk, dv = dqkv[:, :2 * c], dqkv[:, 2 * c:]
        d_scale = None
        if ctx.cosine:
            r = K._sra_cos_bwd(qk[:, :c], qk[:, c:], v, o, lse, do, ctx.plan, ctx.nhead, head_scale, dqkv[:, :c],
                               dqkv[:, c:2 * c], dv)
            d_scale = K.head_scale_grad(r, head_scale)
        else:
            K._sra_bwd(qk[:, :c], qk[:, c:], v, o, lse, do, ctx.plan, ctx.nhead, ctx.scale, ctx.impl, dqkv[:, :c],
                       dqkv[:, c:2 * c], dv)
        dw_in = torch.empty_like(w_in)
        db_in = torch.empty(3 * c, **f32)
        dwo, dbo = torch.empty_like(w_out), torch.empty(w_out.size(0), **f32)
        weight_bias_grad_group([(ds2_for_w2, h, dw2, db2), (dpre, y1, dw1, db1), (ds1, o, dwo, dbo),
                                (dqk, x, dw_in[:2 * c], db_in[:2 * c], pos_spec) if ctx.pos_fold else
                                (dqk, xp, dw_in[:2 * c], db_in[:2 * c]), (dv, x, dw_in[2 * c:], db_in[2 * c:])])
        dxp = None
        if ctx.fold_xp and _LDS_LINEAR and c == 128 and lds_linear_dqkv_ok(dqkv, w_in):
            dx = lds_linear(dqkv, w_in, None, EPI_ADD, trans_w=True, aux_in=ds1, out=ds1)
        elif ctx.split_input:
            dxp = _linear_dgrad(dqk, w_in[:2 * c])
            dx = _linear_dgrad(dv, w_in[2 * c:], out=ds1)
        elif _LDS_LINEAR and lds_linear_ok(dqk, w_in[:2 * c], trans_w=True) and lds_linear_ok(dv, w_in[2 * c:], trans_w=True):
            dx = _linear_dgrad(dv, w_in[2 * c:], out=_linear_dgrad(dqk, w_in[:2 * c], out=ds1))
        else:
            dx = ds1.addmm_(dqkv, w_in)
        return (dx, None, None, None, None, None, dw_in, db_in, dwo, dbo, dw1, db1, dw2, db2, dn1w, dn1b, dn2w, dn2b,
                None, dxp, None, d_scale, None, None, None, None)


class _StackHeadScales(torch.autograd.Function):

    @staticmethod
    def forward(ctx, nhead, tau_mins, *taus):
        flat = torch.cat([t.reshape(-1).expand(nhead) if t.numel() == 1 else t.reshape(-1) for t in taus]).view(len(taus), nhead)
        mins = K.const_tensor(tau_mins, flat.device).view(-1, 1)
        scales = 1.0 / torch.maximum(flat.float(), mins)
        ctx.save_for_backward(flat, scales, mins)
        ctx.shapes = [tuple(t.shape) for t in taus]
        return scales

    @staticmethod
    def backward(ctx, g):
        flat, scales, mins = ctx.saved_tensors
        d = torch.where(flat >= mins, -(g * scales * scales), torch.zeros((), dtype=g.dtype, device=g.device))
        per_layer_sum = None
        out = []
        for l, shape in enumerate(ctx.shapes):
            n = 1
            for v in shape:
                n *= v
            if n == 1:
                if per_layer_sum is None:
                    per_layer_sum = d.sum(1)
                out.append(per_layer_sum[l].reshape(shape))
            else:
                out.append(d[l].reshape(shape))
        return (None, None) + tuple(out)


def stack_head_scales(layers):
    cos = [(i, enc.win_attn) for i, enc in enumerate(layers) if enc.win_attn.cosine]
    out = [None] * len(layers)
    if not cos:
        return out
    heads = {wa.nhead for _, wa in cos}
    if len(heads) != 1:
        for i, wa in cos:
            out[i] = wa.head_scale()
        return out
    nhead = heads.pop()
    rows = _StackHeadScales.apply(nhead, tuple(float(wa.self_attn.tau_min) for _, wa in cos),
                                  *[wa.self_attn.tau for _, wa in cos]).unbind(0)
    for (i, _), row in zip(cos, rows):
        out[i] = row
    return out


def stack_tail_images(layers, like):
    import ctypes
    out = [None] * len(layers)
    take = []
    for i, enc in enumerate(layers):
        attn = enc.win_attn.self_attn
        wo, w1, w2 = attn.out_proj.weight, enc.linear1.weight, enc.linear2.weight
        if (enc.bn_modules() is None and wo.is_cuda and wo.shape == (128, 128) and w1.shape == (256, 128) and w2.shape == (128, 256)
                and all(w.dtype == torch.float32 and w.is_contiguous() and w.data_ptr() % 16 == 0 for w in (wo, w1, w2))
                and enc.act_name in ('gelu', 'relu') and all(b is not None for b in (attn.out_proj.bias, enc.linear1.bias,
                                                                                     enc.linear2.bias))):
            take.append((i, wo, w1, w2))
    if not take or not like.is_cuda:
        return out
    lib = _lib.load()
    nbytes = (int(lib.sst_encoder_tail_pack_bytes()) + 255) // 256 * 256
    buf = torch.empty(len(take) * nbytes, dtype=torch.uint8, device=like.device)
    n = len(take)
    P = ctypes.c_void_p * n
    d = [buf[j * nbytes:(j + 1) * nbytes] for j in range(n)]
    with torch.no_grad():
        _lib.check(lib.sst_encoder_tail_pack_f32x6_many(P(*[t[1].data_ptr() for t in take]), P(*[t[2].data_ptr() for t in take]),
                                                        P(*[t[3].data_ptr() for t in take]), P(*[v.data_ptr() for v in d]), n,
                                                        _lib.stream_ptr()), 'sst_encoder_tail_pack_f32x6_many')
    for (i, _, _, _), v in zip(take, d):
        out[i] = v
    return out


def run_encoder_stack_fp32(blocks, feats, plans, pos_specs, checkpoint_blocks=()):
    n_layers = 2 * len(blocks)

    scales = stack_head_scales([enc for block in blocks for enc in block.encoder_list])

    from . import dense as _dense
    mode = _dense.matmul_mode()
    fold = _POS_FOLD and mode == 'f32x6' and _LDS_LINEAR and all(inproj_pos_ok(feats.contiguous(), spec, blocks[0].encoder_list[0].win_attn.
                                                                 self_attn.in_proj_weight) for spec in pos_specs[:2])

    layers = [enc for block in blocks for enc in block.encoder_list]
    wpacks = stack_tail_images(layers, feats) if (mode == 'f32x6' and _LDS_LINEAR) else [None] * n_layers

    def layer(enc, li, x, xp):
        attn = enc.win_attn.self_attn
        if fold:
            out = FusedEncoderLayerFn.apply(
                x, None, plans[li % 2], enc.win_attn.nhead, enc.win_attn.impl, enc.act_name, attn.in_proj_weight,
                attn.in_proj_bias, attn.out_proj.weight, attn.out_proj.bias, enc.linear1.weight, enc.linear1.bias,
                enc.linear2.weight, enc.linear2.bias, enc.norm1.weight, enc.norm1.bias, enc.norm2.weight, enc.norm2.bias,
# ... 134 lines not shown
```

Before: 104.0.

## Hand over tail-saved activations in MFMA fragment layout and store activation gradient

Adds a handover mode where the fused encoder tail forward writes s1, pre and s2 straight from registers in the per-wave MFMA fragment layout, using non-temporal stores into row-padded buffers. The tail backward then loads them back directly into registers instead of staging through LDS scratch. In this mode the forward also stores the GELU/ReLU derivative in place of the pre-activation, so the backward skips recomputing erf. The mode is enabled by default for both the autograd tail path and the layer-exec path. In exchange, these saved buffers are no longer usable as plain row-major tensors and need padded allocations and a Python helper to convert them back.

```diff
diff --git a/include/sst_amd.h b/include/sst_amd.h
--- a/include/sst_amd.h
+++ b/include/sst_amd.h
@@ -338,6 +338,7 @@
   void* wpack;
   const float* xpos_table;
   const int32_t* xpos_idx;
+  int32_t tail_flags;
 } sst_encoder_layer_fwd_args;
 typedef struct sst_encoder_layer_bwd_args {
   int64_t m, n_windows;
@@ -356,15 +357,17 @@
   const void* wpack;
   const float* xpos_table;
   const int32_t* xpos_idx;
+  int32_t tail_flags;
 } sst_encoder_layer_bwd_args;
 int64_t sst_encoder_layer_bwd_workspace_bytes(int64_t m, int n_heads);
 int64_t sst_encoder_layer_wpack_bytes(void);
 int sst_encoder_layer_fwd_f32x6(const sst_encoder_layer_fwd_args* args, void* stream);
 int sst_encoder_layer_bwd_f32x6(const sst_encoder_layer_bwd_args* args, void* stream);
 
+#define SST_TAIL_HANDOVER 1
 typedef struct sst_encoder_tail_fwd_args {
   int64_t m;
-  int32_t act, reserved;
+  int32_t act, flags;
   float eps, reserved_f;
   const float *o, *x;
   const void* packed;
@@ -375,7 +378,7 @@
 } sst_encoder_tail_fwd_args;
 typedef struct sst_encoder_tail_bwd_args {
   int64_t m;
-  int32_t act, reserved;
+  int32_t act, flags;
   const float *dy2, *dy2p, *s2, *st2, *pre, *s1, *st1;
   const void* packed;
   const float *n1w, *n2w;
@@ -383,6 +386,7 @@
   float *dn2w, *dn2b, *dn1w, *dn1b;
   void* workspace;
 } sst_encoder_tail_bwd_args;
+int64_t sst_encoder_tail_handover_rows(int64_t m);
 int64_t sst_encoder_tail_pack_bytes(void);
 int sst_encoder_tail_pack_f32x6(const float* d_w_out, const float* d_w1, const float* d_w2, void* d_packed, void* stream);
 int sst_encoder_tail_pack_f32x6_many(const float* const* d_w_out, const float* const* d_w1, const float* const* d_w2,
diff --git a/sst_amd/_lib.py b/sst_amd/_lib.py
--- a/sst_amd/_lib.py
+++ b/sst_amd/_lib.py
@@ -194,7 +194,7 @@
     + [(k, _P) for k in ('x', 'xp', 'w_in', 'b_in', 'w_out', 'b_out', 'w1', 'b1', 'w2', 'b2', 'n1w', 'n1b', 'n2w', 'n2b',
                          'tok', 'winoff', 'order', 'pos_table', 'pos_idx',
                          'qkv', 'o', 'lse', 'y1', 's1', 'st1', 'pre', 'h', 's2', 'y2', 'st2', 'y2p', 'head_scale', 'wpack',
-                         'xpos_table', 'xpos_idx')]))
+                         'xpos_table', 'xpos_idx')] + [('tail_flags', ctypes.c_int32)]))
 EncoderLayerBwdArgs = _struct('EncoderLayerBwdArgs', 'sst_encoder_layer_bwd_args of include/sst_amd.h', (
     [('m', c_i64), ('n_windows', c_i64)] + [(k, ctypes.c_int32) for k in ('n_heads', 'act', 'max_tokens', 'impl')]
     + [('eps', ctypes.c_float), ('scale', ctypes.c_float)]
@@ -202,15 +202,17 @@
                          'w_in', 'w_out', 'w1', 'w2', 'n1w', 'n2w', 'tok', 'winoff', 'order',
                          'ds2', 'dpre', 'ds1', 'd_o', 'dqkv',
                          'dw_in', 'db_in', 'dwo', 'dbo', 'dw1', 'db1', 'dw2', 'db2', 'dn1w', 'dn1b', 'dn2w', 'dn2b',
-                         'workspace', 'head_scale', 'cos_r', 'dy1', 'wpack', 'xpos_table', 'xpos_idx')]))
-
-
+                         'workspace', 'head_scale', 'cos_r', 'dy1', 'wpack', 'xpos_table', 'xpos_idx')]
+    + [('tail_flags', ctypes.c_int32)]))
+
+
+TAIL_HANDOVER = 1
 EncoderTailFwdArgs = _struct('EncoderTailFwdArgs', 'sst_encoder_tail_fwd_args of include/sst_amd.h', (
-    [('m', c_i64), ('act', ctypes.c_int32), ('reserved', ctypes.c_int32), ('eps', ctypes.c_float), ('reserved_f', ctypes.c_float)]
+    [('m', c_i64), ('act', ctypes.c_int32), ('flags', ctypes.c_int32), ('eps', ctypes.c_float), ('reserved_f', ctypes.c_float)]
     + [(k, _P) for k in ('o', 'x', 'packed', 'b_out', 'b1', 'b2', 'n1w', 'n1b', 'n2w', 'n2b', 'pos_table', 'pos_idx',
                          's1', 'st1', 'y1', 'pre', 'h', 's2', 'st2', 'y2', 'y2p')]))
 EncoderTailBwdArgs = _struct('EncoderTailBwdArgs', 'sst_encoder_tail_bwd_args of include/sst_amd.h', (
-    [('m', c_i64), ('act', ctypes.c_int32), ('reserved', ctypes.c_int32)]
+    [('m', c_i64), ('act', ctypes.c_int32), ('flags', ctypes.c_int32)]
     + [(k, _P) for k in ('dy2', 'dy2p', 's2', 'st2', 'pre', 's1', 'st1', 'packed', 'n1w', 'n2w',
                          'ds2', 'dpre', 'ds1', 'd_o', 'dn2w', 'dn2b', 'dn1w', 'dn1b', 'workspace')]))
 
@@ -260,6 +262,7 @@
     'sst_encoder_layer_wpack_bytes': (c_i64, []),
     'sst_encoder_layer_fwd_f32x6': (c_i32, [c_ptr, c_ptr]),
     'sst_encoder_layer_bwd_f32x6': (c_i32, [c_ptr, c_ptr]),
+    'sst_encoder_tail_handover_rows': (c_i64, [c_i64]),
     'sst_encoder_tail_pack_bytes': (c_i64, []),
     'sst_encoder_tail_pack_f32x6': (c_i32, [c_ptr, c_ptr, c_ptr, c_ptr, c_ptr]),
     'sst_encoder_tail_pack_f32x6_many': (c_i32, [c_ptr, c_ptr, c_ptr, c_ptr, c_i32, c_ptr]),
diff --git a/sst_amd/csrc/gelu.h b/sst_amd/csrc/gelu.h
--- a/sst_amd/csrc/gelu.h
+++ b/sst_amd/csrc/gelu.h
@@ -23,5 +23,11 @@
   const float phi = 0.5f * (1.f + erf_as(x * 0.70710678118654752f, e));
   return fmaf(x * 0.3989422804014327f, e, phi);
 }
+__device__ __forceinline__ float gelu_with_grad_f(float x, float& grad) {
+  float e;
+  const float s = 1.f + erf_as(x * 0.70710678118654752f, e);
+  grad = fmaf(__fmul_rn(x, 0.3989422804014327f), e, __fmul_rn(0.5f, s));
+  return __fmul_rn(__fmul_rn(0.5f, x), s);
+}
 
 }
diff --git a/sst_amd/csrc/layer_exec.hip b/sst_amd/csrc/layer_exec.hip
--- a/sst_amd/csrc/layer_exec.hip
+++ b/sst_amd/csrc/layer_exec.hip
@@ -77,7 +77,7 @@
     if (rc) return rc;
   }
   sst_encoder_tail_fwd_args t;
-  t.m = m, t.act = a->act, t.reserved = 0, t.eps = a->eps, t.reserved_f = 0.f;
+  t.m = m, t.act = a->act, t.flags = a->tail_flags, t.eps = a->eps, t.reserved_f = 0.f;
   t.o = a->o, t.x = a->x, t.packed = a->wpack;
   t.b_out = a->b_out, t.b1 = a->b1, t.b2 = a->b2, t.n1w = a->n1w, t.n1b = a->n1b, t.n2w = a->n2w, t.n2b = a->n2b;
   t.pos_table = a->pos_table, t.pos_idx = a->pos_idx;
@@ -101,7 +101,7 @@
   void* ws_sra = ws;
   int rc;
   sst_encoder_tail_bwd_args t;
-  t.m = m, t.act = a->act, t.reserved = 0;
+  t.m = m, t.act = a->act, t.flags = a->tail_flags;
   t.dy2 = a->dy2, t.dy2p = a->dy2p, t.s2 = a->s2, t.st2 = a->st2, t.pre = a->pre, t.s1 = a->s1, t.st1 = a->st1;
   t.packed = a->wpack, t.n1w = a->n1w, t.n2w = a->n2w;
   t.ds2 = a->ds2, t.dpre = a->dpre, t.ds1 = a->ds1, t.d_o = a->d_o;
diff --git a/sst_amd/csrc/layer_tail_x6.hip b/sst_amd/csrc/layer_tail_x6.hip
--- a/sst_amd/csrc/layer_tail_x6.hip
+++ b/sst_amd/csrc/layer_tail_x6.hip
@@ -211,6 +211,33 @@
   v1 = *(const f32x4*)(t.scr + (t.frag_off0 ^ 16));
 }
 
+__device__ __forceinline__ int64_t ho_tile(int wave) {
+  return (int64_t)blockIdx.x * kWaves + __builtin_amdgcn_readfirstlane(wave);
+}
+typedef __attribute__((address_space(1))) unsigned char gbyte;
+__device__ __forceinline__ gbyte* ho_block(const float* base, int64_t tile, int ncb, int cb) {
+  const uint64_t b = (uint64_t)((const unsigned char*)base + (tile * ncb + cb) * (int64_t)kScr);
+  const uint32_t lo = __builtin_amdgcn_readfirstlane((uint32_t)b), hi = __builtin_amdgcn_readfirstlane((uint32_t)(b >> 32));
+  return (gbyte*)(((uint64_t)hi << 32) | lo);
+}
+__device__ __forceinline__ unsigned ho_lane_off(int lane) {
+  unsigned off = (unsigned)lane * 16u;
+  asm volatile("" : "+v"(off));
+  return off;
+}
+__device__ __forceinline__ void store_ho(float* base, int64_t tile, int ncb, int cb, int lane, const f32x4& v0, const f32x4& v1) {
+  gbyte* p = ho_block(base, tile, ncb, cb);
+  const unsigned off = ho_lane_off(lane);
+  __builtin_nontemporal_store(v0, (__attribute__((address_space(1))) f32x4*)(p + off));
+  __builtin_nontemporal_store(v1, (__attribute__((address_space(1))) f32x4*)(p + 1024 + off));
+}
+__device__ __forceinline__ void load_ho(const float* base, int64_t tile, int ncb, int cb, int lane, f32x4 (&w)[2]) {
+  const gbyte* p = ho_block(base, tile, ncb, cb);
+  const unsigned off = ho_lane_off(lane);
+  w[0] = *(const __attribute__((address_space(1))) f32x4*)(p + off);
+  w[1] = *(const __attribute__((address_space(1))) f32x4*)(p + 1024 + off);
+}
+
 template <int HALF>
 __device__ __forceinline__ void mma_half(const unsigned char* slot, int lane_off, const f32x4 (&x)[4][2], f32x4 (&acc)[8]) {
 #pragma unroll
@@ -338,7 +365,7 @@
   float* y2p;
 };
 
-template <int ACT>
+template <int ACT, bool HO>
 __global__ __launch_bounds__(kNTH, 2) void encoder_tail_fwd_x6_k(const tail_fwd_params P) {
   extern __shared__ __attribute__((aligned(16))) unsigned char lds[];
   float* par = (float*)(lds + kArea);
@@ -347,6 +374,7 @@
   const bool valid = r0 + c < P.m;
   const int64_t row = valid ? r0 + c : P.m - 1;
   const tile_io io = make_tile_io(lds + kArea + kParF * 4 + wave * kScr, lane, r0, P.m);
+  const int64_t tile = HO ? ho_tile(wave) : 0;
   const unsigned char* packed = P.packed;
   unsigned char* const part2 = lds + kPart1;
   dma_pieces<kWaves>(packed, lds, 3 * kIA / 1024, wave, lane);
@@ -394,7 +422,12 @@
       const int n0 = 32 * s + 8 * g;
       v[s][0] = acc[2 * s] + *(const f32x4*)(par + n0) + xr[s][0];
       v[s][1] = acc[2 * s + 1] + *(const f32x4*)(par + n0 + 4) + xr[s][1];
-      if (P.s1 != nullptr) store32<true>(io, P.s1, kC, 32 * s, v[s][0], v[s][1]);
+      if (P.s1 != nullptr) {
+        if (HO)
+          store_ho(P.s1, tile, 4, s, lane, v[s][0], v[s][1]);
+        else
+          store32<true>(io, P.s1, kC, 32 * s, v[s][0], v[s][1]);
+      }
     }
     float mean, rstd;
     ln_stats(v, P.eps, mean, rstd);
@@ -415,7 +448,10 @@
 #pragma unroll 1
   for (int j = 0; j < kNF; ++j) {
     if (j > 0) {
-      store32<true>(io, P.pre, kFF, kHC * (j - 1), sp0, sp1);
+      if (HO)
+        store_ho(P.pre, tile, kNF, j - 1, lane, sp0, sp1);
+      else
+        store32<true>(io, P.pre, kFF, kHC * (j - 1), sp0, sp1);
       store32<true>(io, P.h, kFF, kHC * (j - 1), sh0, sh1);
     }
     f32x4 p0, p1;
@@ -426,8 +462,20 @@
     f32x4 h0, h1;
 #pragma unroll
     for (int r = 0; r < 4; ++r) {
-      h0[r] = ACT == 1 ? gelu_f(p0[r]) : fmaxf(p0[r], 0.f);
-      h1[r] = ACT == 1 ? gelu_f(p1[r]) : fmaxf(p1[r], 0.f);
+      if (!HO) {
+        h0[r] = ACT == 1 ? gelu_f(p0[r]) : fmaxf(p0[r], 0.f);
+        h1[r] = ACT == 1 ? gelu_f(p1[r]) : fmaxf(p1[r], 0.f);
+      } else if (ACT == 1) {
+        float d0, d1;
+        h0[r] = gelu_with_grad_f(p0[r], d0);
+        h1[r] = gelu_with_grad_f(p1[r], d1);
+        p0[r] = d0, p1[r] = d1;
+      } else {
+        h0[r] = fmaxf(p0[r], 0.f);
+        h1[r] = fmaxf(p1[r], 0.f);
+        p0[r] = p0[r] > 0.f ? 1.f : 0.f;
+        p1[r] = p1[r] > 0.f ? 1.f : 0.f;
+      }
     }
     const img3 hs = split8(h0, h1);
     barrier_drain();
@@ -437,7 +485,10 @@
     barrier_drain();
     if (j + 1 < kNF) dma_pieces<kWaves>(packed + (size_t)(j + 3) * kSlot + kPart1, part2, kPart2 / 1024, wave, lane);
   }
-  store32<true>(io, P.pre, kFF, kHC * (kNF - 1), sp0, sp1);
+  if (HO)
+    store_ho(P.pre, tile, kNF, kNF - 1, lane, sp0, sp1);
+  else
+    store32<true>(io, P.pre, kFF, kHC * (kNF - 1), sp0, sp1);
   store32<true>(io, P.h, kFF, kHC * (kNF - 1), sh0, sh1);
   f32x4 v[4][2];
 #pragma unroll
@@ -447,7 +498,12 @@
     join8(yi[s], ya, yb);
     v[s][0] = acc[2 * s] + *(const f32x4*)(par + 3 * kC + n0) + ya;
     v[s][1] = acc[2 * s + 1] + *(const f32x4*)(par + 3 * kC + n0 + 4) + yb;
-    if (P.s2 != nullptr) store32<true>(io, P.s2, kC, 32 * s, v[s][0], v[s][1]);
+    if (P.s2 != nullptr) {
+      if (HO)
+        store_ho(P.s2, tile, 4, s, lane, v[s][0], v[s][1]);
+      else
+        store32<true>(io, P.s2, kC, 32 * s, v[s][0], v[s][1]);
+    }
   }
   float mean, rstd;
   ln_stats(v, P.eps, mean, rstd);
@@ -510,7 +566,7 @@
       for (int r = 0; r < 4; ++r) d[s][h][r] = st.y * (d[s][h][r] - mg - sv[s][h][r] * mgx);
 }
 
-template <int ACT>
+template <int ACT, bool HO>
 __global__ __launch_bounds__(kNTH, 2) void encoder_tail_bwd_x6_k(const tail_bwd_params P) {
   extern __shared__ __attribute__((aligned(16))) unsigned char lds[];
   float* par = (float*)(lds + kArea);
@@ -520,6 +576,19 @@
   const bool valid = r0 + c < P.m;
   const int64_t row = valid ? r0 + c : P.m - 1;
   const tile_io io = make_tile_io(lds + kArea + 2 * kC * 4 + kWaves * 2 * kC * 4 + wave * kScr, lane, r0, P.m);
+  const int64_t tile = HO ? ho_tile(wave) : 0;
+  auto saved_issue = [&](const float* base, int ncb, int cb, f32x4 (&w)[2]) __attribute__((always_inline)) {
+    if (HO)
+      load_ho(base, tile, ncb, cb, lane, w);
+    else
+      load32_issue(io, base, 32 * ncb, 32 * cb, w);
+  };
+  auto saved_finish = [&](const f32x4 (&w)[2], f32x4& v0, f32x4& v1) __attribute__((always_inline)) {
+    if (HO)
+      v0 = w[0], v1 = w[1];
+    else
+      load32_finish(io, w, v0, v1);
+  };
   const unsigned char* packed = P.packed;
   unsigned char* const part2 = lds + kPart1;
   dma_pieces<kWaves>(packed, lds, kSlot / 1024, wave, lane);
@@ -538,11 +607,11 @@
       }
     }
 #pragma unroll
-    for (int s = 0; s < 4; ++s) load32_issue(io, P.s2, kC, 32 * s, we[s]);
+    for (int s = 0; s < 4; ++s) saved_issue(P.s2, 4, s, we[s]);
 #pragma unroll
     for (int s = 0; s < 4; ++s) load32_finish(io, wd[s], d[s][0], d[s][1]);
 #pragma unroll
-    for (int s = 0; s < 4; ++s) load32_finish(io, we[s], sv[s][0], sv[s][1]);
+    for (int s = 0; s < 4; ++s) saved_finish(we[s], sv[s][0], sv[s][1]);
   }
   const float2 st2 = ((const float2*)P.st2)[row];
   for (int i = threadIdx.x; i < kC; i += kNTH) {
@@ -567,7 +636,7 @@
   for (int T = 0; T < 8; ++T) acc[T] = z4;
   f32x4 xs1[4][2];
   f32x4 pq[2];
-  load32_issue(io, P.pre, kFF, 0, pq);
+  saved_issue(P.pre, kNF, 0, pq);
 
   f32x4 sd0 = z4, sd1 = z4;
   auto ffn_chunk = [&](int j, const f32x4 q0, const f32x4 q1) __attribute__((always_inline)) {
@@ -576,8 +645,8 @@
     mma_first(lds, lane_off1, di, p0, p1);
 #pragma unroll
     for (int r = 0; r < 4; ++r) {
-      p0[r] *= ACT == 1 ? gelu_grad_f(q0[r]) : (q0[r] > 0.f ? 1.f : 0.f);
-      p1[r] *= ACT == 1 ? gelu_grad_f(q1[r]) : (q1[r] > 0.f ? 1.f : 0.f);
+      p0[r] *= HO ? q0[r] : ACT == 1 ? gelu_grad_f(q0[r]) : (q0[r] > 0.f ? 1.f : 0.f);
+      p1[r] *= HO ? q1[r] : ACT == 1 ? gelu_grad_f(q1[r]) : (q1[r] > 0.f ? 1.f : 0.f);
     }
     const img3 hs = split8(p0, p1);
     barrier_drain();
@@ -600,21 +669,21 @@
 #pragma unroll 1
   for (int j = 0; j < kNF - 1; ++j) {
     f32x4 q0, q1;
-    load32_finish(io, pq, q0, q1);
-    load32_issue(io, P.pre, kFF, kHC * (j + 1), pq);
+    saved_finish(pq, q0, q1);
+    saved_issue(P.pre, kNF, j + 1, pq);
     ffn_chunk(j, q0, q1);
   }
   {
     f32x4 q0, q1;
-    load32_finish(io, pq, q0, q1);
+    saved_finish(pq, q0, q1);
     ffn_chunk(kNF - 1, q0, q1);
     store32<SST_NT_BWD>(io, P.dpre, kFF, kHC * (kNF - 1), sd0, sd1);
     {
       f32x4 ws[4][2];
 #pragma unroll
-      for (int s = 0; s < 4; ++s) load32_issue(io, P.s1, kC, 32 * s, ws[s]);
-#pragma unroll
-      for (int s = 0; s < 4; ++s) load32_finish(io, ws[s], xs1[s][0], xs1[s][1]);
+      for (int s = 0; s < 4; ++s) saved_issue(P.s1, 4, s, ws[s]);
+#pragma unroll
+      for (int s = 0; s < 4; ++s) saved_finish(ws[s], xs1[s][0], xs1[s][1]);
     }
     f32x4 dd[4][2];
 #pragma unroll
@@ -664,11 +733,19 @@
   return SST_OK;
 }
 
+template <typename K, typename PARAMS>
+int launch_tail(K kernel, int lds_bytes, unsigned long long* mask, int64_t rows, hipStream_t st, const PARAMS& P) {
+  const int rc = configure(kernel, lds_bytes, mask);
+  if (rc) return rc;
+  hipLaunchKernelGGL(kernel, dim3((unsigned)rows), dim3(kNTH), lds_bytes, st, P);
+  return SST_OK;
+}
+
 }
 
 int sst_internal_encoder_tail_bwd_f32x6(const sst_encoder_tail_bwd_args* a, float** part2, float** part1, int* partial_rows,
                                         void* stream) {
-  if (!a || a->m <= 0 || (a->act != 1 && a->act != 2)) return SST_ERR_ARG;
+  if (!a || a->m <= 0 || (a->act != 1 && a->act != 2) || (a->flags & ~SST_TAIL_HANDOVER)) return SST_ERR_ARG;
   const void* need[] = {a->dy2, a->s2, a->st2, a->n2w, a->pre, a->s1, a->st1, a->n1w, a->packed,
                         a->ds2, a->dpre, a->ds1, a->d_o, a->workspace};
   for (const void* p : need)
@@ -683,16 +760,15 @@
   P.part2 = (float*)a->workspace;
   P.part1 = P.part2 + rows * 2 * kC;
   hipStream_t st = (hipStream_t)stream;
-  static unsigned long long cfg1 = 0, cfg2 = 0;
-  if (a->act == 1) {
-    const int rc = configure(encoder_tail_bwd_x6_k<1>, kLdsBwd, &cfg1);
-    if (rc) return rc;
-    hipLaunchKernelGGL(encoder_tail_bwd_x6_k<1>, dim3((unsigned)rows), dim3(kNTH), kLdsBwd, st, P);
-  } else {
-    const int rc = configure(encoder_tail_bwd_x6_k<2>, kLdsBwd, &cfg2);
-    if (rc) return rc;
-    hipLaunchKernelGGL(encoder_tail_bwd_x6_k<2>, dim3((unsigned)rows), dim3(kNTH), kLdsBwd, st, P);
-  }
+  static unsigned long long cfg[4] = {0, 0, 0, 0};
+  int rc;
+  if (a->flags & SST_TAIL_HANDOVER)
+    rc = a->act == 1 ? launch_tail(encoder_tail_bwd_x6_k<1, true>, kLdsBwd, &cfg[0], rows, st, P)
+                     : launch_tail(encoder_tail_bwd_x6_k<2, true>, kLdsBwd, &cfg[1], rows, st, P);
+  else
+    rc = a->act == 1 ? launch_tail(encoder_tail_bwd_x6_k<1, false>, kLdsBwd, &cfg[2], rows, st, P)
+                     : launch_tail(encoder_tail_bwd_x6_k<2, false>, kLdsBwd, &cfg[3], rows, st, P);
+  if (rc) return rc;
   SST_LAUNCH_CHECK();
   *part2 = P.part2, *part1 = P.part1, *partial_rows = (int)rows;
   return SST_OK;
@@ -751,13 +827,18 @@
   return sst_encoder_tail_pack_f32x6_many(&d_w_out, &d_w1, &d_w2, &d_packed, 1, stream);
 }
 
+int64_t sst_encoder_tail_handover_rows(int64_t m) {
+  if (m < 0) return SST_ERR_ARG;
+  return sst_div_up(m, (int64_t)kRowsPerWg) * kRowsPerWg;
+}
+
 int64_t sst_encoder_tail_bwd_workspace_bytes(int64_t m) {
   if (m < 0) return SST_ERR_ARG;
   return sst_align_up(2 * sst_div_up(m > 0 ? m : 1, (int64_t)kRowsPerWg) * 2 * kC * (int64_t)sizeof(float), 256);
 }
 
 int sst_encoder_tail_fwd_f32x6(const sst_encoder_tail_fwd_args* a, void* stream) {
-  if (!a || a->m < 0 || (a->act != 1 && a->act != 2)) return SST_ERR_ARG;
+  if (!a || a->m < 0 || (a->act != 1 && a->act != 2) || (a->flags & ~SST_TAIL_HANDOVER)) return SST_ERR_ARG;
   if (a->m == 0) return SST_OK;
   const void* need[] = {a->o, a->x, a->packed, a->n1w, a->n1b, a->n2w, a->n2b, a->st1, a->y1, a->pre, a->h, a->st2, a->y2};
   for (const void* p : need)
@@ -774,16 +855,15 @@
   const int64_t rows = sst_div_up(a->m, (int64_t)kRowsPerWg);
   if (rows > 0x7fffffff) return SST_ERR_UNSUPPORTED;
   hipStream_t st = (hipStream_t)stream;
-  static unsigned long long cfg1 = 0, cfg2 = 0;
-  if (a->act == 1) {
-    const int rc = configure(encoder_tail_fwd_x6_k<1>, kLdsFwd, &cfg1);
-    if (rc) return rc;
-    hipLaunchKernelGGL(encoder_tail_fwd_x6_k<1>, dim3((unsigned)rows), dim3(kNTH), kLdsFwd, st, P);
-  } else {
-    const int rc = configure(encoder_tail_fwd_x6_k<2>, kLdsFwd, &cfg2);
-    if (rc) return rc;
-    hipLaunchKernelGGL(encoder_tail_fwd_x6_k<2>, dim3((unsigned)rows), dim3(kNTH), kLdsFwd, st, P);
-  }
+  static unsigned long long cfg[4] = {0, 0, 0, 0};
+  int rc;
+  if (a->flags & SST_TAIL_HANDOVER)
+    rc = a->act == 1 ? launch_tail(encoder_tail_fwd_x6_k<1, true>, kLdsFwd, &cfg[0], rows, st, P)
+                     : launch_tail(encoder_tail_fwd_x6_k<2, true>, kLdsFwd, &cfg[1], rows, st, P);
+  else
+    rc = a->act == 1 ? launch_tail(encoder_tail_fwd_x6_k<1, false>, kLdsFwd, &cfg[2], rows, st, P)
+                     : launch_tail(encoder_tail_fwd_x6_k<2, false>, kLdsFwd, &cfg[3], rows, st, P);
+  if (rc) return rc;
   SST_LAUNCH_CHECK();
   return SST_OK;
 }
diff --git a/sst_amd/dense.py b/sst_amd/dense.py
--- a/sst_amd/dense.py
+++ b/sst_amd/dense.py
@@ -395,14 +395,29 @@
     return out
 
 
-def encoder_tail_fwd(o, x, packed, b_out, b1, b2, n1w, n1b, n2w, n2b, eps, act, save=True, pos=None, out=None):
+def handover_rows(m):
+    rows = int(_lib.load().sst_encoder_tail_handover_rows(m))
+    if rows < 0:
+        _lib.check(rows, 'sst_encoder_tail_handover_rows')
+    return rows
+
+
+def handover_to_rows(buf, m):
+    rows, cols = buf.shape
+    assert rows % 16 == 0 and cols % 32 == 0 and 0 <= m <= rows
+    v = buf.reshape(rows // 16, cols // 32, 2, 4, 16, 4)
+    return v.permute(0, 4, 1, 3, 2, 5).reshape(rows, cols)[:m]
+
+
+def encoder_tail_fwd(o, x, packed, b_out, b1, b2, n1w, n1b, n2w, n2b, eps, act, save=True, pos=None, out=None, handover=False):
     m = x.size(0)
     dev = x.device
     out = dict(out) if out else {}
+    rows_ho = handover_rows(m) if handover else m
 
     def e(name, cols):
         if name not in out or out[name] is None:
-            out[name] = torch.empty((m, cols), dtype=torch.float32, device=dev)
+            out[name] = torch.empty((rows_ho if name in ('s1', 'pre', 's2') else m, cols), dtype=torch.float32, device=dev)
         return out[name]
     s1 = e('s1', 128) if save else None
     out['s1'] = s1
@@ -411,7 +426,8 @@
     out['y2p'] = y2p
     P = lambda t: None if t is None else t.data_ptr()
     args = _lib.EncoderTailFwdArgs(
-        m, 1 if act == 'gelu' else 2, 0, float(eps), 0.0, P(o), P(x), P(packed), P(b_out), P(b1), P(b2), P(n1w), P(n1b),
+        m, 1 if act == 'gelu' else 2, _lib.TAIL_HANDOVER if handover else 0, float(eps), 0.0, P(o), P(x), P(packed), P(b_out),
+        P(b1), P(b2), P(n1w), P(n1b),
         P(n2w), P(n2b), P(pos[0]) if pos is not None else None, P(pos[1]) if pos is not None else None,
         P(s1), P(st1), P(y1), P(pre), P(h), P(s2), P(st2), P(y2), P(y2p))
     import ctypes
@@ -419,8 +435,12 @@
     return out
 
 
-def encoder_tail_bwd(dy2, dy2p, s2, st2, pre, s1, st1, packed, n1w, n2w, act, out=None):
+def encoder_tail_bwd(dy2, dy2p, s2, st2, pre, s1, st1, packed, n1w, n2w, act, out=None, handover=False):
     m = dy2.size(0)
+    if handover:
+        rows_ho = handover_rows(m)
+        if not all(t.is_contiguous() and t.numel() == rows_ho * c for t, c in ((s1, 128), (pre, 256), (s2, 128))):
+            raise RuntimeError('sst_amd: encoder_tail_bwd(handover=True) takes the buffers encoder_tail_fwd(handover=True) wrote')
     dev = dy2.device
     out = out or {}
 
@@ -432,7 +452,7 @@
     ws = out['ws'] if 'ws' in out else _lib.workspace(lib.sst_encoder_tail_bwd_workspace_bytes(m), dev)
     P = lambda t: None if t is None else t.data_ptr()
     d0 = dn.data_ptr()
-    args = _lib.EncoderTailBwdArgs(m, 1 if act == 'gelu' else 2, 0, P(dy2), P(dy2p), P(s2), P(st2), P(pre), P(s1), P(st1), P(packed),
+    args = _lib.EncoderTailBwdArgs(m, 1 if act == 'gelu' else 2, _lib.TAIL_HANDOVER if handover else 0, P(dy2), P(dy2p), P(s2), P(st2), P(pre), P(s1), P(st1), P(packed),
                                    P(n1w), P(n2w), P(ds2), P(dpre), P(ds1), P(d_o), d0, d0 + 512, d0 + 1024, d0 + 1536, P(ws))
     import ctypes
     _lib.check(lib.sst_encoder_tail_bwd_f32x6(ctypes.byref(args), _lib.stream_ptr()), 'sst_encoder_tail_bwd_f32x6')
diff --git a/sst_amd/sst_basic_block.py b/sst_amd/sst_basic_block.py
--- a/sst_amd/sst_basic_block.py
+++ b/sst_amd/sst_basic_block.py
@@ -188,11 +188,16 @@
          ('st2', 2))
 
 
+_SLAB_HANDOVER = ('s1', 'pre', 's2')
+
+
 def _slab_offsets(m):
+    from .dense import handover_rows
+    rows_ho = handover_rows(m)
     off, out = 0, {}
     for name, cols in _SLAB:
         out[name] = off
-        off += (m * cols * 4 + 255) // 256 * 256
+        off += ((rows_ho if name in _SLAB_HANDOVER else m) * cols * 4 + 255) // 256 * 256
     return out, off
 
 
@@ -223,7 +228,7 @@
         P(pos_next[0]) if pos_next is not None else None, P(pos_next[1]) if pos_next is not None else None,
         S('qkv'), S('o'), S('lse'), S('y1'), S('s1') if need_bwd else None, S('st1'), S('pre'), S('h'), S('s2'), P(y2), S('st2'),
         P(y2p), P(head_scale), P(wpack), P(pos_spec[0]) if pos_spec is not None else None,
-        P(pos_spec[1]) if pos_spec is not None else None)
+        P(pos_spec[1]) if pos_spec is not None else None, _lib.TAIL_HANDOVER)
     rc = K._bracket('sra_fwd', plan.n_tokens, lambda: lib.sst_encoder_layer_fwd_f32x6(ctypes.byref(args), _lib.stream_ptr()))
     if rc == _lib.SST_ERR_UNSUPPORTED:
         return None
@@ -275,7 +280,7 @@
         p_ds2, p_dpre, P(ds1), p_do, p_dqkv,
         P(dw_in), P(db_in), P(dwo), P(dbo), P(dw1), P(db1), P(dw2), P(db2), dnp, dnp + 512, dnp + 1024, dnp + 1536, P(ws),
         P(head_scale), P(cos_r), None, P(wpack), P(pos_spec[0]) if pos_spec is not None else None,
-        P(pos_spec[1]) if pos_spec is not None else None)
+        P(pos_spec[1]) if pos_spec is not None else None, _lib.TAIL_HANDOVER)
     rc = K._bracket('sra_bwd', plan.n_tokens, lambda: lib.sst_encoder_layer_bwd_f32x6(ctypes.byref(args), _lib.stream_ptr()))
     _lib.check(rc, 'sst_encoder_layer_bwd_f32x6')
     d_scale = K.head_scale_grad(cos_r, head_scale) if head_scale is not None else None
@@ -390,7 +395,8 @@
                 and encoder_tail_ok(o, x, w_out, w1, w2) and all(t is not None for t in (b_out, b1, b2))):
             if wpack is None:
                 wpack = encoder_tail_pack(w_out, w1, w2)
-            t = encoder_tail_fwd(o, x, wpack, b_out, b1, b2, n1w, n1b, n2w, n2b, eps, act, save=need_bwd, pos=pos_next)
+            t = encoder_tail_fwd(o, x, wpack, b_out, b1, b2, n1w, n1b, n2w, n2b, eps, act, save=need_bwd, pos=pos_next,
+                                 handover=True)
             s1, st1, y1, pre, h, s2, st2, y2, y2p = (t[k] for k in ('s1', 'st1', 'y1', 'pre', 'h', 's2', 'st2', 'y2', 'y2p'))
             ctx.tail = True
         else:
@@ -479,7 +485,7 @@
         dw1, db1 = torch.empty_like(w1), torch.empty(w1.size(0), **f32)
         if ctx.tail:
             ds2, dpre, ds1, do, dn = encoder_tail_bwd(dy2.contiguous(), dy2p.contiguous() if (ctx.two and dy2p is not None) else None,
-                                                      s2, st2, pre, s1, st1, wpack, n1w, n2w, ctx.act)
+                                                      s2, st2, pre, s1, st1, wpack, n1w, n2w, ctx.act, handover=True)
             ds2_for_w2 = ds2
             dn2w, dn2b, dn1w, dn1b = dn[0], dn[1], dn[2], dn[3]
         else:
```

Result: faster. 105.4 (median of 6 runs) (+1.3%).
